# p2004dr/visual-slam

Hardware: AMD Instinct MI355X
Metric: frames/sec (extract+match+pose) at 640×480, 2000 ORB, 1/2/4/8 MI355X (higher is better)
Workload: dtype u8

## Files before the change

include/vslam_amd.h:

```cpp
#ifndef VSLAM_AMD_H
#define VSLAM_AMD_H

#include <stddef.h>
#include <stdint.h>

#ifdef __cplusplus
extern "C" {
#endif

#define MO_ABI_VERSION 7
int mo_abi_version(void);

#define MO_OK 0
#define MO_ERR_ARG (-1)
#define MO_ERR_HIP (-2)
#define MO_ERR_CAPACITY (-3)
#define MO_ERR_UNSUPPORTED (-4)
#define MO_ERR_INDEX (-5)

#define MO_ORDER_LIBSTDCXX 0
#define MO_ORDER_MSVC 1

typedef struct mo_ctx mo_ctx;

// ... 1 lines not shown
    float x, y, size, angle, response;
    int32_t octave, class_id;
} mo_keypoint;

typedef struct {
    int32_t nfeatures;
    float scale_factor;
    int32_t nlevels;
    int32_t edge_threshold;
    int32_t first_level;
    int32_t wta_k;
    int32_t score_type;
    int32_t patch_size;
    int32_t fast_threshold;
    int32_t select_order;
} mo_orb_params;

mo_ctx* mo_create(int device, int max_w, int max_h, int max_batch);
void mo_destroy(mo_ctx*);
const char* mo_last_error(mo_ctx*);
int mo_set_stream(mo_ctx*, void* hip_stream);
int mo_set_stream_null(mo_ctx*);
int mo_sync(mo_ctx*);
int mo_device_count(void);

int mo_orb_detect_compute(mo_ctx*, const mo_orb_params*, const uint8_t* img, int w, int h, int stride, int ch,
                          int batch, mo_keypoint* kps, uint8_t* desc, int cap, int* counts);

int mo_orb_compute(mo_ctx*, const mo_orb_params*, const uint8_t* img, int w, int h, int stride, int ch,
                   const mo_keypoint* kps_in, int n_in, int32_t* kept_idx, uint8_t* desc, int* n_out);

int mo_orb_grid_good_features(mo_ctx*, const uint8_t* img, int w, int h, int stride, int ch, int n_features, float* xy,
                              int* n_out);
int mo_orb_grid_detect_compute(mo_ctx*, const mo_orb_params*, const uint8_t* img, int w, int h, int stride, int ch, int n_features,
                               float* xy, int* n_xy, int32_t* kept_idx, uint8_t* desc, int* n_kept);

int mo_undistort(mo_ctx*, const uint8_t* img, int w, int h, int stride, int ch, const double K[9], const double dist[5], uint8_t* out);
int mo_dev_undistort(mo_ctx*, const uint8_t* d_src, int w, int h, int ch, int batch, const double K[9], const double dist[5],
                     uint8_t* d_dst);

int mo_match_knn2_ratio(mo_ctx*, const uint8_t* q, int nq, const uint8_t* t, int nt, const double* ratio,
                        int batch, int32_t* train_idx, int32_t* dist, uint8_t* pass);

int mo_init_two_view(mo_ctx*, const float* p1, const float* p2, int m, const double K[9], double thr_px,
                     double prob, int n_hyp, uint64_t seed, double R[9], double t[3], double E[9],
                     uint8_t* ransac_inlier , uint8_t* inlier, float* X,
                     int* n_good);

int mo_recover_pose(mo_ctx*, const double E[9], const float* p1, const float* p2, int m, const double K[9],
                    const uint8_t* mask_in, double R[9], double t[3], uint8_t* mask_out, float* X, int* n_good);

int mo_find_fundamental(mo_ctx*, const float* p1, const float* p2, int m, double thr_px, double prob, int n_hyp, uint64_t seed,
                        double F[9], uint8_t* mask, int* n_inliers);

int mo_track_pair(mo_ctx*, const mo_keypoint* kps1, int n1, const uint8_t* desc1, const mo_keypoint* kps2, int n2,
                  const uint8_t* desc2, int w, int h, double ratio, double disp_frac, const double K[9], double thr_px,
                  int n_hyp, uint64_t seed, double R[9], double t[3], double E[9], int32_t* sel_idx, int32_t* sel_dist,
                  int* n_sel, uint8_t* inlier, int* n_inliers);

typedef struct {
    uint64_t token;
    const mo_keypoint* kps;
    const uint8_t* desc;
    int32_t n;
} mo_frame_ref;

typedef struct {
    int32_t mode;
    int32_t w, h;
    double ratio;
    double disp_frac;
    double K[9];
    double thr_px;
    int32_t n_hyp;
    uint64_t seed;
    uint64_t pair_index;
} mo_pair_params;

typedef struct {
    int32_t* match_idx;
    int32_t* match_dist;
    uint8_t* match_pass;
    int32_t* sel_idx;
    int32_t* sel_dist;
    uint8_t* inlier;
    uint8_t* ransac;
    float* X;
    double R[9], t[3], E[9];
    int32_t n_sel;
    int32_t n_good;
    int32_t n1, n2;
    uint64_t token1, token2;
} mo_pair_out;

int mo_last_token(mo_ctx*, uint64_t* token);
int mo_pair_frontend(mo_ctx*, const mo_frame_ref* f1, const mo_frame_ref* f2, const mo_pair_params*, mo_pair_out*);

int mo_triangulate_points(mo_ctx*, const double P1[12], const double P2[12], const float* p1, const float* p2, int n,
                          float* X4);

typedef struct {
    const uint8_t* d_gray;
    int32_t w, h, batch;
    int32_t cap;
    double ratio;
    double K[9];
    double thr_px;
    int32_t n_hyp;
    uint64_t seed;
    mo_keypoint* d_kps;
    uint8_t* d_desc;
    int32_t* d_counts;
    int32_t* d_match_idx;
    int32_t* d_match_dist;
    uint8_t* d_match_pass;
    double* d_pose;
    float* d_points;
    int32_t* d_n_points;
    int32_t mode;
    double disp_frac;
    int32_t* d_sel_idx;
    int32_t* d_sel_dist;
    int32_t* d_sel_n;
    uint8_t* d_pose_mask;
    uint64_t pair_index_base;
    int32_t detector;
    float* d_grid_xy;
    int32_t* d_grid_n;
    int32_t* d_grid_kept;
    int32_t n_kf_pairs;
    const int32_t* d_kf_query;
    const int32_t* d_kf_train;
    const double* d_kf_P1;
    const double* d_kf_P2;
    double* d_kf_F;
} mo_batch_io;

#define MO_MODE_INIT 0
#define MO_MODE_TRACK 1
#define MO_MODE_KEYFRAME 2
#define MO_DETECT_ORB 0
#define MO_DETECT_GRID 1

int mo_dev_frontend_batch(mo_ctx*, const mo_orb_params*, const mo_batch_io*);
int mo_dev_orb_detect_compute(mo_ctx*, const mo_orb_params*, const uint8_t* d_gray, int w, int h, int batch,
                              mo_keypoint* d_kps, uint8_t* d_desc, int cap, int32_t* d_counts);
int mo_dev_match_pairs(mo_ctx*, const uint8_t* d_desc, const int32_t* d_counts, int cap, const int32_t* d_qf,
                       const int32_t* d_tf, int n_pairs, double ratio, int32_t* d_idx, int32_t* d_dist,
                       uint8_t* d_pass);

typedef struct {
    int32_t w, h, ch;
    int32_t chunk;
    int32_t cap;
    int32_t detector;
    int32_t mode;
    double ratio, disp_frac, K[9], thr_px;
    int32_t n_hyp;
    uint64_t seed;
    uint64_t pair_index_base;
    int32_t want_matches;
    int32_t want_points;
} mo_stream_params;

typedef struct {
    int32_t n_frames, n_pairs;
    uint64_t first_frame;
    uint64_t first_pair;
    int32_t cap, flags;
    int32_t prev_count;
    const int32_t* counts;
    const mo_keypoint* kps;
    const uint8_t* desc;
    const int32_t* sel_idx;
    const int32_t* sel_dist;
    const int32_t* sel_n;
    const double* pose;
    const uint8_t* pose_mask;
    const int32_t* n_points;
    const int32_t* match_idx;
    const int32_t* match_dist;
    const uint8_t* match_pass;
    const float* points;
} mo_stream_result;

typedef struct mo_stream mo_stream;
mo_stream* mo_stream_create(mo_ctx*, const mo_orb_params*, const mo_stream_params*);
void mo_stream_destroy(mo_stream*);
int mo_stream_submit(mo_stream*, const uint8_t* frames, int n, int stride, size_t frame_stride);
int mo_stream_collect(mo_stream*, mo_stream_result*);
int mo_stream_lanes(void);
const char* mo_stream_last_error(mo_stream*);

int mo_comm_unique_id(uint8_t id[128]);
int mo_comm_init(mo_ctx*, const uint8_t id[128], int rank, int world);
int mo_comm_destroy(mo_ctx*);
int mo_gather_map_points(mo_ctx*, const float* d_local, int rows_local, int rows_max, int cap, int root, float* d_all,
                         int32_t* d_rows_all);

typedef struct mo_map mo_map;
typedef struct {
    double ratio;
    double thr_px;
    int32_t n_hyp;
    uint64_t seed;
    uint64_t pair_index;
} mo_map_kf_params;
typedef struct {
    int32_t* match_idx;
    uint8_t* match_pass;
    uint8_t* inlier;
    float* points;
    int32_t* kf_len;
    int32_t* kf_redundant;
    double F[9];
    int32_t n_new;
    int32_t from_token;
    int64_t n_points, n_obs;
} mo_map_kf_out;
typedef struct {
    double ratio;
    double thr_px;
    int32_t min_inliers;
    int32_t max_candidates;
    int32_t n_hyp;
    uint64_t seed;
} mo_map_reloc_params;
typedef struct {
    int32_t* point;
    uint8_t* inlier;
    int32_t* cand_pos;
    int32_t* cand_score;
    int32_t* cand_inliers;
    double pose[12];
    int32_t ok;
    int32_t kf_pos;
    int32_t n_cand;
    int32_t n_corr;
    int32_t n_inliers;
    int32_t from_token;
} mo_map_reloc_out;
#define MO_MAP_XYZ 0
#define MO_MAP_COLOR 1
#define MO_MAP_ID 2
#define MO_MAP_OBS_OFF 3
#define MO_MAP_OBS_KF 4
#define MO_MAP_OBS_KP 5
#define MO_MAP_DREF_KF 6
#define MO_MAP_DREF_ROW 7
#define MO_MAP_LIST_OFF 8
#define MO_MAP_LIST_IDS 9
mo_map* mo_map_create(mo_ctx*, int kf_slots, int kf_rows, int64_t pts_cap, int64_t obs_cap);
void mo_map_destroy(mo_map*);
int mo_map_add_keyframe(mo_map*, const mo_frame_ref* f, const double P[12], const uint8_t* img, int w, int h, int ch,
                        const mo_map_kf_params*, mo_map_kf_out*);
int mo_map_add_points(mo_map*, int n, const float* xyz, const uint8_t* col, const int32_t* id, const int32_t* obs_off, const int32_t* obs_kf,
                      const int32_t* obs_kp, const int32_t* dref_kf, const int32_t* dref_row);
int mo_map_remove_keyframes(mo_map*, const int32_t* positions, int n);
int mo_map_sizes(mo_map*, int64_t out[6]);
int mo_map_download(mo_map*, int field, void* dst, size_t bytes);
int mo_map_write_ply(mo_map*, const char* path, int min_obs, int64_t* n_written);
int mo_map_relocalize(mo_map*, const mo_frame_ref* f, const double K[9], const mo_map_reloc_params*, mo_map_reloc_out*);

typedef struct {
    int32_t w, h;
    int32_t window;
    int32_t n_pass;
    double radius[4];
    double scale_factor;
    double ratio;
    double chi2;
    int32_t max_dist;
    int32_t min_matches;
    int32_t min_inliers;
} mo_map_track_params;
typedef struct {
    int32_t* point;
    int32_t* dist;
    uint8_t* inlier;
    double pose[12];
    double pass_pose[4][12];
    double pass_radius[4];
    int32_t pass_cand[4];
    int32_t pass_matches[4];
    int32_t pass_inliers[4];
    int32_t n_pass_run;
    int32_t n_local;
    int32_t ok;
    int32_t from_token;
} mo_map_track_out;
int mo_map_track(mo_map*, const mo_frame_ref* f, const double K[9], const double pose0[12], const mo_map_track_params*, mo_map_track_out*);
int mo_format_floats(const float* v, int64_t n, char* out, size_t cap, size_t* len);

int mo_dev_status(mo_ctx*, int32_t flags[4]);

int mo_stage_times(mo_ctx*, const char*** names, float* ms, int cap);
int mo_stage_times_back(mo_ctx*, int back, const char*** names, float* ms, int cap);

int mo_host_times(mo_ctx*, double us[4]);
int mo_set_host_timing(mo_ctx*, int on);

int mo_dbg_pyramid_level(mo_ctx*, const mo_orb_params*, const uint8_t* gray, int w, int h, int level, int blurred,
                         uint8_t* out , int* lw, int* lh);
int mo_dbg_fast_level(mo_ctx*, const mo_orb_params*, const uint8_t* gray, int w, int h, int level,
                      int32_t* xys , int cap, int* n);
int mo_dbg_min_eigen(mo_ctx*, const uint8_t* gray, int w, int h, float* eig );
int mo_dbg_set_poison(mo_ctx*, int byte );
int mo_dbg_retain_best(mo_ctx*, const float* resp, int n, int n_points, int select_order, int32_t* order, int* n_out);

#ifdef __cplusplus
}
#endif
#endif
```

visual-slam_amd/csrc/api.hip:

```cpp
#include <algorithm>
#include <cmath>
#include <cstring>
#include <vector>

#include "common.h"

int mo_decode_host_flags(mo_ctx* c, int f0, int f1, const char* cap_msg) {
    if (f0 & 1) { c->tie_overflow = true; c->tie_levels = f1; return mo_fail(c, MO_ERR_CAPACITY, "internal per-level keypoint capacity exceeded (response ties)"); }
    if (f0 & 2) return mo_fail(c, MO_ERR_CAPACITY, cap_msg);
    return MO_OK;
}

extern "C" int mo_set_host_timing(mo_ctx* c, int on) {
    if (!c) return MO_ERR_ARG;
    c->host_timing = on != 0;
    return MO_OK;
}

extern "C" int mo_host_times(mo_ctx* c, double us[4]) {
    if (!c || !us) return MO_ERR_ARG;
    for (int i = 0; i < 4; i++) us[i] = c->host_us[i];
    return MO_OK;
}

static bool grow_fin_slots(mo_ctx* c, int levels);

static int check_flags(mo_ctx* c) {
    int f[4] = {0, 0, 0, 0};
    HIPCHK(c, hipMemcpyAsync(f, mo_host_flags(c), sizeof(f), hipMemcpyDeviceToHost, c->stream));
    HIPCHK(c, hipStreamSynchronize(c->stream));
    return mo_decode_host_flags(c, f[0], f[1]);
}

extern "C" int mo_dev_status(mo_ctx* c, int32_t flags[4]) {
    if (!c) return MO_ERR_ARG;
    HIPCHK(c, hipSetDevice(c->device));
    int f[4] = {0, 0, 0, 0};
    HIPCHK(c, hipMemcpyAsync(f, c->d_flags, sizeof(f), hipMemcpyDeviceToHost, c->stream));
    HIPCHK(c, hipMemsetAsync(c->d_flags, 0, 4 * sizeof(int), c->stream));
    HIPCHK(c, hipStreamSynchronize(c->stream));
    if (flags) { flags[0] = f[0]; flags[1] = f[1]; flags[2] = flags[3] = 0; }
    if (f[0] & 1) grow_fin_slots(c, f[1]);
    if (f[0] & 15) return mo_fail(c, MO_ERR_CAPACITY, "a capacity flag was raised by a mo_dev_* call (see mo_dev_status in vslam_amd.h)");
    return MO_OK;
}

int mo_run_extract(mo_ctx* c, const mo_orb_params* p, const uint8_t* d_gray, int w, int h, int batch,
                   mo_keypoint* d_kps, uint8_t* d_desc, int cap, int32_t* d_counts, int host_call) {
    int rc = mo_build_plan(c, p, w, h, batch);
    if (rc) return rc;
    if (cap < 1) return mo_fail(c, MO_ERR_ARG, "cap must be >= 1");
    c->flags_cur = host_call ? mo_host_flags(c) : c->d_flags;
    if (host_call == 1) HIPCHK(c, hipMemsetAsync(mo_host_flags(c), 0, 4 * sizeof(int), c->stream));
    if (c->poison >= 0) {
        HIPCHK(c, hipMemsetAsync(c->d_pyr, c->poison, (size_t)c->batch_alloc * c->plan.pyr_stride, c->stream));
        HIPCHK(c, hipMemsetAsync(c->d_blur, c->poison, (size_t)c->batch_alloc * c->plan.blur_stride, c->stream));
    }
    if (host_call) mo_stage_mark(c, "h2d");
    else mo_stage_begin(c);
    const int blur_margin = (c->plan.edge_threshold - 19) & ~3, pyr_margin = std::max(blur_margin - 4, 0);
    if (batch <= MO_FS_MAX_BATCH && c->fs_ok) {
        if ((rc = orb_launch_front_single(c, d_gray, batch, d_desc != nullptr))) return rc;
        mo_stage_mark(c, "pyramid");
        if (d_desc) mo_stage_mark(c, "blur");
    } else {
        if ((rc = orb_launch_pyramid(c, d_gray, batch, c->plan.nlevels, pyr_margin))) return rc;
        mo_stage_mark(c, "pyramid");
        if (d_desc) {
            if ((rc = orb_launch_blur(c, d_gray, batch, c->plan.nlevels, blur_margin))) return rc;
            mo_stage_mark(c, "blur");
        }
    }
    if ((rc = orb_launch_fast(c, d_gray, batch))) return rc;
    mo_stage_mark(c, "fast_nms");
    if ((rc = orb_launch_select(c, d_gray, batch))) return rc;
    mo_stage_mark(c, "select_harris");
    if ((rc = orb_launch_describe(c, d_gray, batch, d_kps, d_desc, cap, d_counts))) return rc;
    mo_stage_mark(c, "angle_rbrief");
    return MO_OK;
}

static int run_grid_extract(mo_ctx* c, const mo_orb_params* p, const mo_batch_io* io) {
    const int w = io->w, h = io->h, batch = io->batch, cap = io->cap;
    int rc = mo_build_plan(c, p, w, h, batch);
    if (rc) return rc;
    if (p->nfeatures < 64) return mo_fail(c, MO_ERR_ARG, "n_features must be >= 64 (8x8 grid)");
    if (cap < 1) return mo_fail(c, MO_ERR_ARG, "cap must be >= 1");
    const int per_cell = p->nfeatures / 64, slots = 64 * per_cell;
    const size_t B = (size_t)batch;
    Layout L;
    const size_t o_eig = L.take(B * w * h * sizeof(float)), o_xy = L.take(B * slots * 2 * sizeof(float)), o_n = L.take(B * 66 * sizeof(int)),
                 o_kb = L.take(B * 65 * sizeof(int32_t));
    if ((rc = mo_reserve(c, c->d_tmp, c->tmp_bytes, L.total))) return rc;
    float* d_eig = L.at<float>(c->d_tmp, o_eig);
    float* d_xy = io->d_grid_xy ? io->d_grid_xy : L.at<float>(c->d_tmp, o_xy);
    int* d_n = io->d_grid_n ? io->d_grid_n : L.at<int>(c->d_tmp, o_n);
    c->flags_cur = c->d_flags;
    mo_stage_begin(c);
    if ((rc = gftt_launch(c, io->d_gray, w, h, p->nfeatures, d_eig, d_xy, d_n, batch))) return rc;
    int32_t* d_kb = L.at<int32_t>(c->d_tmp, o_kb);
    if ((rc = gftt_records_launch(c, d_xy, d_n, per_cell, w, h, p->edge_threshold, io->d_kps, io->d_grid_kept, cap, io->d_counts, batch, d_kb))) return rc;
    mo_stage_mark(c, "grid_good_features");
    const int blur_margin = (c->plan.edge_threshold - 19) & ~3;
    if ((rc = orb_launch_blur(c, io->d_gray, batch, 1, blur_margin))) return rc;
    mo_stage_mark(c, "blur");
    rc = orb_launch_describe_cells(c, io->d_kps, d_kb, io->d_desc, cap, batch);
    if (rc == MO_ERR_UNSUPPORTED) rc = orb_launch_describe_given(c, io->d_gray, io->d_kps, cap, io->d_desc, io->d_counts, batch, 1);
    if (rc) return rc;
    mo_stage_mark(c, "compute");
    return MO_OK;
}

static int stage_images(mo_ctx* c, const uint8_t* img, int w, int h, int stride, int ch, int batch, const uint8_t** d_gray) {
    if (!img) return mo_fail(c, MO_ERR_ARG, "img is NULL");
    if (ch != 1 && ch != 3) return mo_fail(c, MO_ERR_ARG, "ch must be 1 (gray) or 3 (BGR)");
    if (stride < w * ch) return mo_fail(c, MO_ERR_ARG, "stride smaller than a row");
    size_t row = (size_t)w * ch, frame = row * h;
    int rc = mo_reserve(c, c->d_in, c->d_in_bytes, frame * batch);
    if (rc) return rc;
    HIPCHK(c, hipMemcpy2DAsync(c->d_in, row, img, (size_t)stride, row, (size_t)h * batch, hipMemcpyHostToDevice, c->stream));
    if (ch == 3) {
        rc = mo_reserve(c, c->d_gray, c->d_gray_bytes, (size_t)w * h * batch);
        if (rc) return rc;
        if ((rc = orb_launch_gray(c, c->d_in, w, h, batch, c->d_gray))) return rc;
        *d_gray = c->d_gray;
    } else {
        *d_gray = c->d_in;
    }
    return MO_OK;
}

static int reserve_out(mo_ctx* c, int batch, int cap) {
    const size_t n = (size_t)batch * cap;
    int rc = mo_reserve(c, c->d_kps, c->kps_bytes, n * sizeof(mo_keypoint));
    if (!rc) rc = mo_reserve(c, c->d_desc, c->desc_bytes, n * 32);
    if (!rc) rc = mo_reserve(c, c->d_counts, c->counts_bytes, (size_t)batch * sizeof(int));
    return rc;
}

int mo_host_stage(mo_ctx* c, size_t bytes) {
    if (c->h_stage_bytes >= bytes) return MO_OK;
    if (c->h_stage) { HIPCHK(c, hipStreamSynchronize(c->stream)); hipHostFree(c->h_stage); c->h_stage = nullptr; c->h_stage_bytes = 0; }
    bytes = (bytes + ((size_t)1 << 20) - 1) & ~(((size_t)1 << 20) - 1);
    HIPCHK(c, hipHostMalloc((void**)&c->h_stage, bytes, hipHostMallocMapped | hipHostMallocCoherent));
    c->h_stage_bytes = bytes;
    return MO_OK;
}

static bool grow_fin_slots(mo_ctx* c, int levels) {
    if (!c->plan_valid) return false;
    if (!levels) levels = (1 << c->plan.nlevels) - 1;
    bool grown = false;
    for (int L = 0; L < c->plan.nlevels; L++)
        if (((levels >> L) & 1) && c->plan.lv[L].fin_cap < c->plan.lv[L].cand_cap && c->fin_slack[L] < (1 << 24)) { c->fin_slack[L] *= 8; grown = true; }
    c->fin_slack_dirty = c->fin_slack_dirty || grown;
    return grown;
}

static int detect_compute_once(mo_ctx* c, const mo_orb_params* p, const uint8_t* img, int w, int h, int stride, int ch,
                               int batch, mo_keypoint* kps, uint8_t* desc, int cap, int* counts) {
    HIPCHK(c, hipSetDevice(c->device));
    if (batch == 1 && (size_t)w * h * ch + (size_t)cap * 60 <= (size_t)64 << 20) return mo_detect_single(c, p, img, w, h, stride, ch, kps, desc, cap, counts);
    HostClock clk(c);
    const uint8_t* d_gray = nullptr;
    int rc = mo_build_plan(c, p, w, h, batch);
    if (rc) return rc;
    mo_stage_begin(c);
    if ((rc = stage_images(c, img, w, h, stride, ch, batch, &d_gray))) return rc;
    if ((rc = reserve_out(c, batch, cap))) return rc;
    if ((rc = mo_run_extract(c, p, d_gray, w, h, batch, c->d_kps, desc ? c->d_desc : nullptr, cap, c->d_counts, true))) return rc;
    const size_t n_rows = (size_t)batch * cap, o_cnt = 4 * sizeof(int), o_kps = (o_cnt + (size_t)batch * sizeof(int) + 15) & ~(size_t)15;
    const size_t o_desc = o_kps + n_rows * sizeof(mo_keypoint), total = o_desc + (desc ? n_rows * 32 : 0);
    if (total <= (size_t)2 << 20) {
        if ((rc = mo_host_stage(c, total))) return rc;
        uint8_t* hs = c->h_stage;
        HIPCHK(c, hipMemcpyAsync(hs, mo_host_flags(c), 4 * sizeof(int), hipMemcpyDeviceToHost, c->stream));
        HIPCHK(c, hipMemcpyAsync(hs + o_cnt, c->d_counts, (size_t)batch * sizeof(int), hipMemcpyDeviceToHost, c->stream));
        HIPCHK(c, hipMemcpyAsync(hs + o_kps, c->d_kps, n_rows * sizeof(mo_keypoint), hipMemcpyDeviceToHost, c->stream));
        if (desc) HIPCHK(c, hipMemcpyAsync(hs + o_desc, c->d_desc, n_rows * 32, hipMemcpyDeviceToHost, c->stream));
        mo_stage_mark(c, "d2h");
        clk.enqueued();
        HIPCHK(c, hipStreamSynchronize(c->stream));
        clk.waited();
        std::memcpy(counts, hs + o_cnt, (size_t)batch * sizeof(int));
        if ((rc = mo_decode_host_flags(c, ((const int*)hs)[0], ((const int*)hs)[1]))) return rc;
        for (int f = 0; f < batch; f++) {
            const int n = std::min(counts[f], cap);
            if (n <= 0) continue;
            std::memcpy(kps + (size_t)f * cap, hs + o_kps + (size_t)f * cap * sizeof(mo_keypoint), (size_t)n * sizeof(mo_keypoint));
            if (desc) std::memcpy(desc + (size_t)f * cap * 32, hs + o_desc + (size_t)f * cap * 32, (size_t)n * 32);
        }
        return MO_OK;
    }
    HIPCHK(c, hipMemcpyAsync(counts, c->d_counts, (size_t)batch * sizeof(int), hipMemcpyDeviceToHost, c->stream));
    rc = check_flags(c);
    if (rc) return rc;
    for (int f = 0; f < batch; f++) {
        int n = std::min(counts[f], cap);
        if (n <= 0) continue;
        HIPCHK(c, hipMemcpyAsync(kps + (size_t)f * cap, c->d_kps + (size_t)f * cap, (size_t)n * sizeof(mo_keypoint),
                                 hipMemcpyDeviceToHost, c->stream));
        if (desc)
            HIPCHK(c, hipMemcpyAsync(desc + (size_t)f * cap * 32, c->d_desc + (size_t)f * cap * 32, (size_t)n * 32,
                                     hipMemcpyDeviceToHost, c->stream));
    }
    HIPCHK(c, hipStreamSynchronize(c->stream));
    return MO_OK;
}

extern "C" int mo_orb_detect_compute(mo_ctx* c, const mo_orb_params* p, const uint8_t* img, int w, int h, int stride, int ch,
                                     int batch, mo_keypoint* kps, uint8_t* desc, int cap, int* counts) {
    if (!c) return MO_ERR_ARG;
    if (!kps || !counts) return mo_fail(c, MO_ERR_ARG, "kps/counts is NULL");
    for (;;) {
        c->tie_overflow = false; c->tie_levels = 0;
        const int rc = detect_compute_once(c, p, img, w, h, stride, ch, batch, kps, desc, cap, counts);
        if (rc != MO_ERR_CAPACITY || !c->tie_overflow || !grow_fin_slots(c, c->tie_levels)) return rc;
    }
}

extern "C" int mo_orb_compute(mo_ctx* c, const mo_orb_params* p, const uint8_t* img, int w, int h, int stride, int ch,
                              const mo_keypoint* kps_in, int n_in, int32_t* kept_idx, uint8_t* desc, int* n_out) {
    if (!c) return MO_ERR_ARG;
    if (!p || !n_out || (n_in > 0 && (!kps_in || !kept_idx || !desc))) return mo_fail(c, MO_ERR_ARG, "NULL argument");
    HIPCHK(c, hipSetDevice(c->device));
    *n_out = 0;
    int nlevels = 0;
    bool sorted = true;
    for (int i = 0; i < n_in; i++) {
        int L = kps_in[i].octave;
        if (L < 0) return mo_fail(c, MO_ERR_ARG, "keypoint octave < 0");
        if (i > 0 && L < kps_in[i - 1].octave) sorted = false;
        nlevels = std::max(nlevels, L);
    }
    nlevels++;
    if (nlevels > MO_MAX_LEVELS) return mo_fail(c, MO_ERR_UNSUPPORTED, "keypoint octave >= 12");
    std::vector<int> keep;
    int et = p->edge_threshold;
    if (!(et > 0 && (h <= et * 2 || w <= et * 2))) {
        for (int i = 0; i < n_in; i++) {
            int x = (int)lrintf(kps_in[i].x), y = (int)lrintf(kps_in[i].y);
            if (et > 0 && !(x >= et && x < w - et && y >= et && y < h - et)) continue;
            keep.push_back(i);
        }
    }
    if (!sorted) {
        std::vector<int> re;
        for (int L = 0; L < nlevels; L++)
            for (int i : keep)
                if (kps_in[i].octave == L) re.push_back(i);
        keep.swap(re);
    }
    int n = (int)keep.size();
    for (int i = 0; i < n; i++) kept_idx[i] = keep[i];
    *n_out = n;
    if (n == 0) return MO_OK;
    mo_orb_params pp = *p;
    if (nlevels > pp.nlevels) pp.nlevels = nlevels;
    int rc = mo_build_plan(c, &pp, w, h, 1);
    if (rc) return rc;
    const uint8_t* d_gray = nullptr;
    if ((rc = stage_images(c, img, w, h, stride, ch, 1, &d_gray))) return rc;
    std::vector<mo_keypoint> kk(n);
    for (int i = 0; i < n; i++) kk[i] = kps_in[keep[i]];
    const size_t kb = (size_t)n * sizeof(mo_keypoint);
    Layout L;
    const size_t o_k = L.take(kb), o_d = L.take((size_t)n * 32);
    if ((rc = mo_reserve(c, c->d_tmp, c->tmp_bytes, L.total))) return rc;
    mo_keypoint* d_k = L.at<mo_keypoint>(c->d_tmp, o_k);
    uint8_t* d_d = L.at<uint8_t>(c->d_tmp, o_d);
    HIPCHK(c, hipMemcpyAsync(d_k, kk.data(), kb, hipMemcpyHostToDevice, c->stream));
    mo_stage_begin(c);
    if ((rc = orb_launch_pyramid(c, d_gray, 1, nlevels, 0))) return rc;
    if ((rc = orb_launch_blur(c, d_gray, 1, nlevels, 0))) return rc;
    if ((rc = orb_launch_describe_given(c, d_gray, d_k, n, d_d))) return rc;
    mo_stage_mark(c, "compute");
    HIPCHK(c, hipMemcpyAsync(desc, d_d, (size_t)n * 32, hipMemcpyDeviceToHost, c->stream));
    HIPCHK(c, hipStreamSynchronize(c->stream));
    return MO_OK;
}

extern "C" int mo_dev_undistort(mo_ctx* c, const uint8_t* d_src, int w, int h, int ch, int batch, const double K[9],
                                const double dist[5], uint8_t* d_dst) {
    if (!c) return MO_ERR_ARG;
    if (!d_src || !d_dst || !K || !dist || d_src == d_dst) return mo_fail(c, MO_ERR_ARG, "NULL argument (or in-place)");
    if (w < 1 || h < 1 || batch < 1 || (ch != 1 && ch != 3)) return mo_fail(c, MO_ERR_ARG, "bad size / channel count");
    if (!(K[0] != 0.0) || !(K[4] != 0.0)) return mo_fail(c, MO_ERR_ARG, "focal length is zero");
    HIPCHK(c, hipSetDevice(c->device));
    return undistort_launch(c, d_src, d_dst, w, h, ch, batch, K, dist);
}

extern "C" int mo_undistort(mo_ctx* c, const uint8_t* img, int w, int h, int stride, int ch, const double K[9], const double dist[5],
                            uint8_t* out) {
    if (!c) return MO_ERR_ARG;
    if (!img || !out || !K || !dist) return mo_fail(c, MO_ERR_ARG, "NULL argument");
    if (w < 1 || h < 1 || (ch != 1 && ch != 3) || stride < w * ch) return mo_fail(c, MO_ERR_ARG, "bad size / stride / channel count");
    if (!(K[0] != 0.0) || !(K[4] != 0.0)) return mo_fail(c, MO_ERR_ARG, "focal length is zero");
    HIPCHK(c, hipSetDevice(c->device));
    const size_t row = (size_t)w * ch, frame = row * h;
    Layout L;
    const size_t o_src = L.take(frame), o_dst = L.take(frame);
    int rc = mo_reserve(c, c->d_tmp, c->tmp_bytes, L.total);
    if (rc) return rc;
    uint8_t* d_src = L.at<uint8_t>(c->d_tmp, o_src);
    uint8_t* d_dst = L.at<uint8_t>(c->d_tmp, o_dst);
    HIPCHK(c, hipMemcpy2DAsync(d_src, row, img, (size_t)stride, row, (size_t)h, hipMemcpyHostToDevice, c->stream));
    mo_stage_begin(c);
    if ((rc = undistort_launch(c, d_src, d_dst, w, h, ch, 1, K, dist))) return rc;
    mo_stage_mark(c, "undistort");
    HIPCHK(c, hipMemcpyAsync(out, d_dst, frame, hipMemcpyDeviceToHost, c->stream));
    HIPCHK(c, hipStreamSynchronize(c->stream));
    return MO_OK;
}

static int gftt_run(mo_ctx* c, const uint8_t* img, int w, int h, int stride, int ch, int n_features, float* xy, int* n_out,
                    float* eig_out) {
    if (w < 64 || h < 64 || w > c->max_w || h > c->max_h) return mo_fail(c, MO_ERR_ARG, "image size outside the context limits");
    if (n_features < 64) return mo_fail(c, MO_ERR_ARG, "n_features must be >= 64 (8x8 grid)");
    const uint8_t* d_gray = nullptr;
    int rc = stage_images(c, img, w, h, stride, ch, 1, &d_gray);
    if (rc) return rc;
    const int per_cell = n_features / 64;
    const size_t eig_b = (size_t)w * h * sizeof(float), xy_b = (size_t)64 * per_cell * 2 * sizeof(float);
    Layout L;
    const size_t o_eig = L.take(eig_b), o_xy = L.take(xy_b), o_n = L.take(64 * sizeof(int));
    if ((rc = mo_reserve(c, c->d_tmp, c->tmp_bytes, L.total))) return rc;
    float* d_eig = L.at<float>(c->d_tmp, o_eig);
    float* d_xy = L.at<float>(c->d_tmp, o_xy);
    int* d_n = L.at<int>(c->d_tmp, o_n);
    c->flags_cur = mo_host_flags(c);
    HIPCHK(c, hipMemsetAsync(mo_host_flags(c), 0, 4 * sizeof(int), c->stream));
    mo_stage_begin(c);
    if ((rc = gftt_launch(c, d_gray, w, h, n_features, d_eig, d_xy, d_n))) return rc;
    mo_stage_mark(c, "grid_good_features");
    if (eig_out) HIPCHK(c, hipMemcpyAsync(eig_out, d_eig, eig_b, hipMemcpyDeviceToHost, c->stream));
    std::vector<float> hxy((size_t)64 * per_cell * 2);
    int hn[64];
    HIPCHK(c, hipMemcpyAsync(hxy.data(), d_xy, xy_b, hipMemcpyDeviceToHost, c->stream));
    HIPCHK(c, hipMemcpyAsync(hn, d_n, sizeof(hn), hipMemcpyDeviceToHost, c->stream));
    HIPCHK(c, hipStreamSynchronize(c->stream));
    int n = 0;
    if (xy)
        for (int cell = 0; cell < 64; cell++)
            for (int i = 0; i < hn[cell]; i++, n++) {
                xy[2 * n] = hxy[((size_t)cell * per_cell + i) * 2];
                xy[2 * n + 1] = hxy[((size_t)cell * per_cell + i) * 2 + 1];
            }
    if (n_out) *n_out = n;
    return MO_OK;
}

extern "C" int mo_orb_grid_good_features(mo_ctx* c, const uint8_t* img, int w, int h, int stride, int ch, int n_features,
                                         float* xy, int* n_out) {
    if (!c) return MO_ERR_ARG;
    if (!img || !xy || !n_out) return mo_fail(c, MO_ERR_ARG, "NULL argument");
    HIPCHK(c, hipSetDevice(c->device));
    return gftt_run(c, img, w, h, stride, ch, n_features, xy, n_out, nullptr);
}

extern "C" int mo_orb_grid_detect_compute(mo_ctx* c, const mo_orb_params* p, const uint8_t* img, int w, int h, int stride, int ch,
                                          int n_features, float* xy, int* n_xy, int32_t* kept_idx, uint8_t* desc, int* n_kept) {
    if (!c) return MO_ERR_ARG;
    if (!p || !img || !xy || !n_xy || !kept_idx || !desc || !n_kept) return mo_fail(c, MO_ERR_ARG, "NULL argument");
    HIPCHK(c, hipSetDevice(c->device));
    HostClock clk(c);
    *n_xy = 0; *n_kept = 0;
    c->last_token = 0;
    if (w < 64 || h < 64 || w > c->max_w || h > c->max_h) return mo_fail(c, MO_ERR_ARG, "image size outside the context limits");
    if (n_features < 64) return mo_fail(c, MO_ERR_ARG, "n_features must be >= 64 (8x8 grid)");
    if (ch != 1 && ch != 3) return mo_fail(c, MO_ERR_ARG, "ch must be 1 (gray) or 3 (BGR)");
    if (stride < w * ch) return mo_fail(c, MO_ERR_ARG, "stride smaller than a row");
    int rc = mo_build_plan(c, p, w, h, 1);
// ... 135 lines not shown
    if (!p1 || !p2 || !K || !R || !t || !inlier || !X || !n_good) return mo_fail(c, MO_ERR_ARG, "NULL argument");
    if (m < 0) return mo_fail(c, MO_ERR_ARG, "m must be >= 0");
    HIPCHK(c, hipSetDevice(c->device));
    *n_good = 0;
    if (m < 8) {
        for (int i = 0; i < 9; i++) R[i] = NAN;
        for (int i = 0; i < 3; i++) t[i] = NAN;
        std::memset(inlier, 0, (size_t)m);
        if (ransac_inlier) std::memset(ransac_inlier, 0, (size_t)m);
        if (E) for (int i = 0; i < 9; i++) E[i] = NAN;
        for (int i = 0; i < 3 * m; i++) X[i] = NAN;
        return MO_OK;
    }
    const size_t pb = (size_t)m * 2 * sizeof(float);
    Layout L;
    const size_t o_pose = L.take(12 * sizeof(double)), o_E = L.take(9 * sizeof(double)), o_n = L.take(sizeof(int32_t)), o_p1 = L.take(pb),
                 o_p2 = L.take(pb), o_X = L.take((size_t)m * 3 * sizeof(float)), o_inl = L.take(m), o_ran = L.take(m);
    int rc = mo_reserve(c, c->d_tmp, c->tmp_bytes, L.total);
    if (rc) return rc;
    uint8_t* b = (uint8_t*)c->d_tmp;
    double* d_pose = L.at<double>(b, o_pose);
    double* d_E = L.at<double>(b, o_E);
    int32_t* d_n = L.at<int32_t>(b, o_n);
    float* d_p1 = L.at<float>(b, o_p1);
    float* d_p2 = L.at<float>(b, o_p2);
    float* d_X = L.at<float>(b, o_X);
    uint8_t* d_inl = b + o_inl;
    uint8_t* d_ran = b + o_ran;
    HIPCHK(c, hipMemcpyAsync(d_p1, p1, pb, hipMemcpyHostToDevice, c->stream));
    HIPCHK(c, hipMemcpyAsync(d_p2, p2, pb, hipMemcpyHostToDevice, c->stream));
    TwoViewArgs a;
    a.n_pairs = 1; a.cap = m; a.n_hyp = n_hyp;
    for (int i = 0; i < 9; i++) a.K[i] = K[i];
    a.thr_px = thr_px; a.seed = seed;
    a.d_p1 = d_p1; a.d_p2 = d_p2; a.m_fixed = m;
    a.d_pose = d_pose; a.d_E = d_E; a.d_points = d_X; a.d_inlier = d_inl; a.d_ransac = d_ran; a.d_n_points = d_n;
    mo_stage_begin(c);
    if ((rc = twoview_launch(c, a))) return rc;
    mo_stage_mark(c, "two_view");
    double pose[12];
    int32_t ng = 0;
    HIPCHK(c, hipMemcpyAsync(pose, d_pose, sizeof(pose), hipMemcpyDeviceToHost, c->stream));
    if (E) HIPCHK(c, hipMemcpyAsync(E, d_E, 9 * sizeof(double), hipMemcpyDeviceToHost, c->stream));
    HIPCHK(c, hipMemcpyAsync(&ng, d_n, sizeof(ng), hipMemcpyDeviceToHost, c->stream));
    HIPCHK(c, hipMemcpyAsync(X, d_X, (size_t)m * 3 * sizeof(float), hipMemcpyDeviceToHost, c->stream));
    HIPCHK(c, hipMemcpyAsync(inlier, d_inl, (size_t)m, hipMemcpyDeviceToHost, c->stream));
    if (ransac_inlier) HIPCHK(c, hipMemcpyAsync(ransac_inlier, d_ran, (size_t)m, hipMemcpyDeviceToHost, c->stream));
    HIPCHK(c, hipStreamSynchronize(c->stream));
    for (int i = 0; i < 9; i++) R[i] = pose[i];
    for (int i = 0; i < 3; i++) t[i] = pose[9 + i];
    *n_good = ng;
    return MO_OK;
}

extern "C" int mo_recover_pose(mo_ctx* c, const double E[9], const float* p1, const float* p2, int m, const double K[9],
                               const uint8_t* mask_in, double R[9], double t[3], uint8_t* mask_out, float* X, int* n_good) {
    if (!c) return MO_ERR_ARG;
    if (!E || !K || !R || !t || !n_good || m < 0 || (m > 0 && (!p1 || !p2 || !mask_out))) return mo_fail(c, MO_ERR_ARG, "NULL / negative argument");
    HIPCHK(c, hipSetDevice(c->device));
    *n_good = 0;
    for (int i = 0; i < 9; i++) R[i] = NAN;
    for (int i = 0; i < 3; i++) t[i] = NAN;
    if (m == 0) return MO_OK;
    const size_t pb = (size_t)m * 2 * sizeof(float);
    Layout L;
    const size_t o_p1 = L.take(pb), o_p2 = L.take(pb), o_E = L.take(9 * sizeof(double)), o_min = L.take(m), o_pose = L.take(12 * sizeof(double)),
                 o_X = L.take((size_t)m * 3 * sizeof(float)), o_inl = L.take(m), o_n = L.take(sizeof(int32_t));
    int rc = mo_reserve(c, c->d_tmp, c->tmp_bytes, L.total);
    if (rc) return rc;
    uint8_t* b = (uint8_t*)c->d_tmp;
    HIPCHK(c, hipMemcpyAsync(b + o_p1, p1, pb, hipMemcpyHostToDevice, c->stream));
    HIPCHK(c, hipMemcpyAsync(b + o_p2, p2, pb, hipMemcpyHostToDevice, c->stream));
    HIPCHK(c, hipMemcpyAsync(b + o_E, E, 9 * sizeof(double), hipMemcpyHostToDevice, c->stream));
    if (mask_in) HIPCHK(c, hipMemcpyAsync(b + o_min, mask_in, (size_t)m, hipMemcpyHostToDevice, c->stream));
    TwoViewArgs a;
    a.n_pairs = 1; a.cap = m;
    for (int i = 0; i < 9; i++) a.K[i] = K[i];
    a.thr_px = 1.0;
    a.d_p1 = L.at<float>(b, o_p1); a.d_p2 = L.at<float>(b, o_p2); a.m_fixed = m;
    a.d_E_in = L.at<double>(b, o_E); a.d_mask_in = mask_in ? b + o_min : nullptr;
    a.d_pose = L.at<double>(b, o_pose); a.d_points = L.at<float>(b, o_X); a.d_inlier = b + o_inl; a.d_n_points = L.at<int32_t>(b, o_n);
    mo_stage_begin(c);
    if ((rc = twoview_launch(c, a))) return rc;
    mo_stage_mark(c, "recover_pose");
    double pose[12];
    int32_t ng = 0;
    HIPCHK(c, hipMemcpyAsync(pose, b + o_pose, sizeof(pose), hipMemcpyDeviceToHost, c->stream));
    HIPCHK(c, hipMemcpyAsync(mask_out, b + o_inl, (size_t)m, hipMemcpyDeviceToHost, c->stream));
    if (X) HIPCHK(c, hipMemcpyAsync(X, b + o_X, (size_t)m * 3 * sizeof(float), hipMemcpyDeviceToHost, c->stream));
    HIPCHK(c, hipMemcpyAsync(&ng, b + o_n, sizeof(ng), hipMemcpyDeviceToHost, c->stream));
    HIPCHK(c, hipStreamSynchronize(c->stream));
    for (int i = 0; i < 9; i++) R[i] = pose[i];
    for (int i = 0; i < 3; i++) t[i] = pose[9 + i];
    *n_good = ng;
    return MO_OK;
}

extern "C" int mo_find_fundamental(mo_ctx* c, const float* p1, const float* p2, int m, double thr_px, double prob, int n_hyp,
                                   uint64_t seed, double F[9], uint8_t* mask, int* n_inliers) {
    (void)prob;
    if (!c) return MO_ERR_ARG;
    if (!F || !n_inliers || m < 0 || (m > 0 && (!p1 || !p2 || !mask))) return mo_fail(c, MO_ERR_ARG, "NULL / negative argument");
    HIPCHK(c, hipSetDevice(c->device));
    *n_inliers = 0;
    for (int i = 0; i < 9; i++) F[i] = NAN;
    if (m < 8) { if (m > 0) std::memset(mask, 0, (size_t)m); return MO_OK; }
    const size_t pb = (size_t)m * 2 * sizeof(float);
    Layout L;
    const size_t o_p1 = L.take(pb), o_p2 = L.take(pb), o_F = L.take(9 * sizeof(double)), o_X = L.take((size_t)m * 3 * sizeof(float)),
                 o_ran = L.take(m), o_n = L.take(sizeof(int32_t));
    int rc = mo_reserve(c, c->d_tmp, c->tmp_bytes, L.total);
    if (rc) return rc;
    uint8_t* b = (uint8_t*)c->d_tmp;
    HIPCHK(c, hipMemcpyAsync(b + o_p1, p1, pb, hipMemcpyHostToDevice, c->stream));
    HIPCHK(c, hipMemcpyAsync(b + o_p2, p2, pb, hipMemcpyHostToDevice, c->stream));
    TwoViewArgs a = tv_fundamental(1, m, n_hyp, thr_px, seed, 0);
    a.d_p1 = L.at<float>(b, o_p1); a.d_p2 = L.at<float>(b, o_p2); a.m_fixed = m;
    a.d_E = L.at<double>(b, o_F); a.d_points = L.at<float>(b, o_X); a.d_ransac = b + o_ran; a.d_n_points = L.at<int32_t>(b, o_n);
    mo_stage_begin(c);
    if ((rc = twoview_launch(c, a))) return rc;
    mo_stage_mark(c, "find_fundamental");
    int32_t ng = 0;
    HIPCHK(c, hipMemcpyAsync(F, b + o_F, 9 * sizeof(double), hipMemcpyDeviceToHost, c->stream));
    HIPCHK(c, hipMemcpyAsync(mask, b + o_ran, (size_t)m, hipMemcpyDeviceToHost, c->stream));
    HIPCHK(c, hipMemcpyAsync(&ng, b + o_n, sizeof(ng), hipMemcpyDeviceToHost, c->stream));
    HIPCHK(c, hipStreamSynchronize(c->stream));
    *n_inliers = ng;
    return MO_OK;
}

extern "C" int mo_track_pair(mo_ctx* c, const mo_keypoint* kps1, int n1, const uint8_t* desc1, const mo_keypoint* kps2, int n2,
                             const uint8_t* desc2, int w, int h, double ratio, double disp_frac, const double K[9], double thr_px,
                             int n_hyp, uint64_t seed, double R[9], double t[3], double E[9], int32_t* sel_idx, int32_t* sel_dist,
                             int* n_sel, uint8_t* inlier, int* n_inliers) {
    if (!c) return MO_ERR_ARG;
    if (!K || !R || !t || !n_sel || !n_inliers || n1 < 0 || n2 < 0) return mo_fail(c, MO_ERR_ARG, "NULL / negative argument");
    *n_sel = 0; *n_inliers = 0;
    for (int i = 0; i < 9; i++) { R[i] = NAN; if (E) E[i] = NAN; }
    for (int i = 0; i < 3; i++) t[i] = NAN;
    if (n1 == 0 || n2 == 0) return MO_OK;
    if (!kps1 || !kps2 || !desc1 || !desc2 || !sel_idx || !inlier) return mo_fail(c, MO_ERR_ARG, "NULL argument");
    mo_frame_ref f1 = {0, kps1, desc1, n1}, f2 = {0, kps2, desc2, n2};
    mo_pair_params pp;
    std::memset(&pp, 0, sizeof(pp));
    pp.mode = MO_MODE_TRACK; pp.w = w; pp.h = h; pp.ratio = ratio; pp.disp_frac = disp_frac; pp.thr_px = thr_px; pp.n_hyp = n_hyp; pp.seed = seed;
    for (int i = 0; i < 9; i++) pp.K[i] = K[i];
    mo_pair_out o;
    std::memset(&o, 0, sizeof(o));
    o.sel_idx = sel_idx; o.sel_dist = sel_dist; o.inlier = inlier;
    const int rc = mo_pair_frontend(c, &f1, &f2, &pp, &o);
    if (rc) return rc;
    *n_sel = o.n_sel; *n_inliers = o.n_good;
    for (int i = 0; i < 9; i++) { R[i] = o.R[i]; if (E) E[i] = o.E[i]; }
    for (int i = 0; i < 3; i++) t[i] = o.t[i];
    return MO_OK;
}

extern "C" int mo_triangulate_points(mo_ctx* c, const double P1[12], const double P2[12], const float* p1, const float* p2,
                                     int n, float* X4) {
    if (!c) return MO_ERR_ARG;
    if (n < 0 || !P1 || !P2 || (n > 0 && (!p1 || !p2 || !X4))) return mo_fail(c, MO_ERR_ARG, "NULL argument");
    if (n == 0) return MO_OK;
    HIPCHK(c, hipSetDevice(c->device));
    const size_t pb = (size_t)n * 2 * sizeof(float);
    Layout L;
    const size_t o_p1 = L.take(pb), o_p2 = L.take(pb), o_X = L.take((size_t)n * 4 * sizeof(float));
    int rc = mo_reserve(c, c->d_tmp, c->tmp_bytes, L.total);
    if (rc) return rc;
    float* d_p1 = L.at<float>(c->d_tmp, o_p1);
    float* d_p2 = L.at<float>(c->d_tmp, o_p2);
    float* d_X = L.at<float>(c->d_tmp, o_X);
    HIPCHK(c, hipMemcpyAsync(d_p1, p1, pb, hipMemcpyHostToDevice, c->stream));
    HIPCHK(c, hipMemcpyAsync(d_p2, p2, pb, hipMemcpyHostToDevice, c->stream));
    if ((rc = triangulate_launch(c, P1, P2, d_p1, d_p2, n, d_X))) return rc;
    HIPCHK(c, hipMemcpyAsync(X4, d_X, (size_t)n * 4 * sizeof(float), hipMemcpyDeviceToHost, c->stream));
    HIPCHK(c, hipStreamSynchronize(c->stream));
    return MO_OK;
}

extern "C" int mo_dev_orb_detect_compute(mo_ctx* c, const mo_orb_params* p, const uint8_t* d_gray, int w, int h, int batch,
                                         mo_keypoint* d_kps, uint8_t* d_desc, int cap, int32_t* d_counts) {
    if (!c) return MO_ERR_ARG;
    if (!d_gray || !d_kps || !d_counts) return mo_fail(c, MO_ERR_ARG, "NULL device pointer");
    HIPCHK(c, hipSetDevice(c->device));
    return mo_run_extract(c, p, d_gray, w, h, batch, d_kps, d_desc, cap, d_counts, false);
}

extern "C" int mo_dev_match_pairs(mo_ctx* c, const uint8_t* d_desc, const int32_t* d_counts, int cap, const int32_t* d_qf,
                                  const int32_t* d_tf, int n_pairs, double ratio, int32_t* d_idx, int32_t* d_dist,
                                  uint8_t* d_pass) {
    if (!c) return MO_ERR_ARG;
    if (!d_desc || !d_counts || !d_idx || !d_dist || !d_pass) return mo_fail(c, MO_ERR_ARG, "NULL device pointer");
    HIPCHK(c, hipSetDevice(c->device));
    mo_stage_begin(c);
    int rc = match_launch_pairs(c, d_desc, d_desc, (size_t)cap * 32, (size_t)cap * 32, d_counts, d_qf, d_tf, 0, 0, n_pairs, cap,
                                ratio, d_idx, d_dist, d_pass);
    mo_stage_mark(c, "match_knn2_ratio");
    return rc;
}

__global__ void k_pair_frames(int32_t* qf, int32_t* tf, int n) {
    int i = blockIdx.x * blockDim.x + threadIdx.x;
    if (i < n) { qf[i] = i; tf[i] = i + 1; }
}

extern "C" int mo_dev_frontend_batch(mo_ctx* c, const mo_orb_params* p, const mo_batch_io* io) {
    if (!c) return MO_ERR_ARG;
    if (!io || !io->d_gray || !io->d_kps || !io->d_desc || !io->d_counts) return mo_fail(c, MO_ERR_ARG, "NULL in mo_batch_io");
    HIPCHK(c, hipSetDevice(c->device));
    if (io->detector != MO_DETECT_ORB && io->detector != MO_DETECT_GRID) return mo_fail(c, MO_ERR_ARG, "mo_batch_io.detector must be MO_DETECT_ORB or MO_DETECT_GRID");
    int rc = io->detector == MO_DETECT_GRID ? run_grid_extract(c, p, io)
                                            : mo_run_extract(c, p, io->d_gray, io->w, io->h, io->batch, io->d_kps, io->d_desc, io->cap, io->d_counts, false);
    if (rc) return rc;
    if (io->mode == MO_MODE_KEYFRAME) {
        const int np = io->n_kf_pairs;
        if (np < 1) return MO_OK;
        if (!io->d_kf_query || !io->d_kf_train || !io->d_kf_P1 || !io->d_kf_P2 || !io->d_match_idx || !io->d_match_dist || !io->d_match_pass ||
            !io->d_points || !io->d_n_points)
            return mo_fail(c, MO_ERR_ARG, "MO_MODE_KEYFRAME needs d_kf_query / d_kf_train / d_kf_P1 / d_kf_P2, the match outputs, d_points and d_n_points");
        if (io->n_hyp < 1) return mo_fail(c, MO_ERR_ARG, "MO_MODE_KEYFRAME needs n_hyp >= 1");
        rc = match_launch_pairs(c, io->d_desc, io->d_desc, (size_t)io->cap * 32, (size_t)io->cap * 32, io->d_counts, io->d_kf_query, io->d_kf_train,
                                0, 0, np, io->cap, io->ratio, io->d_match_idx, io->d_match_dist, io->d_match_pass);
        if (rc) return rc;
        mo_stage_mark(c, "match_knn2_ratio");
        TwoViewArgs a = tv_fundamental(np, io->cap, io->n_hyp, io->thr_px, io->seed, io->pair_index_base);
        a.d_kps = io->d_kps; a.d_counts = io->d_counts; a.d_match_idx = io->d_match_idx; a.d_match_pass = io->d_match_pass;
        a.d_qf = io->d_kf_query; a.d_tf = io->d_kf_train; a.need_two = 1; a.d_P1 = io->d_kf_P1; a.d_P2 = io->d_kf_P2;
        a.d_E = io->d_kf_F; a.d_points = io->d_points; a.d_n_points = io->d_n_points; a.d_inlier = io->d_pose_mask;
        if ((rc = twoview_launch(c, a))) return rc;
        mo_stage_mark(c, "keyframe_f_ransac_triangulate");
        return MO_OK;
    }
    int n_pairs = io->batch - 1;
    if (n_pairs < 1 || !io->d_match_idx) return MO_OK;
    if (!io->d_match_dist || !io->d_match_pass) return mo_fail(c, MO_ERR_ARG, "match outputs missing");
    if (c->pair_frames_n < n_pairs) {
        if (c->d_pair_frames) { HIPCHK(c, hipStreamSynchronize(c->stream)); HIPCHK(c, hipFree(c->d_pair_frames)); c->d_pair_frames = nullptr; }
        c->pair_frames_n = 0;
        HIPCHK(c, hipMalloc((void**)&c->d_pair_frames, (size_t)n_pairs * 2 * sizeof(int32_t)));
        hipLaunchKernelGGL(k_pair_frames, dim3((n_pairs + 255) / 256), dim3(256), 0, c->stream, c->d_pair_frames, c->d_pair_frames + n_pairs,
                           n_pairs);
        HIPCHK(c, hipGetLastError());
        c->pair_frames_n = n_pairs;
        c->pair_frames_split = n_pairs;
    }
    int32_t* qf = c->d_pair_frames;
    int32_t* tf = qf + c->pair_frames_split;
    rc = match_launch_pairs(c, io->d_desc, io->d_desc, (size_t)io->cap * 32, (size_t)io->cap * 32, io->d_counts, qf, tf, 0, 0,
                            n_pairs, io->cap, io->ratio, io->d_match_idx, io->d_match_dist, io->d_match_pass);
    if (rc) return rc;
    mo_stage_mark(c, "match_knn2_ratio");
    if (io->n_hyp > 0) {
        if (!io->d_points || !io->d_n_points) return mo_fail(c, MO_ERR_ARG, "two-view outputs missing");
        TwoViewArgs a;
        a.n_pairs = n_pairs; a.cap = io->cap; a.n_hyp = io->n_hyp;
        for (int i = 0; i < 9; i++) a.K[i] = io->K[i];
        a.thr_px = io->thr_px; a.seed = io->seed; a.pair_base = io->pair_index_base;
        a.d_kps = io->d_kps; a.d_counts = io->d_counts; a.d_match_idx = io->d_match_idx; a.d_match_pass = io->d_match_pass;
        a.d_pose = io->d_pose; a.d_points = io->d_points; a.d_n_points = io->d_n_points; a.d_inlier = io->d_pose_mask;
        if (io->mode == MO_MODE_TRACK) {
            if (!io->d_sel_idx || !io->d_sel_n) return mo_fail(c, MO_ERR_ARG, "MO_MODE_TRACK needs d_sel_idx and d_sel_n");
            if ((rc = track_select_launch(c, io->d_kps, io->d_counts, qf, tf, io->d_match_idx, io->d_match_dist, io->d_match_pass,
                                          io->cap, n_pairs, io->w, io->h, io->disp_frac, io->d_sel_idx, io->d_sel_dist, io->d_sel_n)))
                return rc;
            mo_stage_mark(c, "track_filters");
            a.d_sel = io->d_sel_idx; a.d_sel_n = io->d_sel_n;
        } else if (io->mode != MO_MODE_INIT) return mo_fail(c, MO_ERR_ARG, "mo_batch_io.mode must be MO_MODE_INIT or MO_MODE_TRACK");
        if ((rc = twoview_launch(c, a))) return rc;
        mo_stage_mark(c, "two_view");
    }
    return MO_OK;
}

extern "C" int mo_dbg_pyramid_level(mo_ctx* c, const mo_orb_params* p, const uint8_t* gray, int w, int h, int level,
                                    int blurred, uint8_t* out, int* lw, int* lh) {
    if (!c) return MO_ERR_ARG;
    HIPCHK(c, hipSetDevice(c->device));
    int rc = mo_build_plan(c, p, w, h, 1);
    if (rc) return rc;
    if (level < 0 || level >= c->plan.nlevels) return mo_fail(c, MO_ERR_ARG, "level out of range");
    const uint8_t* d_gray = nullptr;
    if ((rc = stage_images(c, gray, w, h, w, 1, 1, &d_gray))) return rc;
    const bool fused = (blurred & 2) != 0;
    blurred &= 1;
    if (fused) {
        if (!c->fs_ok) return mo_fail(c, MO_ERR_UNSUPPORTED, std::string("the single-frame pyramid kernel does not cover this geometry: ") + c->fs_why);
        HIPCHK(c, hipMemsetAsync(c->d_pyr, 0xA5, (size_t)c->plan.pyr_stride, c->stream));
        HIPCHK(c, hipMemsetAsync(c->d_blur, 0xA5, (size_t)c->plan.blur_stride, c->stream));
        if ((rc = orb_launch_front_single(c, d_gray, 1, 1))) return rc;
    } else if ((rc = orb_launch_pyramid(c, d_gray, 1, c->plan.nlevels, 0))) return rc;
    const LevelInfo& v = c->plan.lv[level];
    *lw = v.w; *lh = v.h;
    if (blurred) {
        if (!fused && (rc = orb_launch_blur(c, d_gray, 1, c->plan.nlevels, 0))) return rc;
        HIPCHK(c, hipMemcpy2DAsync(out, v.w, c->d_blur + v.boff, v.bpitch, v.w, v.h, hipMemcpyDeviceToHost, c->stream));
    } else {
        const uint8_t* src = level == 0 ? d_gray : c->d_pyr + v.off;
        HIPCHK(c, hipMemcpy2DAsync(out, v.w, src, v.pitch, v.w, v.h, hipMemcpyDeviceToHost, c->stream));
    }
    HIPCHK(c, hipStreamSynchronize(c->stream));
    return MO_OK;
}

extern "C" int mo_dbg_fast_level(mo_ctx* c, const mo_orb_params* p, const uint8_t* gray, int w, int h, int level,
                                 int32_t* xys, int cap, int* n) {
    if (!c) return MO_ERR_ARG;
    HIPCHK(c, hipSetDevice(c->device));
    int rc = mo_build_plan(c, p, w, h, 1);
    if (rc) return rc;
    if (level < 0 || level >= c->plan.nlevels) return mo_fail(c, MO_ERR_ARG, "level out of range");
    const uint8_t* d_gray = nullptr;
    if ((rc = stage_images(c, gray, w, h, w, 1, 1, &d_gray))) return rc;
    if ((rc = orb_launch_pyramid(c, d_gray, 1, c->plan.nlevels, 0))) return rc;
    if ((rc = orb_launch_fast(c, d_gray, 1))) return rc;
    const LevelInfo& v = c->plan.lv[level];
    std::vector<int> cnt(std::max(v.nstrips, 1));
    std::vector<uint32_t> ent((size_t)std::max(v.cand_cap, 1));
    if (v.nstrips > 0) {
        HIPCHK(c, hipMemcpyAsync(cnt.data(), c->d_strip_cnt + v.strip_base, v.nstrips * sizeof(int), hipMemcpyDeviceToHost, c->stream));
        HIPCHK(c, hipMemcpyAsync(ent.data(), c->d_cand + v.cand_off, (size_t)v.cand_cap * sizeof(uint32_t), hipMemcpyDeviceToHost, c->stream));
    }
    HIPCHK(c, hipStreamSynchronize(c->stream));
    int k = 0;
    for (int s = 0; s < v.nstrips; s++)
        for (int i = 0; i < cnt[s]; i++) {
            uint32_t e = ent[(size_t)s * v.strip_cap + i];
            if (k < cap) { xys[3 * k] = e & 0xFFF; xys[3 * k + 1] = (e >> 12) & 0xFFF; xys[3 * k + 2] = e >> 24; }
            k++;
        }
    *n = k;
    return MO_OK;
}

extern "C" int mo_dbg_retain_best(mo_ctx* c, const float* resp, int n, int n_points, int select_order, int32_t* order,
                                  int* n_out) {
    if (!c) return MO_ERR_ARG;
    HIPCHK(c, hipSetDevice(c->device));
    if (n <= 0) { *n_out = 0; return MO_OK; }
    float* d_r = nullptr; int32_t* d_o = nullptr; int* d_n = nullptr;
    HIPCHK(c, hipMalloc((void**)&d_r, (size_t)n * sizeof(float)));
    HIPCHK(c, hipMalloc((void**)&d_o, (size_t)n * sizeof(int32_t)));
    HIPCHK(c, hipMalloc((void**)&d_n, sizeof(int)));
    HIPCHK(c, hipMemcpyAsync(d_r, resp, (size_t)n * sizeof(float), hipMemcpyHostToDevice, c->stream));
    int rc = orb_launch_retain_probe(c, d_r, n, n_points, select_order, d_o, d_n);
    if (!rc) {
        HIPCHK(c, hipMemcpyAsync(n_out, d_n, sizeof(int), hipMemcpyDeviceToHost, c->stream));
        HIPCHK(c, hipStreamSynchronize(c->stream));
        HIPCHK(c, hipMemcpy(order, d_o, (size_t)(*n_out) * sizeof(int32_t), hipMemcpyDeviceToHost));
    }
    hipFree(d_r); hipFree(d_o); hipFree(d_n);
    return rc;
}
```

visual-slam_amd/csrc/common.h:

```cpp
#pragma once
#include <hip/hip_runtime.h>
#include <chrono>
#include <cstring>
#include <stdint.h>
#include <string>
#include <type_traits>
#include <vector>

#include "../../include/vslam_amd.h"

#define MO_MAX_LEVELS 12
#define MO_HALF_PATCH 15
#define MO_STRIP_ROWS 8
#ifndef MO_STRIP_ROWS_LATENCY
#define MO_STRIP_ROWS_LATENCY 2
#endif
#define SEL_MAXSTRIPS 2047

struct LevelInfo {
    int w, h, pitch;
    int off;
    int bpitch, boff;
    float scale;
    int quota;
    int bx0, by0, bw, bh;
    uint32_t inv_bw;
    int strip_rows;
    int nstrips;
    int strip_cap;
    int strip_base;
    int cand_off;
    int cand_cap;
    int fin_off, fin_cap;
    int scr_off;
};

struct Plan {
    int w, h, nlevels;
    int edge_threshold, fast_threshold, select_order, nfeatures;
    int pyr_stride;
    int blur_stride;
    int strips_per_frame;
    int cand_stride;
    int fin_stride;
    int umax[MO_HALF_PATCH + 1];
    int gk[7];
    LevelInfo lv[MO_MAX_LEVELS];
};

struct FinalKp {
    uint16_t x, y;
    float response;
};

struct ResizeTab {
    uint32_t* xpk = nullptr; uint32_t* ypk = nullptr;
    int* xofs = nullptr; int* xc1 = nullptr; int* yofs = nullptr; int* yc1 = nullptr;
    bool two_pass_ok = true;
};

#define MO_RESULT_SLOTS 4
#define MO_NSTAGES 16
#define MO_TIMING_SLOTS 64

struct TimingSet {
    hipEvent_t ev[MO_NSTAGES + 1] = {};
    const char* names[MO_NSTAGES + 1] = {};
    int n_stages = 0;
};

struct mo_ctx {
    int device = 0;
    int max_w = 0, max_h = 0, max_batch = 0;
    hipStream_t own_stream = nullptr, stream = nullptr;
    int match_mode = 0;
    int poison = -1;
    std::string err;

    bool plan_valid = false;
    int fin_slack[MO_MAX_LEVELS] = {1, 1, 1, 1, 1, 1, 1, 1, 1, 1, 1, 1};
    bool fin_slack_dirty = false;
    bool tie_overflow = false;
    int tie_levels = 0;
    mo_orb_params plan_params{};
    Plan plan{};
    ResizeTab rtab[MO_MAX_LEVELS];
    int batch_alloc = 0;

    uint8_t* d_in = nullptr;       size_t d_in_bytes = 0;
    uint8_t* d_gray = nullptr;     size_t d_gray_bytes = 0;
    uint8_t* d_pyr = nullptr;
    uint8_t* d_blur = nullptr;
    uint32_t* d_cand = nullptr;
    int* d_strip_cnt = nullptr;
    uint64_t* d_scratch = nullptr;
    size_t scratch_stride = 0;
    FinalKp* d_fin = nullptr;
    int* d_fin_cnt = nullptr;
    uint32_t* d_tile_tab[2] = {nullptr, nullptr};
    int tile_cum[2][MO_MAX_LEVELS + 1] = {};
    int tile_margin = 0;
    uint32_t* d_fs_tab = nullptr; int fs_tiles = 0, fs_stride = 0, fs_lds = 0; bool fs_ok = false; int fs_geom[10] = {}; const char* fs_why = "";
    uint32_t* d_strip_tab = nullptr; int n_strip_tab = 0;
    uint32_t* d_dtile_tab = nullptr; int n_dtiles = 0, dtile_icw_off = 0;
    int* d_dtodo = nullptr; size_t dtodo_bytes = 0;
    int* d_flags = nullptr;
    int* flags_cur = nullptr;
    unsigned lds_attr_done = 0;
    mo_keypoint* d_kps = nullptr; uint8_t* d_desc = nullptr; int* d_counts = nullptr; size_t kps_bytes = 0, desc_bytes = 0, counts_bytes = 0;
    mo_keypoint* d_slot_kps = nullptr; uint8_t* d_slot_desc = nullptr; int32_t* d_slot_cnt = nullptr; int32_t* d_slot_ids = nullptr;
    int slot_cap = 0, slot_cur = -1;
    uint64_t slot_token[MO_RESULT_SLOTS] = {}; int slot_n[MO_RESULT_SLOTS] = {}; uint64_t token_next = 1, last_token = 0;
    bool host_timing = false;
    uint8_t* d_mq = nullptr; uint8_t* d_mt = nullptr; int32_t* d_midx = nullptr; int32_t* d_mdist = nullptr;
    uint8_t* d_mpass = nullptr; size_t m_q_bytes = 0, m_t_bytes = 0, m_idx_bytes = 0, m_dist_bytes = 0, m_pass_bytes = 0;
    uint2* d_match_part = nullptr; size_t match_part_bytes = 0;
    void* d_tv = nullptr; size_t tv_bytes = 0;
    float* d_stream_pts = nullptr; size_t stream_pts_bytes = 0;
    uint32_t* d_track_keys = nullptr; size_t track_keys_bytes = 0;
    void* d_tmp = nullptr; size_t tmp_bytes = 0;

    void* comm = nullptr; int comm_rank = 0, comm_world = 1;
    int32_t* d_comm_cnt = nullptr;

    double host_us[4] = {0, 0, 0, 0};
    uint8_t* h_stage = nullptr; size_t h_stage_bytes = 0;
    int32_t* d_pair_frames = nullptr; int pair_frames_n = 0, pair_frames_split = 0;
    TimingSet tsets[MO_TIMING_SLOTS];
    int tcur = 0;
    bool timing = true;
};

int mo_fail(mo_ctx* c, int code, const std::string& msg);

#define HIPCHK(c, expr)                                                                              \
    do {                                                                                             \
        hipError_t e__ = (expr);                                                                     \
        if (e__ != hipSuccess)                                                                       \
            return mo_fail((c), MO_ERR_HIP, std::string(#expr) + ": " + hipGetErrorString(e__));     \
    } while (0)

template <class T> int mo_reserve(mo_ctx* c, T*& p, size_t& have_bytes, size_t need_bytes) {
    if (need_bytes <= have_bytes && p) return MO_OK;
    T* old = p;
    p = nullptr; have_bytes = 0;
    if (old) HIPCHK(c, hipFree(old));
    HIPCHK(c, hipMalloc((void**)&p, need_bytes ? need_bytes : 16));
    have_bytes = need_bytes;
    return MO_OK;
}

static inline size_t mo_align(size_t v, size_t a) { return (v + a - 1) & ~(a - 1); }

struct Layout {
    size_t total = 0;
    size_t take(size_t bytes) { const size_t o = total; total += mo_align(bytes, 256); return o; }
    template <class T> static T* at(void* base, size_t off) { return (T*)((uint8_t*)base + off); }
};

static inline void mo_copy_rows(uint8_t* dst, const uint8_t* src, size_t row, int h, size_t stride) {
    if (stride == row) std::memcpy(dst, src, row * h);
    else for (int y = 0; y < h; y++) std::memcpy(dst + (size_t)y * row, src + (size_t)y * stride, row);
}

int mo_host_stage(mo_ctx* c, size_t bytes);
static inline int* mo_host_flags(mo_ctx* c) { return c->d_flags + 4; }
int mo_decode_host_flags(mo_ctx* c, int f0, int f1, const char* cap_msg = "more keypoints than cap; counts holds the required sizes");

static inline double now_us() { return std::chrono::duration<double, std::micro>(std::chrono::steady_clock::now().time_since_epoch()).count(); }
struct HostClock {
    mo_ctx* c; double t0, t1 = 0, t2 = 0;
    explicit HostClock(mo_ctx* c_) : c(c_), t0(now_us()) { c->timing = c->host_timing; }
    void enqueued() { t1 = now_us(); }
    void waited() { t2 = now_us(); }
    ~HostClock() {
        const double t3 = now_us();
        if (t1 == 0) t1 = t2 = t3; else if (t2 == 0) t2 = t3;
        c->host_us[0] = t1 - t0; c->host_us[1] = t2 - t1; c->host_us[2] = t3 - t2; c->host_us[3] = t3 - t0;
        c->timing = true;
    }
};

int mo_run_extract(mo_ctx* c, const mo_orb_params* p, const uint8_t* d_gray, int w, int h, int batch, mo_keypoint* d_kps, uint8_t* d_desc,
                   int cap, int32_t* d_counts, int host_call);
int mo_detect_single(mo_ctx* c, const mo_orb_params* p, const uint8_t* img, int w, int h, int stride, int ch, mo_keypoint* kps,
                     uint8_t* desc, int cap, int* counts);

int mo_slot_acquire(mo_ctx* c, int rows, int* slot);
uint64_t mo_slot_commit(mo_ctx* c, int slot, int n);
uint8_t* mo_stage_dev(mo_ctx* c);
int mo_slot_of(const mo_ctx* c, uint64_t token);
int mo_frame_lookup(mo_ctx* c, const mo_frame_ref* f, const char* what, int* slot, int* n);
int mo_frame_copy_rows(mo_ctx* c, const mo_frame_ref* f, int slot, int n, mo_keypoint* d_kps, uint8_t* d_desc);
void mo_copy_out_launch(mo_ctx* c, const void* d_src, void* h_dst_dev, size_t bytes);

void mo_stage_begin(mo_ctx* c);
void mo_stage_mark(mo_ctx* c, const char* name);

int mo_build_plan(mo_ctx* c, const mo_orb_params* p, int w, int h, int batch);

int orb_launch_gray(mo_ctx* c, const uint8_t* d_bgr, int w, int h, int batch, uint8_t* d_gray);
int orb_launch_ingest(mo_ctx* c, const uint8_t* src_mapped, int w, int h, int ch, uint8_t* d_gray, int* flags_clear);
int orb_launch_pyramid(mo_ctx* c, const uint8_t* d_gray, int batch, int nlevels, int margin);
#define MO_FS_MAX_BATCH 2
int fs_build(mo_ctx* c);
int orb_launch_front_single(mo_ctx* c, const uint8_t* d_gray, int batch, int want_blur);
void mo_linear_coeffs(int srcsize, int dstsize, std::vector<int>& ofs, std::vector<int>& c1);
int orb_launch_blur(mo_ctx* c, const uint8_t* d_gray, int batch, int nlevels, int margin);
int orb_launch_fast(mo_ctx* c, const uint8_t* d_gray, int batch, int level_lo = 0, int level_hi = MO_MAX_LEVELS);
int orb_launch_select(mo_ctx* c, const uint8_t* d_gray, int batch, int level_lo = 0, int level_hi = MO_MAX_LEVELS);
int orb_launch_describe(mo_ctx* c, const uint8_t* d_gray, int batch, mo_keypoint* d_kps, uint8_t* d_desc, int cap,
                        int* d_counts);
int orb_launch_describe_given(mo_ctx* c, const uint8_t* d_gray, const mo_keypoint* d_kps, int n, uint8_t* d_desc, const int* d_n = nullptr,
                              int batch = 1, int n_stride = 0);
int gftt_records_launch(mo_ctx* c, const float* d_xy, int* d_cell_n, int per_cell, int w, int h, int edge, mo_keypoint* d_rec,
                        int32_t* d_kept, int rec_stride, int32_t* d_counts_out, int batch, int32_t* d_kbase = nullptr);
int orb_launch_describe_cells(mo_ctx* c, const mo_keypoint* d_kps, const int32_t* d_kbase, uint8_t* d_desc, int cap, int batch);
int orb_launch_retain_probe(mo_ctx* c, const float* d_resp, int n, int n_points, int order, int32_t* d_order,
                            int* d_nout);
int match_launch_pairs(mo_ctx* c, const uint8_t* d_q, const uint8_t* d_t, size_t q_stride, size_t t_stride,
                       const int32_t* d_counts, const int32_t* d_qf, const int32_t* d_tf, int nq_fixed, int nt_fixed,
                       int n_pairs, int out_stride, double ratio, int32_t* d_idx, int32_t* d_dist, uint8_t* d_pass);
int gftt_launch(mo_ctx* c, const uint8_t* d_gray, int w, int h, int n_features, float* d_eig, float* d_xy, int* d_n, int batch = 1);
struct TwoViewArgs {
    int n_pairs = 0, cap = 0, n_hyp = 0;
    int model = 0;
    double K[9] = {}, thr_px = 0;
    uint64_t seed = 0;
    uint64_t pair_base = 0;
    const mo_keypoint* d_kps = nullptr; const int32_t* d_counts = nullptr; const int32_t* d_match_idx = nullptr; const uint8_t* d_match_pass = nullptr;
    const int32_t* d_sel = nullptr; const int32_t* d_sel_n = nullptr;
    const float* d_p1 = nullptr; const float* d_p2 = nullptr; int m_fixed = 0;
    const int32_t* d_qf = nullptr; const int32_t* d_tf = nullptr;
    int need_two = 0;
    const double* d_P1 = nullptr; const double* d_P2 = nullptr;
    const double* d_E_in = nullptr; const uint8_t* d_mask_in = nullptr;
    double* d_pose = nullptr;
    double* d_E = nullptr;
    float* d_points = nullptr;
    uint8_t* d_inlier = nullptr;
    uint8_t* d_ransac = nullptr;
    int32_t* d_n_points = nullptr;
    int* flags = nullptr;
};
static_assert(std::is_trivially_copyable<TwoViewArgs>::value, "TwoViewArgs is a kernel argument");
static inline TwoViewArgs tv_fundamental(int n_pairs, int cap, int n_hyp, double thr_px, uint64_t seed, uint64_t pair_base) {
    TwoViewArgs a;
    a.n_pairs = n_pairs; a.cap = cap; a.n_hyp = n_hyp; a.model = 1;
    a.K[0] = a.K[4] = a.K[8] = 1.0;
    a.thr_px = thr_px; a.seed = seed; a.pair_base = pair_base;
    return a;
}
int twoview_launch(mo_ctx* c, const TwoViewArgs& a);
int undistort_launch(mo_ctx* c, const uint8_t* d_src, uint8_t* d_dst, int w, int h, int ch, int batch, const double K[9],
                     const double dist[5]);
int track_select_launch(mo_ctx* c, const mo_keypoint* d_kps, const int32_t* d_counts, const int32_t* d_qf, const int32_t* d_tf,
                        const int32_t* d_midx, const int32_t* d_mdist, const uint8_t* d_mpass, int cap, int n_pairs, int w, int h,
                        double disp_frac, int32_t* d_sel, int32_t* d_sel_dist, int32_t* d_sel_n);
size_t twoview_workspace_bytes(int n_pairs, int cap, int n_hyp);
int triangulate_launch(mo_ctx* c, const double* P1, const double* P2, const float* d_p1, const float* d_p2, int n, float* d_X4);
```

visual-slam_amd/csrc/ctx.hip:

```cpp
#include <algorithm>
#include <cmath>
#include <cstring>
#include <vector>

#include <cstdlib>

#include "common.h"

int mo_fail(mo_ctx* c, int code, const std::string& msg) {
    if (c) c->err = msg;
    return code;
}

static std::string g_create_err;

static inline int cv_round_f(float v) { return (int)lrintf(v); }
static inline int cv_round_d(double v) { return (int)lrint(v); }
static inline int align_up(int v, int a) { return (v + a - 1) / a * a; }

extern "C" int mo_abi_version(void) { return MO_ABI_VERSION; }

extern "C" int mo_device_count(void) {
    int n = 0;
    if (hipGetDeviceCount(&n) != hipSuccess) return 0;
    return n;
}

extern "C" mo_ctx* mo_create(int device, int max_w, int max_h, int max_batch) {
    int n = 0;
    hipError_t e = hipGetDeviceCount(&n);
    if (e != hipSuccess || n <= 0) {
        g_create_err = "mo_create: no HIP device available (this library has no CPU fallback)";
        return nullptr;
    }
    if (device < 0 || device >= n || max_w < 64 || max_h < 64 || max_w > 4095 || max_h > 4095 || max_batch < 1) {
        g_create_err = "mo_create: bad arguments (need 64 <= w,h <= 4095, batch >= 1, valid device)";
        return nullptr;
    }
    if (hipSetDevice(device) != hipSuccess) {
        g_create_err = "mo_create: hipSetDevice failed";
        return nullptr;
    }
    mo_ctx* c = new mo_ctx();
    c->device = device;
    c->max_w = max_w; c->max_h = max_h; c->max_batch = max_batch;
    if (hipStreamCreateWithFlags(&c->own_stream, hipStreamNonBlocking) != hipSuccess) {
        g_create_err = "mo_create: hipStreamCreate failed";
        delete c;
        return nullptr;
    }
    c->stream = c->own_stream;
    if (const char* e = getenv("VSLAM_AMD_MATCHER")) c->match_mode = std::strcmp(e, "mfma") == 0 ? 1 : 0;
    const unsigned evf = (unsigned)hipEventDisableSystemFence;
    for (TimingSet& t : c->tsets)
        for (int i = 0; i <= MO_NSTAGES; i++) hipEventCreateWithFlags(&t.ev[i], evf);
    if (hipMalloc((void**)&c->d_flags, 8 * sizeof(int)) != hipSuccess) {
        g_create_err = "mo_create: hipMalloc failed";
        delete c;
        return nullptr;
    }
    hipMemset(c->d_flags, 0, 8 * sizeof(int));
    c->flags_cur = c->d_flags;
    return c;
}

static void free_plan_buffers(mo_ctx* c) {
    for (int L = 0; L < MO_MAX_LEVELS; L++) {
        ResizeTab& t = c->rtab[L];
        if (t.xpk) hipFree(t.xpk);
        t = ResizeTab();
    }
    void* bufs[] = {c->d_pyr, c->d_blur, c->d_cand, c->d_strip_cnt, c->d_scratch, c->d_fin, c->d_fin_cnt, c->d_tile_tab[0], c->d_tile_tab[1], c->d_strip_tab, c->d_dtile_tab};
    c->d_dtile_tab = nullptr; c->n_dtiles = 0;
    if (c->d_fs_tab) hipFree(c->d_fs_tab);
    c->d_fs_tab = nullptr; c->fs_ok = false;
    for (void* b : bufs) if (b) hipFree(b);
    c->d_tile_tab[0] = c->d_tile_tab[1] = nullptr; c->d_strip_tab = nullptr; c->n_strip_tab = 0;
    c->d_pyr = c->d_blur = nullptr; c->d_cand = nullptr; c->d_strip_cnt = nullptr; c->d_scratch = nullptr;
    c->d_fin = nullptr; c->d_fin_cnt = nullptr;
    c->batch_alloc = 0;
    c->plan_valid = false;
}

extern "C" void mo_destroy(mo_ctx* c) {
    if (!c) return;
    hipSetDevice(c->device);
    hipDeviceSynchronize();
    mo_comm_destroy(c);
    free_plan_buffers(c);
    void* bufs[] = {c->d_in, c->d_gray, c->d_flags, c->d_kps, c->d_desc, c->d_counts, c->d_mq, c->d_mt,
                    c->d_midx, c->d_mdist, c->d_mpass, c->d_match_part, c->d_tv, c->d_tmp, c->d_pair_frames, c->d_dtodo, c->d_comm_cnt,
                    c->d_slot_kps, c->d_slot_desc, c->d_slot_cnt, c->d_slot_ids, c->d_track_keys, c->d_stream_pts};
    for (void* b : bufs) if (b) hipFree(b);
    if (c->h_stage) hipHostFree(c->h_stage);
    for (TimingSet& t : c->tsets) {
        for (int i = 0; i <= MO_NSTAGES; i++) if (t.ev[i]) hipEventDestroy(t.ev[i]);
    }
    if (c->own_stream) hipStreamDestroy(c->own_stream);
    delete c;
}

extern "C" const char* mo_last_error(mo_ctx* c) { return c ? c->err.c_str() : g_create_err.c_str(); }

extern "C" int mo_set_stream(mo_ctx* c, void* s) {
    if (!c) return MO_ERR_ARG;
    c->stream = s ? (hipStream_t)s : c->own_stream;
    return MO_OK;
}

extern "C" int mo_set_stream_null(mo_ctx* c) {
    if (!c) return MO_ERR_ARG;
    c->stream = nullptr;
    return MO_OK;
}

extern "C" int mo_sync(mo_ctx* c) {
    if (!c) return MO_ERR_ARG;
    HIPCHK(c, hipStreamSynchronize(c->stream));
    return MO_OK;
}

void mo_stage_begin(mo_ctx* c) {
    c->tcur = (c->tcur + 1) % MO_TIMING_SLOTS;
    TimingSet& t = c->tsets[c->tcur];
    t.n_stages = 0;
    if (c->timing) hipEventRecord(t.ev[0], c->stream);
}

void mo_stage_mark(mo_ctx* c, const char* name) {
    TimingSet& t = c->tsets[c->tcur];
    if (!c->timing || t.n_stages >= MO_NSTAGES) return;
    t.names[t.n_stages] = name;
    t.n_stages++;
    hipEventRecord(t.ev[t.n_stages], c->stream);
}

extern "C" int mo_stage_times_back(mo_ctx* c, int back, const char*** names, float* ms, int cap) {
    if (!c) return MO_ERR_ARG;
    if (back < 0 || back >= MO_TIMING_SLOTS) return mo_fail(c, MO_ERR_ARG, "mo_stage_times_back: back outside the ring of event sets");
    TimingSet& t = c->tsets[((c->tcur - back) % MO_TIMING_SLOTS + MO_TIMING_SLOTS) % MO_TIMING_SLOTS];
    if (t.n_stages == 0) return 0;
    HIPCHK(c, hipEventSynchronize(t.ev[t.n_stages]));
    int n = std::min(cap, t.n_stages);
    for (int i = 0; i < n; i++) {
        float v = 0;
        hipEventElapsedTime(&v, t.ev[i], t.ev[i + 1]);
        ms[i] = v;
    }
    t.names[t.n_stages] = nullptr;
    if (names) *names = t.names;
    return n;
}

extern "C" int mo_stage_times(mo_ctx* c, const char*** names, float* ms, int cap) { return mo_stage_times_back(c, 0, names, ms, cap); }

void mo_linear_coeffs(int srcsize, int dstsize, std::vector<int>& ofs, std::vector<int>& c1) {
    ofs.assign(dstsize, 0);
    c1.assign(dstsize, 0);
    double inv_scale = (double)dstsize / (double)srcsize;
    double scale = 1.0 / inv_scale;
    int minofst = 0, maxofst = dstsize;
    for (int val = 0; val < dstsize; val++) {
        double fval = scale * ((double)val + 0.5) - 0.5;
        int ival = (int)std::floor(fval);
        if (ival >= 0 && srcsize > 1) {
            if (ival < srcsize - 1) {
                ofs[val] = ival;
                c1[val] = cv_round_d((fval - (double)ival) * 256.0);
            } else {
                ofs[val] = srcsize - 1;
                maxofst = std::min(maxofst, val);
            }
        } else {
            minofst = std::max(minofst, val + 1);
        }
    }
    for (int val = 0; val < dstsize; val++) {
        if (val < minofst) { ofs[val] = 0; c1[val] = 0; }
        if (val >= maxofst) { ofs[val] = srcsize - 1; c1[val] = 0; }
    }
}

static bool params_equal(const mo_orb_params& a, const mo_orb_params& b) {
    return std::memcmp(&a, &b, sizeof(a)) == 0;
}

int mo_build_plan(mo_ctx* c, const mo_orb_params* p, int w, int h, int batch) {
    if (!p) return mo_fail(c, MO_ERR_ARG, "params is NULL");
    if (w < 64 || h < 64 || w > c->max_w || h > c->max_h)
        return mo_fail(c, MO_ERR_ARG, "image size outside the context's max_w/max_h (or < 64)");
    if (batch < 1 || batch > c->max_batch) return mo_fail(c, MO_ERR_ARG, "batch outside 1..max_batch");
    if (p->nlevels < 1 || p->nlevels > MO_MAX_LEVELS) return mo_fail(c, MO_ERR_ARG, "nlevels must be 1..12");
    if (p->first_level != 0 || p->wta_k != 2 || p->score_type != 0 || p->patch_size != 31)
        return mo_fail(c, MO_ERR_UNSUPPORTED,
                       "only firstLevel=0, WTA_K=2, HARRIS_SCORE, patchSize=31 (the reference's values) are built");
    if (p->edge_threshold < 19 || p->edge_threshold > 1024)
        return mo_fail(c, MO_ERR_UNSUPPORTED, "edge_threshold must be >= 19 (descriptor radius)");
    if (p->nfeatures < 1 || !(p->scale_factor > 1.0f) || p->scale_factor > 2.0f)
        return mo_fail(c, MO_ERR_ARG, "nfeatures >= 1, 1 < scale_factor <= 2");
    if (p->select_order != MO_ORDER_LIBSTDCXX && p->select_order != MO_ORDER_MSVC)
        return mo_fail(c, MO_ERR_ARG, "select_order must be MO_ORDER_LIBSTDCXX or MO_ORDER_MSVC");

    const bool same_key = c->plan_valid && params_equal(c->plan_params, *p) && c->plan.w == w && c->plan.h == h;
    const bool same = same_key && !c->fin_slack_dirty;
    if (!same_key)
        for (int L = 0; L < MO_MAX_LEVELS; L++) c->fin_slack[L] = 1;
    if (same && batch <= c->batch_alloc) return MO_OK;
    HIPCHK(c, hipStreamSynchronize(c->stream));
    free_plan_buffers(c);

    Plan& P = c->plan;
    std::memset(&P, 0, sizeof(P));
    P.w = w; P.h = h; P.nlevels = p->nlevels;
    P.edge_threshold = p->edge_threshold;
    P.fast_threshold = std::min(std::max(p->fast_threshold, 0), 255);
    P.select_order = p->select_order;
    P.nfeatures = p->nfeatures;

    int nl = p->nlevels;
    {
        float factor = (float)(1.0 / (double)p->scale_factor);
        float nd = p->nfeatures * (1 - factor) / (1 - (float)std::pow((double)factor, (double)nl));
        int sum = 0;
        for (int L = 0; L < nl - 1; L++) {
            P.lv[L].quota = cv_round_f(nd);
            sum += P.lv[L].quota;
            nd *= factor;
        }
        P.lv[nl - 1].quota = std::max(p->nfeatures - sum, 0);
    }
    {
        int umax[MO_HALF_PATCH + 2];
        int vmax = (int)std::floor(MO_HALF_PATCH * std::sqrt(2.f) / 2 + 1);
        int vmin = (int)std::ceil(MO_HALF_PATCH * std::sqrt(2.f) / 2);
        for (int v = 0; v <= vmax; ++v) umax[v] = cv_round_d(std::sqrt((double)MO_HALF_PATCH * MO_HALF_PATCH - v * v));
        for (int v = MO_HALF_PATCH, v0 = 0; v >= vmin; --v) {
            while (umax[v0] == umax[v0 + 1]) ++v0;
            umax[v] = v0;
            ++v0;
        }
        for (int v = 0; v <= MO_HALF_PATCH; v++) P.umax[v] = umax[v];
    }
    {
        double k[7], sum = 0;
        for (int i = 0; i < 7; i++) {
            double x = 2.0 * i - 6.0;
            k[i] = std::exp(x * x * (-0.125 / 4.0));
            sum += k[i];
        }
        double mul1 = 1.0 / sum;
        for (int i = 0; i < 7; i++) P.gk[i] = cv_round_f((float)(k[i] * mul1) * 256.f);
    }

    int et = p->edge_threshold;
    int pyr_off = 0, blur_off = 0, strip_base = 0, cand_off = 0, fin_off = 0, scr_off = 0;
    for (int L = 0; L < nl; L++) {
        LevelInfo& v = P.lv[L];
        v.scale = (float)std::pow((double)p->scale_factor, (double)L);
        float inv_scale = 1.0f / v.scale;
        v.w = cv_round_f((float)w * inv_scale);
        v.h = cv_round_f((float)h * inv_scale);
        if (v.w < 1 || v.h < 1) return mo_fail(c, MO_ERR_ARG, "pyramid level collapses to zero size; reduce nlevels");
        if (L == 0) { v.pitch = w; v.off = 0; }
        else {
            v.pitch = align_up(v.w, 16);
            v.off = pyr_off;
            pyr_off += align_up(v.pitch * v.h, 256);
        }
        v.bpitch = align_up(v.w, 16);
        v.boff = blur_off;
        blur_off += align_up(v.bpitch * v.h, 256);
        if (v.w <= 2 * et || v.h <= 2 * et) { v.bx0 = v.by0 = et; v.bw = v.bh = 0; }
        else { v.bx0 = et; v.by0 = et; v.bw = v.w - 2 * et; v.bh = v.h - 2 * et; }
        v.inv_bw = v.bw > 1 ? 0xFFFFFFFFu / (uint32_t)v.bw + 1u : 0u;
        v.strip_rows = c->max_batch <= 2 ? MO_STRIP_ROWS_LATENCY : MO_STRIP_ROWS;
        while (v.strip_rows > 1 && v.strip_rows * v.bw > 16384) v.strip_rows /= 2;
        while (v.strip_rows < MO_STRIP_ROWS && v.bh > 0 && (v.bh + v.strip_rows - 1) / v.strip_rows > SEL_MAXSTRIPS && 2 * v.strip_rows * v.bw <= 16384)
            v.strip_rows *= 2;
        if (v.bw > 16384) return mo_fail(c, MO_ERR_UNSUPPORTED, "level too wide");
        v.nstrips = v.bh > 0 ? (v.bh + v.strip_rows - 1) / v.strip_rows : 0;
        v.strip_cap = ((v.strip_rows + 1) / 2) * ((v.bw + 1) / 2);
        v.strip_base = strip_base;
        strip_base += v.nstrips;
        v.cand_off = cand_off;
        v.cand_cap = v.nstrips * v.strip_cap;
        cand_off += v.cand_cap;
        v.fin_off = fin_off;
        v.fin_cap = (int)std::max<long long>(1, std::min<long long>(v.cand_cap, (4ll * v.quota + 256) * c->fin_slack[L]));
        fin_off += v.fin_cap;
        v.scr_off = scr_off;
        scr_off += v.cand_cap + (v.cand_cap + 1) / 2 + (v.cand_cap / 2 + 8) / 4 + 2 + v.cand_cap / 64 + 12;
    }
    P.pyr_stride = std::max(pyr_off, 256);
    P.blur_stride = blur_off;
    P.strips_per_frame = std::max(strip_base, 1);
    P.cand_stride = std::max(cand_off, 1);
    P.fin_stride = fin_off;
    c->scratch_stride = (size_t)scr_off;

    for (int L = 1; L < nl; L++) {
        std::vector<int> xo, xc, yo, yc;
        mo_linear_coeffs(P.lv[L - 1].w, P.lv[L].w, xo, xc);
        mo_linear_coeffs(P.lv[L - 1].h, P.lv[L].h, yo, yc);
        const int dw = P.lv[L].w, dh = P.lv[L].h, wp = ((dw + 63) & ~63) + 64, hp = ((dh + 63) & ~63) + 64;
        auto pack = [](const std::vector<int>& o, const std::vector<int>& c1, int srcsize, int padded) {
            std::vector<uint32_t> t((size_t)padded);
            for (int i = 0; i < padded; i++) {
                const int j = std::min(i, (int)o.size() - 1), o1 = std::min(o[j] + 1, srcsize - 1);
                t[i] = (uint32_t)o[j] | ((uint32_t)(o1 - o[j]) << 15) | ((uint32_t)c1[j] << 16);
            }
            return t;
        };
        const std::vector<uint32_t> xp = pack(xo, xc, P.lv[L - 1].w, wp), yp = pack(yo, yc, P.lv[L - 1].h, hp);
        bool window_ok = true;
        for (int x = 0; x < dw && window_ok; x++) {
            const int xl = std::min(x + 3, dw - 1);
            window_ok = std::min(xo[xl] + 1, P.lv[L - 1].w - 1) - xo[x] <= 7;
        }
        c->rtab[L].two_pass_ok = window_ok;
        size_t n = (size_t)wp + hp + 2 * dw + 2 * dh;
        int* d = nullptr;
        HIPCHK(c, hipMalloc((void**)&d, n * sizeof(int)));
        ResizeTab& t = c->rtab[L];
        t.xpk = (uint32_t*)d; t.ypk = t.xpk + wp;
        t.xofs = d + wp + hp; t.xc1 = t.xofs + dw; t.yofs = t.xc1 + dw; t.yc1 = t.yofs + dh;
        HIPCHK(c, hipMemcpy(t.xpk, xp.data(), xp.size() * sizeof(uint32_t), hipMemcpyHostToDevice));
        HIPCHK(c, hipMemcpy(t.ypk, yp.data(), yp.size() * sizeof(uint32_t), hipMemcpyHostToDevice));
        HIPCHK(c, hipMemcpy(t.xofs, xo.data(), xo.size() * sizeof(int), hipMemcpyHostToDevice));
        HIPCHK(c, hipMemcpy(t.xc1, xc.data(), xc.size() * sizeof(int), hipMemcpyHostToDevice));
        HIPCHK(c, hipMemcpy(t.yofs, yo.data(), yo.size() * sizeof(int), hipMemcpyHostToDevice));
        HIPCHK(c, hipMemcpy(t.yc1, yc.data(), yc.size() * sizeof(int), hipMemcpyHostToDevice));
    }

    size_t B = (size_t)batch;
    HIPCHK(c, hipMalloc((void**)&c->d_pyr, B * P.pyr_stride));
    HIPCHK(c, hipMalloc((void**)&c->d_blur, B * P.blur_stride));
    HIPCHK(c, hipMalloc((void**)&c->d_cand, B * P.cand_stride * sizeof(uint32_t)));
    HIPCHK(c, hipMalloc((void**)&c->d_strip_cnt, B * P.strips_per_frame * sizeof(int)));
    HIPCHK(c, hipMalloc((void**)&c->d_scratch, B * c->scratch_stride * sizeof(uint64_t)));
    if (hipMalloc((void**)&c->d_fin, B * P.fin_stride * sizeof(FinalKp)) != hipSuccess)
        return mo_fail(c, MO_ERR_HIP, "hipMalloc of the final-keypoint slots failed: " + std::to_string(B * P.fin_stride * sizeof(FinalKp)) +
                                          " bytes (" + std::to_string(batch) + " frames x " + std::to_string(P.fin_stride) + " slots; slots grow with response ties)");
    HIPCHK(c, hipMalloc((void**)&c->d_fin_cnt, B * MO_MAX_LEVELS * sizeof(int)));
    {
        const int rc_fs = fs_build(c);
        if (rc_fs) return rc_fs;
    }
    c->batch_alloc = batch;
    c->plan_params = *p;
    c->plan_valid = true;
    c->fin_slack_dirty = false;
    return MO_OK;
}
```

visual-slam_amd/csrc/orb_kernels.hip:

```cpp
#include <cstring>

#include "common.h"
#include "select_replay.h"
#include "fast_score.h"

__constant__ __attribute__((aligned(16))) int8_t c_pattern[256 * 4] = {
#include "orb_pattern.inc"
};

#define WAVE 64

__device__ __forceinline__ int reflect101(int p, int len) {
    if (len == 1) return 0;
    while (p < 0 || p >= len) p = p < 0 ? -p : 2 * len - 2 - p;
    return p;
}

__device__ __forceinline__ void xcd_map(uint32_t lin, uint32_t per, uint32_t inv_per, uint32_t batch, int& frame, int& item) {
    const uint32_t b8 = batch & ~7u, cut = per * b8;
    const bool head = lin < cut;
    const uint32_t n = head ? lin >> 3 : lin - cut;
    const uint32_t q = inv_per ? __umulhi(n, inv_per) : n;
    item = (int)(n - q * per);
    frame = (int)(head ? (lin & 7u) + 8u * q : b8 + q);
}

__device__ __forceinline__ const uint8_t* level_ptr(const Plan& P, int L, const uint8_t* gray, const uint8_t* pyr,
                                                    int frame) {
    return L == 0 ? gray + (size_t)frame * P.w * P.h : pyr + (size_t)frame * P.pyr_stride + P.lv[L].off;
}

__global__ void k_gray(const uint8_t* __restrict__ bgr, uint8_t* __restrict__ gray, size_t npx) {
    size_t i = (size_t)blockIdx.x * blockDim.x + threadIdx.x;
    if (i >= npx) return;
    int b = bgr[3 * i], g = bgr[3 * i + 1], r = bgr[3 * i + 2];
    gray[i] = (uint8_t)((b * 3735 + g * 19235 + r * 9798 + (1 << 14)) >> 15);
}

int orb_launch_gray(mo_ctx* c, const uint8_t* d_bgr, int w, int h, int batch, uint8_t* d_gray) {
    size_t npx = (size_t)w * h * batch;
    hipLaunchKernelGGL(k_gray, dim3((unsigned)((npx + 255) / 256)), dim3(256), 0, c->stream, d_bgr, d_gray, npx);
    HIPCHK(c, hipGetLastError());
    return MO_OK;
}

__global__ __launch_bounds__(256) void k_ingest(const uint8_t* __restrict__ src, uint8_t* __restrict__ gray, int npx, int ch, int* flags_clear) {
    const int i = (blockIdx.x * 256 + threadIdx.x) * 16;
    if (blockIdx.x == 0 && threadIdx.x == 0 && flags_clear) { flags_clear[0] = 0; flags_clear[1] = 0; flags_clear[2] = 0; flags_clear[3] = 0; }
    if (i >= npx) return;
    if (i + 16 <= npx) {
        if (ch == 1) {
            *(uint4*)(gray + i) = *(const uint4*)(src + i);
        } else {
            const uint4* s4 = (const uint4*)(src + (size_t)3 * i);
            const uint4 a = s4[0], b = s4[1], c = s4[2];
            const uint32_t wsrc[12] = {a.x, a.y, a.z, a.w, b.x, b.y, b.z, b.w, c.x, c.y, c.z, c.w};
            uint32_t o[4];
#pragma unroll
            for (int q = 0; q < 4; q++) {
                uint32_t v = 0;
#pragma unroll
                for (int k = 0; k < 4; k++) {
                    const int byte = 3 * (4 * q + k);
                    const uint32_t bb = (wsrc[byte >> 2] >> (8 * (byte & 3))) & 255u, gg = (wsrc[(byte + 1) >> 2] >> (8 * ((byte + 1) & 3))) & 255u,
                                   rr = (wsrc[(byte + 2) >> 2] >> (8 * ((byte + 2) & 3))) & 255u;
                    v |= ((bb * 3735u + gg * 19235u + rr * 9798u + (1u << 14)) >> 15) << (8 * k);
                }
                o[q] = v;
            }
            *(uint4*)(gray + i) = make_uint4(o[0], o[1], o[2], o[3]);
        }
        return;
    }
    for (int j = i; j < npx; j++) {
        if (ch == 1) gray[j] = src[j];
        else gray[j] = (uint8_t)(((int)src[3 * (size_t)j] * 3735 + (int)src[3 * (size_t)j + 1] * 19235 + (int)src[3 * (size_t)j + 2] * 9798 + (1 << 14)) >> 15);
    }
}

int orb_launch_ingest(mo_ctx* c, const uint8_t* src_mapped, int w, int h, int ch, uint8_t* d_gray, int* flags_clear) {
    const int npx = w * h;
    hipLaunchKernelGGL(k_ingest, dim3((unsigned)((npx + 4095) / 4096)), dim3(256), 0, c->stream, src_mapped, d_gray, npx, ch, flags_clear);
    HIPCHK(c, hipGetLastError());
    return MO_OK;
}

typedef unsigned short u16x2 __attribute__((ext_vector_type(2)));
__device__ __forceinline__ uint32_t udot2(uint32_t a, uint32_t b, uint32_t c) {
    return __builtin_amdgcn_udot2(__builtin_bit_cast(u16x2, a), __builtin_bit_cast(u16x2, b), c, false);
}

#define RS_TW 64
#define RS_TH 64
#define RS_SRC_ROWS 136
#define RS_SRC_PITCH 144

__global__ __launch_bounds__(256) void k_resize(const uint8_t* __restrict__ src, size_t src_fstride, int spitch, int sw, int sh,
                                                uint8_t* __restrict__ dst, size_t dst_fstride, int dpitch, int dw, int dh,
                                                const int* __restrict__ xofs, const int* __restrict__ xc1,
                                                const int* __restrict__ yofs, const int* __restrict__ yc1,
                                                uint32_t inv_per, uint32_t inv_gx, int org) {
    __shared__ __attribute__((aligned(16))) uint8_t s_src[RS_SRC_ROWS * RS_SRC_PITCH];
    __shared__ int s_xo[RS_TW], s_xc[RS_TW], s_yo[RS_TH], s_yc[RS_TH];
    const int tid = threadIdx.x;
    int bx = blockIdx.x, by = blockIdx.y, bz = blockIdx.z;
    {
        int rem;
        xcd_map(bx + gridDim.x * (by + gridDim.y * bz), gridDim.x * gridDim.y, inv_per, gridDim.z, bz, rem);
        by = (int)(inv_gx ? __umulhi((uint32_t)rem, inv_gx) : (uint32_t)rem);
        bx = rem - by * (int)gridDim.x;
    }
    const int tx0 = org + bx * RS_TW, ty0 = org + by * RS_TH;
    const uint8_t* s = src + (size_t)bz * src_fstride;
    const int sx0 = xofs[tx0], sx1 = min(xofs[min(tx0 + RS_TW - 1, dw - 1)] + 1, sw - 1);
    const int sy0 = yofs[ty0], sy1 = min(yofs[min(ty0 + RS_TH - 1, dh - 1)] + 1, sh - 1);
    const int sxa = sx0 & ~3;
    const int ncols = sx1 - sxa + 1, nrows = sy1 - sy0 + 1;
    if (ncols > RS_SRC_PITCH || nrows > RS_SRC_ROWS) return;
    if (tid < RS_TW) {
        int x = min(tx0 + tid, dw - 1);
        s_xo[tid] = xofs[x];
        s_xc[tid] = xc1[x];
    } else if (tid < RS_TW + RS_TH) {
        int y = min(ty0 + tid - RS_TW, dh - 1);
        s_yo[tid - RS_TW] = yofs[y];
        s_yc[tid - RS_TW] = yc1[y];
    }
    if ((spitch & 3) == 0 && (((size_t)s) & 3) == 0) {
        const int ndw = (ncols + 3) >> 2;
        const uint32_t inv = 0x100000u / (uint32_t)ndw + 1u;
        const uint8_t* s0 = s + (size_t)sy0 * spitch + sxa;
        for (int i = tid; i < nrows * ndw; i += 256) {
            const uint32_t r = ((uint32_t)i * inv) >> 20, c4 = (uint32_t)i - r * (uint32_t)ndw;
            ((uint32_t*)(s_src + r * RS_SRC_PITCH))[c4] = *(const uint32_t*)(s0 + r * (uint32_t)spitch + 4u * c4);
        }
    } else {
        for (int i = tid; i < nrows * ncols; i += 256) {
            int r = i / ncols, cc = i - r * ncols;
            s_src[r * RS_SRC_PITCH + cc] = s[(size_t)(sy0 + r) * spitch + sxa + cc];
        }
    }
    __syncthreads();
    const int c0 = (tid & 15) * 4, x = tx0 + c0;
    if (x >= dw) return;
    int ox[4], ox1[4];
    uint32_t mx1[4];
#pragma unroll
    for (int k = 0; k < 4; k++) {
        ox[k] = s_xo[c0 + k] - sxa;
        ox1[k] = min(s_xo[c0 + k] + 1, sw - 1) - sxa;
        mx1[k] = s_xc[c0 + k];
    }
#pragma unroll
    for (int half = 0; half < RS_TH / 16; half++) {
        const int ry = (tid >> 4) + 16 * half, y = ty0 + ry;
        if (y >= dh) break;
        const int oy = s_yo[ry] - sy0, oy1 = min(s_yo[ry] + 1, sh - 1) - sy0;
        const uint32_t my1 = s_yc[ry], my0 = 256 - my1;
        const uint8_t* r0 = s_src + oy * RS_SRC_PITCH;
        const uint8_t* r1 = s_src + oy1 * RS_SRC_PITCH;
        uint32_t packed = 0;
#pragma unroll
        for (int k = 0; k < 4; k++) {
            const uint32_t mx0 = 256 - mx1[k];
            uint32_t h0 = mx0 * r0[ox[k]] + mx1[k] * r0[ox1[k]];
            uint32_t h1 = mx0 * r1[ox[k]] + mx1[k] * r1[ox1[k]];
            uint32_t v = my0 * h0 + my1 * h1;
            packed |= ((v + 32768u) >> 16) << (8 * k);
        }
        *(uint32_t*)(dst + (size_t)bz * dst_fstride + (size_t)y * dpitch + x) = packed;
    }
}


#define RS2_ROWS 136
#define RS2_UNR 5
__global__ __launch_bounds__(256) void k_resize2(const uint8_t* __restrict__ src, size_t src_fstride, int spitch, int sw, int sh,
                                                 uint8_t* __restrict__ dst, size_t dst_fstride, int dpitch, int dw, int dh,
                                                 const uint32_t* __restrict__ xpk, const uint32_t* __restrict__ ypk,
                                                 uint32_t inv_per, uint32_t inv_gx, int org) {
    __shared__ __attribute__((aligned(16))) uint2 s_h[RS2_ROWS][16];
    const int tid = threadIdx.x;
    int bx = blockIdx.x, by = blockIdx.y, bz = blockIdx.z;
    {
        int rem;
        xcd_map(bx + gridDim.x * (by + gridDim.y * bz), gridDim.x * gridDim.y, inv_per, gridDim.z, bz, rem);
        by = (int)(inv_gx ? __umulhi((uint32_t)rem, inv_gx) : (uint32_t)rem);
        bx = rem - by * (int)gridDim.x;
    }
    const int tx0 = org + bx * RS_TW, ty0 = org + by * RS_TH;
    const uint32_t ey0 = ypk[ty0], ey1 = ypk[min(ty0 + RS_TH - 1, dh - 1)];
    const int sy0 = (int)(ey0 & 0x7FFFu), sy1 = (int)(ey1 & 0x7FFFu) + (int)((ey1 >> 15) & 1u);
    const int nrows = sy1 - sy0 + 1;
    if (nrows > RS2_ROWS) return;
    const int cg = tid & 15, rr = tid >> 4;
    const uint4 xe = *(const uint4*)(xpk + tx0 + 4 * cg);
    uint32_t ye[RS_TH / 16];
#pragma unroll
    for (int half = 0; half < RS_TH / 16; half++) ye[half] = ypk[ty0 + rr + 16 * half];
    const uint32_t xk[4] = {xe.x, xe.y, xe.z, xe.w};
    const int ox0 = (int)(xk[0] & 0x7FFFu), ab = ox0 & ~3;
    const uint32_t sh8 = (uint32_t)(ox0 & 3);
    uint32_t sel[4], coef[4];
#pragma unroll
    for (int k = 0; k < 4; k++) {
        const uint32_t a = (xk[k] & 0x7FFFu) - (uint32_t)ox0, b = a + ((xk[k] >> 15) & 1u), c1 = xk[k] >> 16;
        sel[k] = a | (b << 16) | 0x0C000C00u;
        coef[k] = (256u - c1) | (c1 << 16);
    }
    const int o1 = min(ab + 4, spitch - 4), o2 = min(ab + 8, spitch - 4);
    const uint8_t* s0 = src + (size_t)bz * src_fstride + (size_t)sy0 * spitch;
    for (int r0 = rr; r0 < nrows; r0 += 16 * RS2_UNR) {
        uint32_t w[RS2_UNR][3];
#pragma unroll
        for (int i = 0; i < RS2_UNR; i++) {
            const uint8_t* row = s0 + (uint32_t)(min(r0 + 16 * i, nrows - 1) * spitch);
            w[i][0] = *(const uint32_t*)(row + ab); w[i][1] = *(const uint32_t*)(row + o1); w[i][2] = *(const uint32_t*)(row + o2);
        }
#pragma unroll
        for (int i = 0; i < RS2_UNR; i++) {
            const int r = r0 + 16 * i;
            if (r >= nrows) break;
            const uint32_t u0 = __builtin_amdgcn_alignbyte(w[i][1], w[i][0], sh8), u1 = __builtin_amdgcn_alignbyte(w[i][2], w[i][1], sh8);
            uint32_t hv[4];
#pragma unroll
            for (int k = 0; k < 4; k++) hv[k] = udot2(__builtin_amdgcn_perm(u1, u0, sel[k]), coef[k], 0u);
            s_h[r][cg] = make_uint2(hv[0] | (hv[1] << 16), hv[2] | (hv[3] << 16));
        }
    }
    __syncthreads();
    const int x = tx0 + 4 * cg;
    if (x >= dw) return;
#pragma unroll
    for (int half = 0; half < RS_TH / 16; half++) {
        const int y = ty0 + rr + 16 * half;
        if (y >= dh) break;
        const uint32_t e = ye[half], c1 = e >> 16, cy = (256u - c1) | (c1 << 16);
        const int oy = (int)(e & 0x7FFFu) - sy0, oy1 = oy + (int)((e >> 15) & 1u);
        const uint2 a = s_h[oy][cg], b = s_h[oy1][cg];
        const uint32_t v0 = udot2(__builtin_amdgcn_perm(b.x, a.x, 0x05040100u), cy, 32768u);
        const uint32_t v1 = udot2(__builtin_amdgcn_perm(b.x, a.x, 0x07060302u), cy, 32768u);
        const uint32_t v2 = udot2(__builtin_amdgcn_perm(b.y, a.y, 0x05040100u), cy, 32768u);
        const uint32_t v3 = udot2(__builtin_amdgcn_perm(b.y, a.y, 0x07060302u), cy, 32768u);
        const uint32_t packed = __builtin_amdgcn_perm(v1, v0, 0x0C0C0602u) | (__builtin_amdgcn_perm(v3, v2, 0x0C0C0602u) << 16);
        *(uint32_t*)(dst + (size_t)bz * dst_fstride + (size_t)y * dpitch + x) = packed;
    }
}

int orb_launch_pyramid(mo_ctx* c, const uint8_t* d_gray, int batch, int nlevels, int margin) {
    const Plan& P = c->plan;
    for (int L = 1; L < nlevels; L++) {
        const LevelInfo& s = P.lv[L - 1];
        const LevelInfo& d = P.lv[L];
        const uint8_t* src = L == 1 ? d_gray : c->d_pyr + s.off;
        size_t sfs = L == 1 ? (size_t)P.w * P.h : (size_t)P.pyr_stride;
        const ResizeTab& t = c->rtab[L];
        const int org = (d.w > 2 * margin + 8 && d.h > 2 * margin + 8) ? margin : 0;
        dim3 grid((d.w - 2 * org + RS_TW - 1) / RS_TW, (d.h - 2 * org + RS_TH - 1) / RS_TH, batch);
        const uint32_t per = grid.x * grid.y, inv_per = per > 1 ? 0xFFFFFFFFu / per + 1u : 0u, inv_gx = grid.x > 1 ? 0xFFFFFFFFu / grid.x + 1u : 0u;
        const bool al4 = ((((size_t)src) | sfs | (size_t)s.pitch) & 3) == 0 && s.pitch >= 12;
        if (al4 && t.two_pass_ok)
            hipLaunchKernelGGL(k_resize2, grid, dim3(256), 0, c->stream, src, sfs, s.pitch, s.w, s.h, c->d_pyr + d.off,
                               (size_t)P.pyr_stride, d.pitch, d.w, d.h, t.xpk, t.ypk, inv_per, inv_gx, org);
        else
            hipLaunchKernelGGL(k_resize, grid, dim3(256), 0, c->stream, src, sfs, s.pitch, s.w, s.h, c->d_pyr + d.off,
                               (size_t)P.pyr_stride, d.pitch, d.w, d.h, t.xofs, t.xc1, t.yofs, t.yc1, inv_per, inv_gx, org);
    }
    HIPCHK(c, hipGetLastError());
    return MO_OK;
}

#define BT_W 64
#define BT_QW (BT_W / 4)
#define BT_PP (256 / BT_QW)
#define BT_H 58
#define BT_PW (BT_W + 16)
#define BT_ROWS (BT_H + 6)


__device__ __forceinline__ uint32_t hi16_pair_sat_u8(uint32_t a, uint32_t b) {
    uint32_t d;
    asm("v_sat_pk_u8_i16 %0, %1" : "=v"(d) : "v"(__builtin_amdgcn_perm(b, a, 0x07060302u)));
    return d;
}

__global__ __launch_bounds__(256) void k_blur(Plan P, const uint32_t* __restrict__ tile_tab, uint32_t inv_per, int org,
                                              const uint8_t* __restrict__ gray, const uint8_t* __restrict__ pyr,
                                              uint8_t* __restrict__ blur) {
    __shared__ __attribute__((aligned(16))) uint8_t s_px[BT_ROWS * BT_PW];
    __shared__ __attribute__((aligned(16))) uint32_t s_row[(BT_ROWS / 2) * BT_W];
    int tile = blockIdx.x, frame = blockIdx.y;
    xcd_map(blockIdx.x + gridDim.x * blockIdx.y, gridDim.x, inv_per, gridDim.y, frame, tile);
    const uint32_t te = tile_tab[tile];
    const int L = te & 0xFF;
    const LevelInfo lv = P.lv[L];
    const int tx0 = org + (int)((te >> 8) & 0xFFF) * BT_W, ty0 = org + (int)(te >> 20) * BT_H;
    const uint8_t* img = level_ptr(P, L, gray, pyr, frame);
    const int tid = threadIdx.x;
    if ((lv.pitch & 3) == 0 && (((size_t)img) & 3) == 0) {
        auto stage = [&](int r, int c4) {
            const int y = reflect101(ty0 + r - 3, lv.h), x0 = tx0 - 4 + 4 * c4;
            const uint8_t* row = img + (uint32_t)(y * lv.pitch);
            uint32_t v;
            if (x0 >= 0 && x0 + 3 < lv.w) v = *(const uint32_t*)(row + x0);
            else {
                v = 0;
#pragma unroll
                for (int b = 0; b < 4; b++) v |= (uint32_t)row[reflect101(x0 + b, lv.w)] << (8 * b);
            }
            ((uint32_t*)(s_px + r * BT_PW))[c4] = v;
        };
        if (ty0 >= 3 && ty0 + BT_ROWS - 3 <= lv.h && tx0 >= 4 && tx0 + BT_W + 4 <= lv.w) {
            const uint8_t* base = img + (uint32_t)((ty0 - 3) * lv.pitch + tx0 - 4);
#pragma unroll
            for (int r = tid / BT_QW; r < BT_ROWS; r += BT_PP)
                ((uint32_t*)(s_px + r * BT_PW))[1 + tid % BT_QW] = *(const uint32_t*)(base + (uint32_t)(r * lv.pitch) + 4 + 4 * (tid % BT_QW));
            if (tid < 2 * BT_ROWS)
                ((uint32_t*)(s_px + (tid >> 1) * BT_PW))[(tid & 1) * (BT_QW + 1)] =
                    *(const uint32_t*)(base + (uint32_t)((tid >> 1) * lv.pitch) + (tid & 1) * (BT_W + 4));
        } else {
            for (int r = tid / BT_QW; r < BT_ROWS; r += BT_PP) stage(r, 1 + tid % BT_QW);
            for (int i = tid; i < 2 * BT_ROWS; i += 256) stage(i >> 1, (i & 1) * (BT_QW + 1));
        }
    } else {
        for (int i = tid; i < BT_ROWS * (BT_W + 6); i += 256) {
            int r = i / (BT_W + 6), cidx = i - r * (BT_W + 6);
            int y = reflect101(ty0 + r - 3, lv.h), x = reflect101(tx0 + cidx - 3, lv.w);
            s_px[r * BT_PW + cidx + 1] = img[(size_t)y * lv.pitch + x];
        }
    }
    __syncthreads();
    const uint32_t g0 = P.gk[0], g1 = P.gk[1], g2 = P.gk[2], g3 = P.gk[3];
#pragma unroll
    for (int h2 = 0; h2 < BT_ROWS / 2 / BT_PP; h2++) {
        const uint32_t ta = g0 | (g1 << 8) | (g2 << 16) | (g3 << 24), tb = g2 | (g1 << 8) | (g0 << 16);
        const int p = tid / BT_QW + BT_PP * h2, q = tid % BT_QW;
        uint32_t o[2][4];
#pragma unroll
        for (int h = 0; h < 2; h++) {
            const uint32_t* pw = (const uint32_t*)(s_px + (2 * p + h) * BT_PW + 4 * q);
            const uint32_t w0 = pw[0], w1 = pw[1], w2 = pw[2];
            o[h][0] = __builtin_amdgcn_udot4(__builtin_amdgcn_alignbyte(w1, w0, 1), ta, __builtin_amdgcn_udot4(__builtin_amdgcn_alignbyte(w2, w1, 1), tb, 0, false), false);
            o[h][1] = __builtin_amdgcn_udot4(__builtin_amdgcn_alignbyte(w1, w0, 2), ta, __builtin_amdgcn_udot4(__builtin_amdgcn_alignbyte(w2, w1, 2), tb, 0, false), false);
            o[h][2] = __builtin_amdgcn_udot4(__builtin_amdgcn_alignbyte(w1, w0, 3), ta, __builtin_amdgcn_udot4(__builtin_amdgcn_alignbyte(w2, w1, 3), tb, 0, false), false);
            o[h][3] = __builtin_amdgcn_udot4(w1, ta, __builtin_amdgcn_udot4(w2, tb, 0, false), false);
        }
        uint4 packed;
        packed.x = o[0][0] | (o[1][0] << 16);
        packed.y = o[0][1] | (o[1][1] << 16);
        packed.z = o[0][2] | (o[1][2] << 16);
        packed.w = o[0][3] | (o[1][3] << 16);
        *(uint4*)(&s_row[p * BT_W + 4 * q]) = packed;
    }
    __syncthreads();
#pragma unroll
    for (int h2 = 0; h2 < BT_ROWS / 2 / BT_PP; h2++) {
        const int p = tid / BT_QW + BT_PP * h2, c0 = (tid % BT_QW) * 4;
        const int x = tx0 + c0, y = ty0 + 2 * p;
        if (p < BT_H / 2 && y < lv.h && x < lv.w) {
            const uint32_t e0 = g0 | (g1 << 16), e1 = g2 | (g3 << 16), e2 = g2 | (g1 << 16), e3 = g0;
            const uint32_t d0 = g0 << 16, d1 = g1 | (g2 << 16), d2 = g3 | (g2 << 16), d3 = g1 | (g0 << 16);
            uint4 v[4];
#pragma unroll
            for (int j = 0; j < 4; j++) v[j] = *(const uint4*)(&s_row[(p + j) * BT_W + c0]);
            uint32_t se[4], so[4];
#pragma unroll
            for (int k = 0; k < 4; k++) {
                const uint32_t a0 = k == 0 ? v[0].x : k == 1 ? v[0].y : k == 2 ? v[0].z : v[0].w;
                const uint32_t a1 = k == 0 ? v[1].x : k == 1 ? v[1].y : k == 2 ? v[1].z : v[1].w;
                const uint32_t a2 = k == 0 ? v[2].x : k == 1 ? v[2].y : k == 2 ? v[2].z : v[2].w;
                const uint32_t a3 = k == 0 ? v[3].x : k == 1 ? v[3].y : k == 2 ? v[3].z : v[3].w;
                se[k] = udot2(a0, e0, udot2(a1, e1, udot2(a2, e2, udot2(a3, e3, 1u << 15))));
                so[k] = udot2(a0, d0, udot2(a1, d1, udot2(a2, d2, udot2(a3, d3, 1u << 15))));
            }
            const uint32_t pe = hi16_pair_sat_u8(se[0], se[1]) | (hi16_pair_sat_u8(se[2], se[3]) << 16);
            const uint32_t po = hi16_pair_sat_u8(so[0], so[1]) | (hi16_pair_sat_u8(so[2], so[3]) << 16);
            uint8_t* out = blur + (size_t)frame * P.blur_stride + lv.boff + (size_t)y * lv.bpitch + x;
            *(uint32_t*)out = pe;
            if (y + 1 < lv.h) *(uint32_t*)(out + lv.bpitch) = po;
        }
    }
}

int orb_launch_blur(mo_ctx* c, const uint8_t* d_gray, int batch, int nlevels, int margin) {
    const Plan& P = c->plan;
    if (nlevels < 1 || nlevels > P.nlevels) return mo_fail(c, MO_ERR_ARG, "blur: level count outside the plan");
    const int slot = margin > 0 ? 1 : 0;
    if (slot && c->tile_margin != margin && c->d_tile_tab[1]) { hipFree(c->d_tile_tab[1]); c->d_tile_tab[1] = nullptr; }
    if (!c->d_tile_tab[slot]) {
        std::vector<uint32_t> tab;
        for (int L = 0; L < P.nlevels; L++) {
            const int cw = std::max(P.lv[L].w - 2 * margin, 1), chh = std::max(P.lv[L].h - 2 * margin, 1);
            const int tx = (cw + BT_W - 1) / BT_W, ty = (chh + BT_H - 1) / BT_H;
            c->tile_cum[slot][L] = (int)tab.size();
            for (int y = 0; y < ty; y++)
                for (int x = 0; x < tx; x++) tab.push_back((uint32_t)L | ((uint32_t)x << 8) | ((uint32_t)y << 20));
        }
        c->tile_cum[slot][P.nlevels] = (int)tab.size();
        HIPCHK(c, hipMalloc((void**)&c->d_tile_tab[slot], tab.size() * sizeof(uint32_t)));
        HIPCHK(c, hipMemcpy(c->d_tile_tab[slot], tab.data(), tab.size() * sizeof(uint32_t), hipMemcpyHostToDevice));
        if (slot) c->tile_margin = margin;
    }
    const uint32_t per = (uint32_t)c->tile_cum[slot][nlevels], inv_per = per > 1 ? 0xFFFFFFFFu / per + 1u : 0u;
    hipLaunchKernelGGL(k_blur, dim3(per, batch), dim3(256), 0, c->stream, P, c->d_tile_tab[slot], inv_per, margin, d_gray, c->d_pyr,
                       c->d_blur);
    HIPCHK(c, hipGetLastError());
    return MO_OK;
}

__device__ __forceinline__ bool arc9(uint32_t m) {
    uint32_t m32 = m | (m << 16);
    uint32_t x = m32 & (m32 >> 1);
    x &= x >> 2;
    x &= x >> 4;
    x &= m32 >> 8;
    return (x & 0xFFFFu) != 0;
}

__device__ __forceinline__ int arc_score(const int d[16]) {
    int m2[16], m4[16], best = -1000;
#pragma unroll
    for (int i = 0; i < 16; i++) m2[i] = min(d[i], d[(i + 1) & 15]);
#pragma unroll
    for (int i = 0; i < 16; i++) m4[i] = min(m2[i], m2[(i + 2) & 15]);
#pragma unroll
    for (int i = 0; i < 16; i++) {
        int m8 = min(m4[i], m4[(i + 4) & 15]);
        int m9 = min(m8, d[(i + 8) & 15]);
        best = max(best, m9);
    }
    return best - 1;
}

#define FAST_LOAD_D(d, v, p, TW)                                                                              \
    d[0] = v - p[3 * TW];   d[1] = v - p[3 * TW + 1];   d[2] = v - p[2 * TW + 2];   d[3] = v - p[TW + 3];        \
    d[4] = v - p[3];        d[5] = v - p[-TW + 3];      d[6] = v - p[-2 * TW + 2];  d[7] = v - p[-3 * TW + 1];   \
    d[8] = v - p[-3 * TW];  d[9] = v - p[-3 * TW - 1];  d[10] = v - p[-2 * TW - 2]; d[11] = v - p[-TW - 3];      \
    d[12] = v - p[-3];      d[13] = v - p[TW - 3];      d[14] = v - p[2 * TW - 2];  d[15] = v - p[3 * TW - 1];

typedef short s16x2 __attribute__((ext_vector_type(2)));
__device__ __forceinline__ s16x2 pk_min(s16x2 a, s16x2 b) { return __builtin_elementwise_min(a, b); }
__device__ __forceinline__ s16x2 pk_max(s16x2 a, s16x2 b) { return __builtin_elementwise_max(a, b); }

__device__ __forceinline__ int sub16(int a, int b) { int r; asm("v_sub_u16 %0, %1, %2" : "=v"(r) : "v"(a), "v"(b)); return r; }
__device__ __forceinline__ int min16(int a, int b) { int r; asm("v_min_i16 %0, %1, %2" : "=v"(r) : "v"(a), "v"(b)); return r; }
__device__ __forceinline__ int max16(int a, int b) { int r; asm("v_max_i16 %0, %1, %2" : "=v"(r) : "v"(a), "v"(b)); return r; }
__device__ __forceinline__ int add16(int a, int b) { int r; asm("v_add_u16 %0, %1, %2" : "=v"(r) : "v"(a), "v"(b)); return r; }
__device__ __forceinline__ int min16u(int a, int b) { int r; asm("v_min_u16 %0, %1, %2" : "=v"(r) : "v"(a), "v"(b)); return r; }
__device__ __forceinline__ int max16u(int a, int b) { int r; asm("v_max_u16 %0, %1, %2" : "=v"(r) : "v"(a), "v"(b)); return r; }
__device__ __forceinline__ unsigned long long ballot_gt16(int a, int b) {
    unsigned long long m;
    asm("v_cmp_gt_i16 %0, %1, %2" : "=s"(m) : "v"(a), "v"(b));
    return m;
}

__device__ __forceinline__ void lds_store_u16_masked(unsigned long long mask, uint32_t addr, uint32_t val) {
    unsigned long long keep;
    asm volatile("s_mov_b64 %0, exec\n\ts_and_b64 exec, exec, %1\n\tds_write_b16 %2, %3\n\ts_mov_b64 exec, %0"
                 : "=&s"(keep) : "s"(mask), "v"(addr), "v"(val) : "memory", "scc");
}

#define FAST_KEEP_WORDS 512
#define FAST_STACK 384
#define FAST_NMS_Q 128

template <int TW, int NT>
__global__ __launch_bounds__(NT) void k_fast(Plan P, const uint32_t* __restrict__ strip_tab, uint32_t inv_per, int strip0,
                                              const uint8_t* __restrict__ gray, const uint8_t* __restrict__ pyr,
                                              uint32_t* __restrict__ cand, int* __restrict__ strip_cnt, int score_bytes) {
    extern __shared__ __attribute__((aligned(16))) uint8_t smem[];
    int strip = blockIdx.x, frame = blockIdx.y;
    xcd_map(blockIdx.x + gridDim.x * blockIdx.y, gridDim.x, inv_per, gridDim.y, frame, strip);
    const uint32_t se = strip_tab[strip0 + strip];
    const int L = se & 0xFF;
    const LevelInfo lv = P.lv[L];
    strip = (int)(se >> 8);
    if (strip >= lv.nstrips) return;
    const int R = lv.strip_rows;
    const int y0 = lv.by0 + strip * R;
    const int rows = min(R, lv.by0 + lv.bh - y0);
    const int SW = lv.bw + 2;
    const int xs0 = lv.bx0 - 1;
    uint8_t* s_score = smem;
    uint8_t* s_tile = smem + score_bytes;
    constexpr int NW = NT / 64;
    __shared__ int s_wsum[NW];
    __shared__ __attribute__((aligned(16))) uint16_t s_wq[NW][FAST_STACK];
    uint32_t* const s_keep = (uint32_t*)&s_wq[0][0];
    static_assert(sizeof(uint16_t) * NW * FAST_STACK >= 4 * FAST_KEEP_WORDS + sizeof(uint16_t) * NW * FAST_NMS_Q, "bitmap and queues overlay the stacks");
    const uint8_t* img = level_ptr(P, L, gray, pyr, frame);
    const int t = P.fast_threshold;
    const int tid = threadIdx.x, lane = tid & 63;
    const int wv = __builtin_amdgcn_readfirstlane(tid >> 6);

    const bool al16 = (lv.pitch & 15) == 0 && (((size_t)img) & 15) == 0;
    const bool al4 = (lv.pitch & 3) == 0 && (((size_t)img) & 3) == 0;
    const int gx0 = al16 ? (xs0 - 3) & ~15 : (xs0 - 3) & ~3, lead = xs0 - 3 - gx0;
    const int th = rows + 8, gy0 = y0 - 4;
    if (al16) {
        const int tw16 = (SW + 6 + lead + 15) >> 4;
        const uint32_t inv = 0xFFFFFFFFu / (uint32_t)tw16 + 1u;
        for (int i = tid; i < th * tw16; i += NT) {
            const int r = tw16 > 1 ? (int)__umulhi((uint32_t)i, inv) : i, c16 = i - r * tw16;
            *(uint4*)(s_tile + r * TW + 16 * c16) = *(const uint4*)(img + (size_t)(gy0 + r) * lv.pitch + gx0 + 16 * c16);
        }
    } else if (al4) {
        const int tw4 = (SW + 6 + lead + 3) >> 2;
        for (int r = wv; r < th; r += NW) {
            const uint32_t* src = (const uint32_t*)(img + (size_t)(gy0 + r) * lv.pitch + gx0);
            uint32_t* dst = (uint32_t*)(s_tile + r * TW);
            for (int c4 = lane; c4 < tw4; c4 += 64) dst[c4] = src[c4];
        }
    } else {
        const int tw_used = (SW + 6 + lead + 3) & ~3;
        for (int r = wv; r < th; r += NW) {
            const uint8_t* src = img + (size_t)(gy0 + r) * lv.pitch + gx0;
            for (int cc = lane; cc < tw_used; cc += 64) s_tile[r * TW + cc] = (gx0 + cc < lv.w) ? src[cc] : 0;
        }
    }
    for (int i = tid; i < ((rows + 2) * SW + 3) >> 2; i += NT) ((uint32_t*)s_score)[i] = 0;
    __syncthreads();

    typedef const volatile __attribute__((address_space(3))) uint8_t lds_cvu8;
    const int xbits = R > 8 ? 11 : 12;
    const uint32_t xmask = (1u << xbits) - 1u;
    auto score_one = [&](uint32_t e, int flip, bool own) {
        const int r = e >> xbits, x = e & xmask;
        const int pos = r * SW + x;
        lds_cvu8* p = (lds_cvu8*)&s_tile[(r + 3) * TW + x + 3 + lead];
        const int v = (int)p[0];
        int q[16];
#define FAST_P(k, o) q[k] = (int)p[o];
        FAST_P(0, 3 * TW)        FAST_P(1, 3 * TW + 1)    FAST_P(2, 2 * TW + 2)    FAST_P(3, TW + 3)
        FAST_P(4, 3)             FAST_P(5, -TW + 3)       FAST_P(6, -2 * TW + 2)   FAST_P(7, -3 * TW + 1)
        FAST_P(8, -3 * TW)       FAST_P(9, -3 * TW - 1)   FAST_P(10, -2 * TW - 2)  FAST_P(11, -TW - 3)
        FAST_P(12, -3)           FAST_P(13, TW - 3)       FAST_P(14, 2 * TW - 2)   FAST_P(15, 3 * TW - 1)
#undef FAST_P
        auto mn = [](int a, int b2) { return min16u(a, b2); };
        auto mx = [](int a, int b2) { return max16u(a, b2); };
        const int L = flip ? sub16(fast_arc_extreme(q, mn, mx), v) : sub16(v, fast_arc_extreme(q, mx, mn));
        const int b = (int)(short)L;
        if (own && b > t) s_score[pos] = (uint8_t)(b - 1);
    };
    {
        uint16_t* wq = s_wq[wv];
        const int nxc = (SW + 63) >> 6;
        int qd = 0, qb = 0;
        int ra = 0, ja = wv, rb = 0, jb = wv + NW;
        while (ja >= nxc) { ja -= nxc; ra++; }
        while (jb >= nxc) { jb -= nxc; rb++; }
        const int tv = t;
        auto chunk = [&](int r, int j) {
            const int x = (j << 6) + lane;
            const int rem = SW - (j << 6);
            const unsigned long long valid = rem >= 64 ? ~0ull : (1ull << rem) - 1ull;
            const uint8_t* w = &s_tile[r * TW + lead + min(x, SW - 1)];
            const int v = w[3 * TW + 3];
            const int p0 = w[6 * TW + 3], p4 = w[3 * TW + 6], p8 = w[3], p12 = w[3 * TW];
            const int pair_hi = min16u(min16u(max16u(p0, p4), max16u(p4, p8)), min16u(max16u(p8, p12), max16u(p12, p0)));
            const int pair_lo = max16u(max16u(min16u(p0, p4), min16u(p4, p8)), max16u(min16u(p8, p12), min16u(p12, p0)));
            const unsigned long long md = ballot_gt16(sub16(v, tv), pair_hi) & valid;
            const unsigned long long mb = ballot_gt16(pair_lo, add16(v, tv)) & valid;
            const uint32_t e = (uint32_t)((r << xbits) | x);
            const uint32_t wq_lds = (uint32_t)(uintptr_t)wq;
            lds_store_u16_masked(md, wq_lds + 2u * (uint32_t)(qd + __builtin_amdgcn_mbcnt_hi((unsigned)(md >> 32), __builtin_amdgcn_mbcnt_lo((unsigned)md, 0u))), e);
            qd += __popcll(md);
            lds_store_u16_masked(mb, wq_lds + 2u * (uint32_t)(FAST_STACK - 1 - qb - (int)__builtin_amdgcn_mbcnt_hi((unsigned)(mb >> 32), __builtin_amdgcn_mbcnt_lo((unsigned)mb, 0u))), e);
            qb += __popcll(mb);
        };
        while (ra < rows + 2) {
            chunk(ra, ja);
            if (rb < rows + 2) chunk(rb, jb);
            if (qd >= 64 || qb >= 64) {
                replay::wave_sync();
                while (qd >= 64) { qd -= 64; score_one(wq[qd + lane], 0, true); }
                while (qb >= 64) { qb -= 64; score_one(wq[FAST_STACK - 1 - qb - lane], 0xFF, true); }
                replay::wave_sync();
            }
            ja += 2 * NW;
            while (ja >= nxc) { ja -= nxc; ra++; }
            jb += 2 * NW;
            while (jb >= nxc) { jb -= nxc; rb++; }
        }
        replay::wave_sync();
        if (qd > 0) score_one(wq[min(lane, qd - 1)], 0, lane < qd);
        if (qb > 0) score_one(wq[FAST_STACK - 1 - min(lane, qb - 1)], 0xFF, lane < qb);
    }
    __syncthreads();
    for (int i = tid; i < FAST_KEEP_WORDS; i += NT) s_keep[i] = 0;
    __syncthreads();

    const int nitems = rows * lv.bw;
    {
        const uint32_t inv_sw = 0xFFFFFFFFu / (uint32_t)SW + 1u;
        auto nms_at = [&](int p) {
            const int r = (int)__umulhi((uint32_t)p, inv_sw), x = p - r * SW;
            if (r < 1 || r > rows || x < 1 || x > lv.bw) return;
            const uint8_t* c = &s_score[p];
            const int mid = c[0];
            const int nb = max16u(max16u(max16u((int)c[-SW - 1], (int)c[-SW]), max16u((int)c[-SW + 1], (int)c[-1])),
                                  max16u(max16u((int)c[1], (int)c[SW - 1]), max16u((int)c[SW], (int)c[SW + 1])));
            if ((uint16_t)mid > (uint16_t)nb) {
                const int i = (r - 1) * lv.bw + (x - 1);
                atomicOr(&s_keep[i >> 5], 1u << (i & 31));
            }
        };
        uint16_t* const nq = (uint16_t*)(s_keep + FAST_KEEP_WORDS) + wv * FAST_NMS_Q;
        const uint32_t nq_lds = (uint32_t)(uintptr_t)nq;
        const int k_end = ((rows + 1) * SW + 3) >> 2;
        int qn = 0;
        for (int k0 = (SW >> 2) + (wv << 6); k0 < k_end; k0 += NT) {
            const int k = k0 + lane;
            const uint32_t w = k < k_end ? ((const uint32_t*)s_score)[k] : 0u;
#pragma unroll
            for (int bq = 0; bq < 4; bq++) {
                const unsigned long long m = __ballot((w & (0xFFu << (8 * bq))) != 0u);
                lds_store_u16_masked(m, nq_lds + 2u * (uint32_t)(qn + __builtin_amdgcn_mbcnt_hi((unsigned)(m >> 32), __builtin_amdgcn_mbcnt_lo((unsigned)m, 0u))),
                                     (uint32_t)(4 * k + bq));
                qn += __popcll(m);
                if (qn >= 64) {
                    replay::wave_sync();
                    qn -= 64;
                    nms_at(nq[qn + lane]);
                    replay::wave_sync();
                }
            }
        }
        replay::wave_sync();
        if (lane < qn) nms_at(nq[lane]);
    }
    __syncthreads();
    const int nwords = (nitems + 31) >> 5, wpt = (nwords + NT - 1) / NT;
    uint32_t kw[2] = {0u, 0u};
#pragma unroll
    for (int q = 0; q < 2; q++)
        if (q < wpt && tid * wpt + q < nwords) kw[q] = s_keep[tid * wpt + q];
    const int cnt = __popc(kw[0]) + __popc(kw[1]);
    int incl = cnt;
#pragma unroll
    for (int o = 1; o < 64; o <<= 1) {
        int n = __shfl_up(incl, o, 64);
        if (lane >= o) incl += n;
    }
    if (lane == 63) s_wsum[wv] = incl;
    __syncthreads();
    int base = 0;
    for (int k = 0; k < wv; k++) base += s_wsum[k];
    int total = 0;
    for (int k = 0; k < NW; k++) total += s_wsum[k];
    int pos = base + incl - cnt;
    uint32_t* out = cand + (size_t)frame * P.cand_stride + lv.cand_off + (size_t)strip * lv.strip_cap;
#pragma unroll
    for (int q = 0; q < 2; q++) {
        uint32_t bits = kw[q];
        while (bits) {
            const int j = __ffs((int)bits) - 1;
            bits &= bits - 1;
            const int i = (tid * wpt + q) * 32 + j;
            const int rr = lv.bw > 1 ? (int)__umulhi((uint32_t)i, lv.inv_bw) : i, xx = i - rr * lv.bw;
            const int sc = s_score[(rr + 1) * SW + xx + 1];
            if (pos < lv.strip_cap) out[pos] = ((uint32_t)sc << 24) | ((uint32_t)(y0 + rr) << 12) | (uint32_t)(lv.bx0 + xx);
            pos++;
        }
    }
    if (tid == 0) strip_cnt[(size_t)frame * P.strips_per_frame + lv.strip_base + strip] = min(total, lv.strip_cap);
}

template <int TW, int NT> static int launch_fast_tw(mo_ctx* c, const uint8_t* d_gray, int batch, size_t score_bytes, int max_rows,
                                                    int strip0, int nstrips) {
    const Plan& P = c->plan;
    size_t lds = score_bytes + (size_t)(max_rows + 8) * TW + 16;
    if (lds > 128 * 1024) return mo_fail(c, MO_ERR_UNSUPPORTED, "level too wide for the FAST strip kernel");
    const unsigned bit = (TW == 704 ? 1u : TW == 1344 ? 2u : TW == 2112 ? 4u : TW == 608 ? 32u : 8u) << (NT == 512 ? 8 : 0);
    if (!(c->lds_attr_done & bit)) {
        HIPCHK(c, hipFuncSetAttribute((const void*)k_fast<TW, NT>, hipFuncAttributeMaxDynamicSharedMemorySize, 128 * 1024));
        c->lds_attr_done |= bit;
    }
    if (!c->d_strip_tab) {
        std::vector<uint32_t> tab((size_t)P.strips_per_frame, 0xFFFFFF00u);
        for (int L = 0; L < P.nlevels; L++)
            for (int st = 0; st < P.lv[L].nstrips; st++) tab[(size_t)P.lv[L].strip_base + st] = (uint32_t)L | ((uint32_t)st << 8);
        HIPCHK(c, hipMalloc((void**)&c->d_strip_tab, tab.size() * sizeof(uint32_t)));
        HIPCHK(c, hipMemcpy(c->d_strip_tab, tab.data(), tab.size() * sizeof(uint32_t), hipMemcpyHostToDevice));
        c->n_strip_tab = (int)tab.size();
    }
    const uint32_t per = (uint32_t)nstrips, inv_per = per > 1 ? 0xFFFFFFFFu / per + 1u : 0u;
    hipLaunchKernelGGL((k_fast<TW, NT>), dim3(nstrips, batch), dim3(NT), lds, c->stream, P, c->d_strip_tab, inv_per, strip0, d_gray,
                       c->d_pyr, c->d_cand, c->d_strip_cnt, (int)score_bytes);
    HIPCHK(c, hipGetLastError());
    return MO_OK;
}

int orb_launch_fast(mo_ctx* c, const uint8_t* d_gray, int batch, int level_lo, int level_hi) {
    const Plan& P = c->plan;
    level_lo = std::max(level_lo, 0); level_hi = std::min(level_hi, P.nlevels);
    if (level_lo >= level_hi) return MO_OK;
    const int strip0 = P.lv[level_lo].strip_base;
    const int nstrips = (level_hi < P.nlevels ? P.lv[level_hi].strip_base : P.strips_per_frame) - strip0;
    if (nstrips < 1) return MO_OK;
    size_t score_bytes = 0;
    int tw_need = 0, max_rows = 1;
    for (int L = 0; L < P.nlevels; L++) {
        const LevelInfo& v = P.lv[L];
        score_bytes = std::max(score_bytes, (((size_t)(v.strip_rows + 2) * (v.bw + 2) + 15) & ~(size_t)15));
        tw_need = std::max(tw_need, (v.bw + 2 + 6 + 15 + 15) & ~15);
        max_rows = std::max(max_rows, v.strip_rows);
    }
    if (P.strips_per_frame < 1) return MO_OK;
// ... 790 lines not shown
```

visual-slam_amd/vslam_amd/__init__.py:

```python
import ctypes as C
import os
import weakref

import numpy as np

_PKG_ROOT = os.path.dirname(os.path.dirname(os.path.abspath(__file__)))
LIB_PATH = os.environ.get("VSLAM_AMD_LIB") or os.path.join(_PKG_ROOT, "libvslam_amd.so")

MO_OK, MO_ERR_ARG, MO_ERR_HIP, MO_ERR_CAPACITY, MO_ERR_UNSUPPORTED, MO_ERR_INDEX = 0, -1, -2, -3, -4, -5
ABI_VERSION = 7
ORDER_LIBSTDCXX, ORDER_MSVC = 0, 1

KP_DTYPE = np.dtype([("x", "<f4"), ("y", "<f4"), ("size", "<f4"), ("angle", "<f4"), ("response", "<f4"),
                     ("octave", "<i4"), ("class_id", "<i4")])
assert KP_DTYPE.itemsize == 28


class NativeUnavailable(RuntimeError):
    pass


class NativeError(RuntimeError):
    def __init__(self, code, msg):
        super().__init__("libvslam_amd error %d: %s" % (code, msg))
        self.code = code


class OrbParams(C.Structure):
    _fields_ = [("nfeatures", C.c_int32), ("scale_factor", C.c_float), ("nlevels", C.c_int32),
                ("edge_threshold", C.c_int32), ("first_level", C.c_int32), ("wta_k", C.c_int32),
                ("score_type", C.c_int32), ("patch_size", C.c_int32), ("fast_threshold", C.c_int32),
                ("select_order", C.c_int32)]


class BatchIO(C.Structure):
    _fields_ = [("d_gray", C.c_void_p), ("w", C.c_int32), ("h", C.c_int32), ("batch", C.c_int32), ("cap", C.c_int32),
                ("ratio", C.c_double), ("K", C.c_double * 9), ("thr_px", C.c_double), ("n_hyp", C.c_int32),
                ("seed", C.c_uint64),
                ("d_kps", C.c_void_p), ("d_desc", C.c_void_p), ("d_counts", C.c_void_p), ("d_match_idx", C.c_void_p),
                ("d_match_dist", C.c_void_p), ("d_match_pass", C.c_void_p), ("d_pose", C.c_void_p),
                ("d_points", C.c_void_p), ("d_n_points", C.c_void_p),
                ("mode", C.c_int32), ("disp_frac", C.c_double), ("d_sel_idx", C.c_void_p), ("d_sel_dist", C.c_void_p),
                ("d_sel_n", C.c_void_p), ("d_pose_mask", C.c_void_p), ("pair_index_base", C.c_uint64),
                ("detector", C.c_int32), ("d_grid_xy", C.c_void_p), ("d_grid_n", C.c_void_p), ("d_grid_kept", C.c_void_p),
                ("n_kf_pairs", C.c_int32), ("d_kf_query", C.c_void_p), ("d_kf_train", C.c_void_p), ("d_kf_P1", C.c_void_p),
                ("d_kf_P2", C.c_void_p), ("d_kf_F", C.c_void_p)]


class FrameRef(C.Structure):
    _fields_ = [("token", C.c_uint64), ("kps", C.c_void_p), ("desc", C.c_void_p), ("n", C.c_int32)]


class PairParams(C.Structure):
    _fields_ = [("mode", C.c_int32), ("w", C.c_int32), ("h", C.c_int32), ("ratio", C.c_double), ("disp_frac", C.c_double),
                ("K", C.c_double * 9), ("thr_px", C.c_double), ("n_hyp", C.c_int32), ("seed", C.c_uint64), ("pair_index", C.c_uint64)]


class PairOut(C.Structure):
    _fields_ = [("match_idx", C.c_void_p), ("match_dist", C.c_void_p), ("match_pass", C.c_void_p), ("sel_idx", C.c_void_p),
                ("sel_dist", C.c_void_p), ("inlier", C.c_void_p), ("ransac", C.c_void_p), ("X", C.c_void_p),
                ("R", C.c_double * 9), ("t", C.c_double * 3), ("E", C.c_double * 9), ("n_sel", C.c_int32), ("n_good", C.c_int32),
                ("n1", C.c_int32), ("n2", C.c_int32), ("token1", C.c_uint64), ("token2", C.c_uint64)]


class MapKfParams(C.Structure):
    _fields_ = [("ratio", C.c_double), ("thr_px", C.c_double), ("n_hyp", C.c_int32), ("seed", C.c_uint64), ("pair_index", C.c_uint64)]


class MapKfOut(C.Structure):
    _fields_ = [("match_idx", C.c_void_p), ("match_pass", C.c_void_p), ("inlier", C.c_void_p), ("points", C.c_void_p), ("kf_len", C.c_void_p),
                ("kf_redundant", C.c_void_p), ("F", C.c_double * 9), ("n_new", C.c_int32), ("from_token", C.c_int32),
                ("n_points", C.c_int64), ("n_obs", C.c_int64)]


class MapRelocParams(C.Structure):
    _fields_ = [("ratio", C.c_double), ("thr_px", C.c_double), ("min_inliers", C.c_int32), ("max_candidates", C.c_int32), ("n_hyp", C.c_int32),
                ("seed", C.c_uint64)]


class MapRelocOut(C.Structure):
    _fields_ = [("point", C.c_void_p), ("inlier", C.c_void_p), ("cand_pos", C.c_void_p), ("cand_score", C.c_void_p), ("cand_inliers", C.c_void_p),
                ("pose", C.c_double * 12), ("ok", C.c_int32), ("kf_pos", C.c_int32), ("n_cand", C.c_int32), ("n_corr", C.c_int32),
                ("n_inliers", C.c_int32), ("from_token", C.c_int32)]


class MapTrackParams(C.Structure):
    _fields_ = [("w", C.c_int32), ("h", C.c_int32), ("window", C.c_int32), ("n_pass", C.c_int32), ("radius", C.c_double * 4),
                ("scale_factor", C.c_double), ("ratio", C.c_double), ("chi2", C.c_double), ("max_dist", C.c_int32), ("min_matches", C.c_int32),
                ("min_inliers", C.c_int32)]


class MapTrackOut(C.Structure):
    _fields_ = [("point", C.c_void_p), ("dist", C.c_void_p), ("inlier", C.c_void_p), ("pose", C.c_double * 12), ("pass_pose", (C.c_double * 12) * 4),
                ("pass_radius", C.c_double * 4), ("pass_cand", C.c_int32 * 4), ("pass_matches", C.c_int32 * 4), ("pass_inliers", C.c_int32 * 4),
                ("n_pass_run", C.c_int32), ("n_local", C.c_int32), ("ok", C.c_int32), ("from_token", C.c_int32)]


class StreamParams(C.Structure):
    _fields_ = [("w", C.c_int32), ("h", C.c_int32), ("ch", C.c_int32), ("chunk", C.c_int32), ("cap", C.c_int32), ("detector", C.c_int32),
                ("mode", C.c_int32), ("ratio", C.c_double), ("disp_frac", C.c_double), ("K", C.c_double * 9), ("thr_px", C.c_double),
                ("n_hyp", C.c_int32), ("seed", C.c_uint64), ("pair_index_base", C.c_uint64), ("want_matches", C.c_int32),
                ("want_points", C.c_int32)]


class StreamResult(C.Structure):
    _fields_ = [("n_frames", C.c_int32), ("n_pairs", C.c_int32), ("first_frame", C.c_uint64), ("first_pair", C.c_uint64), ("cap", C.c_int32),
                ("flags", C.c_int32), ("prev_count", C.c_int32), ("counts", C.c_void_p), ("kps", C.c_void_p), ("desc", C.c_void_p),
                ("sel_idx", C.c_void_p), ("sel_dist", C.c_void_p), ("sel_n", C.c_void_p), ("pose", C.c_void_p), ("pose_mask", C.c_void_p),
                ("n_points", C.c_void_p), ("match_idx", C.c_void_p), ("match_dist", C.c_void_p), ("match_pass", C.c_void_p),
                ("points", C.c_void_p)]


MODE_INIT, MODE_TRACK, MODE_KEYFRAME = 0, 1, 2
DETECT_ORB, DETECT_GRID = 0, 1
TIMING_SLOTS = 64


_vp, _i, _d = C.c_void_p, C.c_int, C.c_double
SIGNATURES = {
    "mo_create": (_vp, [_i, _i, _i, _i]),
    "mo_destroy": (None, [_vp]),
    "mo_last_error": (C.c_char_p, [_vp]),
    "mo_set_stream": (_i, [_vp, _vp]),
    "mo_set_stream_null": (_i, [_vp]),
    "mo_sync": (_i, [_vp]),
    "mo_device_count": (_i, []),
    "mo_abi_version": (_i, []),
    "mo_orb_detect_compute": (_i, [_vp, _vp, _vp, _i, _i, _i, _i, _i, _vp, _vp, _i, _vp]),
    "mo_orb_compute": (_i, [_vp, _vp, _vp, _i, _i, _i, _i, _vp, _i, _vp, _vp, _vp]),
    "mo_orb_grid_good_features": (_i, [_vp, _vp, _i, _i, _i, _i, _i, _vp, _vp]),
    "mo_orb_grid_detect_compute": (_i, [_vp, _vp, _vp, _i, _i, _i, _i, _i, _vp, _vp, _vp, _vp, _vp]),
    "mo_dbg_min_eigen": (_i, [_vp, _vp, _i, _i, _vp]),
    "mo_dbg_set_poison": (_i, [_vp, _i]),
    "mo_undistort": (_i, [_vp, _vp, _i, _i, _i, _i, _vp, _vp, _vp]),
    "mo_dev_undistort": (_i, [_vp, _vp, _i, _i, _i, _i, _vp, _vp, _vp]),
    "mo_match_knn2_ratio": (_i, [_vp, _vp, _i, _vp, _i, _vp, _i, _vp, _vp, _vp]),
    "mo_init_two_view": (_i, [_vp, _vp, _vp, _i, _vp, _d, _d, _i, C.c_uint64, _vp, _vp, _vp, _vp, _vp, _vp, _vp]),
    "mo_recover_pose": (_i, [_vp, _vp, _vp, _vp, _i, _vp, _vp, _vp, _vp, _vp, _vp, _vp]),
    "mo_find_fundamental": (_i, [_vp, _vp, _vp, _i, _d, _d, _i, C.c_uint64, _vp, _vp, _vp]),
    "mo_track_pair": (_i, [_vp, _vp, _i, _vp, _vp, _i, _vp, _i, _i, _d, _d, _vp, _d, _i, C.c_uint64, _vp, _vp, _vp, _vp, _vp, _vp, _vp,
                           _vp]),
    "mo_triangulate_points": (_i, [_vp, _vp, _vp, _vp, _vp, _i, _vp]),
    "mo_dev_frontend_batch": (_i, [_vp, _vp, _vp]),
    "mo_dev_orb_detect_compute": (_i, [_vp, _vp, _vp, _i, _i, _i, _vp, _vp, _i, _vp]),
    "mo_dev_match_pairs": (_i, [_vp, _vp, _vp, _i, _vp, _vp, _i, _d, _vp, _vp, _vp]),
    "mo_dev_status": (_i, [_vp, _vp]),
    "mo_stream_create": (_vp, [_vp, _vp, _vp]),
    "mo_stream_destroy": (None, [_vp]),
    "mo_stream_submit": (_i, [_vp, _vp, _i, _i, C.c_size_t]),
    "mo_stream_collect": (_i, [_vp, _vp]),
    "mo_stream_last_error": (C.c_char_p, [_vp]),
    "mo_stream_lanes": (_i, []),
    "mo_comm_unique_id": (_i, [_vp]),
    "mo_comm_init": (_i, [_vp, _vp, _i, _i]),
    "mo_comm_destroy": (_i, [_vp]),
    "mo_gather_map_points": (_i, [_vp, _vp, _i, _i, _i, _i, _vp, _vp]),
    "mo_host_times": (_i, [_vp, _vp]),
    "mo_set_host_timing": (_i, [_vp, _i]),
    "mo_last_token": (_i, [_vp, _vp]),
    "mo_pair_frontend": (_i, [_vp, _vp, _vp, _vp, _vp]),
    "mo_stage_times": (_i, [_vp, _vp, _vp, _i]),
    "mo_stage_times_back": (_i, [_vp, _i, _vp, _vp, _i]),
    "mo_dbg_pyramid_level": (_i, [_vp, _vp, _vp, _i, _i, _i, _i, _vp, _vp, _vp]),
    "mo_dbg_fast_level": (_i, [_vp, _vp, _vp, _i, _i, _i, _vp, _i, _vp]),
    "mo_dbg_retain_best": (_i, [_vp, _vp, _i, _i, _i, _vp, _vp]),
    "mo_map_create": (_vp, [_vp, _i, _i, C.c_int64, C.c_int64]),
    "mo_map_destroy": (None, [_vp]),
    "mo_map_add_keyframe": (_i, [_vp, _vp, _vp, _vp, _i, _i, _i, _vp, _vp]),
    "mo_map_add_points": (_i, [_vp, _i, _vp, _vp, _vp, _vp, _vp, _vp, _vp, _vp]),
    "mo_map_remove_keyframes": (_i, [_vp, _vp, _i]),
    "mo_map_sizes": (_i, [_vp, _vp]),
    "mo_map_download": (_i, [_vp, _i, _vp, C.c_size_t]),
    "mo_map_write_ply": (_i, [_vp, C.c_char_p, _i, _vp]),
    "mo_map_relocalize": (_i, [_vp, _vp, _vp, _vp, _vp]),
    "mo_map_track": (_i, [_vp, _vp, _vp, _vp, _vp, _vp]),
    "mo_format_floats": (_i, [_vp, C.c_int64, _vp, C.c_size_t, _vp]),
}

_lib = None


def _preload_shared_hip_runtime():
    import importlib.util
    import sys
    if "torch" in sys.modules:
        return
    try:
        spec = importlib.util.find_spec("torch")
    except Exception:
        spec = None
    if spec is None or not spec.submodule_search_locations:
        return
    cand = os.path.join(list(spec.submodule_search_locations)[0], "lib", "libamdhip64.so")
    if os.path.exists(cand):
        try:
            C.CDLL(cand, mode=C.RTLD_GLOBAL)
        except OSError:
            pass


def load_library():
    global _lib
    if _lib is not None:
        return _lib
    if not os.path.exists(LIB_PATH):
        raise NativeUnavailable(
            "%s is missing: build it with `make -C visual-slam_amd/csrc` (or __graft_entry__.build()). "
            "There is no CPU fallback." % LIB_PATH)
    _preload_shared_hip_runtime()
    lib = C.CDLL(LIB_PATH)
    for name, (res, args) in SIGNATURES.items():
        try:
            fn = getattr(lib, name)
        except AttributeError:
            if os.environ.get("VSLAM_AMD_LIB"):
                continue
            raise
        fn.restype = res
        fn.argtypes = args
    if not os.environ.get("VSLAM_AMD_LIB") and lib.mo_abi_version() != ABI_VERSION:
        raise NativeUnavailable("libvslam_amd.so has ABI version %d, this binding was written for %d: rebuild (make -C visual-slam_amd/csrc)"
                                % (lib.mo_abi_version(), ABI_VERSION))
    _lib = lib
    return lib


def device_count():
    return int(load_library().mo_device_count())


def _ptr(a):
    return None if a is None else a.ctypes.data_as(C.c_void_p)


_resident = {}


def _bind_resident(ctx, token, kps_arr, desc):
    if not token or desc is None:
        return
    desc.flags.writeable = False
    kps_arr.flags.writeable = False
    key = id(desc)
    _resident[key] = (token, weakref.ref(ctx), weakref.ref(desc, lambda _, key=key: _resident.pop(key, None)), weakref.ref(kps_arr))


def resident_token(ctx, desc, kps_arr=None):
    e = _resident.get(id(desc))
    if e is None or e[1]() is not ctx or e[2]() is not desc:
        return 0
    if kps_arr is not None and e[3]() is not kps_arr:
        return 0
    return e[0]


def _resident_kps(desc):
    e = _resident.get(id(desc))
    return e[3]() if e is not None and e[2]() is desc else None


def orb_params(nfeatures=2000, scale_factor=1.2, nlevels=8, edge_threshold=31, fast_threshold=7,
               select_order=ORDER_LIBSTDCXX):
    return OrbParams(int(nfeatures), float(scale_factor), int(nlevels), int(edge_threshold), 0, 2, 0, 31,
                     int(fast_threshold), int(select_order))


class Context:

    def __init__(self, device=0, max_w=2048, max_h=2048, max_batch=1):
        self.lib = load_library()
        if self.lib.mo_device_count() <= 0:
            raise NativeUnavailable("no HIP device visible: the MI355X front-end has no CPU fallback")
        self.h = self.lib.mo_create(int(device), int(max_w), int(max_h), int(max_batch))
        if not self.h:
            raise NativeUnavailable(self.lib.mo_last_error(None).decode())
        self.device = device
        self.max_batch = max_batch

    def close(self):
        if getattr(self, "h", None):
            for m in list(getattr(self, "_maps", ())):
                m.close()
            self.lib.mo_destroy(self.h)
            self.h = None

    def __del__(self):
        try:
            self.close()
        except Exception:
            pass

    def _check(self, rc):
        if rc != MO_OK:
            raise NativeError(rc, self.lib.mo_last_error(self.h).decode())

    def set_stream(self, stream_handle):
        if stream_handle is None:
            self._check(self.lib.mo_set_stream(self.h, None))
        elif int(stream_handle) == 0:
            self._check(self.lib.mo_set_stream_null(self.h))
        else:
            self._check(self.lib.mo_set_stream(self.h, C.c_void_p(int(stream_handle))))

    def sync(self):
        self._check(self.lib.mo_sync(self.h))

    def dev_status(self):
        f = (C.c_int32 * 4)()
        rc = self.lib.mo_dev_status(self.h, f)
        if rc not in (MO_OK, MO_ERR_CAPACITY):
            self._check(rc)
        return int(f[0])

    @staticmethod
    def comm_unique_id():
        lib = load_library()
        buf = (C.c_uint8 * 128)()
        rc = lib.mo_comm_unique_id(buf)
        if rc != MO_OK:
            raise NativeUnavailable("RCCL could not be loaded (mo_comm_unique_id returned %d)" % rc)
        return bytes(buf)

    def comm_init(self, unique_id, rank, world):
        buf = (C.c_uint8 * 128).from_buffer_copy(unique_id)
        self._check(self.lib.mo_comm_init(self.h, buf, int(rank), int(world)))

    def gather_map_points(self, d_local_ptr, rows_local, rows_max, cap, root, d_all_ptr, d_rows_all_ptr):
        self._check(self.lib.mo_gather_map_points(self.h, C.c_void_p(d_local_ptr), int(rows_local), int(rows_max), int(cap), int(root),
                                                  C.c_void_p(d_all_ptr) if d_all_ptr else None, C.c_void_p(d_rows_all_ptr)))

    def stage_times(self, back=0):
        names = C.POINTER(C.c_char_p)()
        ms = (C.c_float * 32)()
        n = self.lib.mo_stage_times_back(self.h, back, C.byref(names), ms, 32)
        if n < 0:
            self._check(n)
        return [(names[i].decode(), float(ms[i])) for i in range(n)]

    def set_host_timing(self, on):
        self._check(self.lib.mo_set_host_timing(self.h, int(bool(on))))

    def host_times(self):
        us = (C.c_double * 4)()
        self._check(self.lib.mo_host_times(self.h, us))
        return dict(enqueue_us=us[0], wait_us=us[1], unpack_us=us[2], total_us=us[3])

    def orb_detect_compute(self, images, prm, want_desc=True, cap=None):
        a = np.ascontiguousarray(images, dtype=np.uint8)
        if a.ndim == 2:
            a = a[None]
        elif a.ndim == 3 and a.shape[-1] == 3 and images.ndim == 3:
            a = a[None]
        ch = 3 if a.ndim == 4 else 1
        b, h, w = a.shape[0], a.shape[1], a.shape[2]
        cap = int(cap or (prm.nfeatures + 1024))
        while True:
            kps = np.empty((b, cap), KP_DTYPE)
            desc = np.empty((b, cap, 32), np.uint8) if want_desc else None
            counts = np.zeros(b, np.int32)
            rc = self.lib.mo_orb_detect_compute(self.h, C.byref(prm), _ptr(a), w, h, w * ch, ch, b, _ptr(kps),
                                                _ptr(desc), cap, _ptr(counts))
            if rc == MO_ERR_CAPACITY and counts.max() > cap:
                cap = int(counts.max())
                continue
            self._check(rc)
            break
        self.last_token = 0
        if b == 1 and want_desc:
            tok = C.c_uint64(0)
            self.lib.mo_last_token(self.h, C.byref(tok))
            self.last_token = int(tok.value)
        out = []
        for f in range(b):
            n = int(counts[f])
            out.append((kps[f, :n], desc[f, :n] if want_desc and n else None))
        if self.last_token:
            _bind_resident(self, self.last_token, out[0][0], out[0][1])
        return out

    def orb_compute(self, image, prm, kps_in):
        a = np.ascontiguousarray(image, dtype=np.uint8)
        ch = 3 if a.ndim == 3 else 1
        h, w = a.shape[0], a.shape[1]
        k = np.ascontiguousarray(kps_in, KP_DTYPE)
        n = len(k)
        kept = np.zeros(max(n, 1), np.int32)
        desc = np.zeros((max(n, 1), 32), np.uint8)
        n_out = C.c_int(0)
        self._check(self.lib.mo_orb_compute(self.h, C.byref(prm), _ptr(a), w, h, w * ch, ch, _ptr(k), n, _ptr(kept),
                                            _ptr(desc), C.byref(n_out)))
        return kept[:n_out.value].copy(), desc[:n_out.value].copy()

    def grid_good_features(self, image, n_features):
        a = np.ascontiguousarray(image, dtype=np.uint8)
        ch = 3 if a.ndim == 3 else 1
        h, w = a.shape[0], a.shape[1]
        xy = np.zeros((64 * max(int(n_features) // 64, 1), 2), np.float32)
        n = C.c_int(0)
        self._check(self.lib.mo_orb_grid_good_features(self.h, _ptr(a), w, h, w * ch, ch, int(n_features), _ptr(xy), C.byref(n)))
        return xy[:n.value].copy()

    def grid_detect_compute(self, image, prm, n_features, records=False):
        a = np.ascontiguousarray(image, dtype=np.uint8)
        ch = 3 if a.ndim == 3 else 1
        h, w = a.shape[0], a.shape[1]
        slots = 64 * max(int(n_features) // 64, 1)
        xy = np.empty((slots, 2), np.float32)
        kept = np.empty(slots, np.int32)
        desc = np.empty((slots, 32), np.uint8)
        n, nk = C.c_int(0), C.c_int(0)
        self._check(self.lib.mo_orb_grid_detect_compute(self.h, C.byref(prm), _ptr(a), w, h, w * ch, ch, int(n_features), _ptr(xy),
                                                        C.byref(n), _ptr(kept), _ptr(desc), C.byref(nk)))
        xy, kept, desc = xy[:n.value], kept[:nk.value], desc[:nk.value]
        if not records:
            return xy, kept, desc
        rec = np.zeros(nk.value, KP_DTYPE)
        rec["x"], rec["y"] = xy[kept, 0], xy[kept, 1]
        rec["size"], rec["angle"], rec["class_id"] = 31.0, -1.0, -1
        tok = C.c_uint64(0)
        self.lib.mo_last_token(self.h, C.byref(tok))
        self.last_token = int(tok.value)
        if self.last_token and nk.value:
            _bind_resident(self, self.last_token, rec, desc)
        return xy, kept, desc, rec

    def undistort(self, image, K, dist):
        a = np.ascontiguousarray(image, dtype=np.uint8)
        ch = 3 if a.ndim == 3 else 1
        h, w = a.shape[0], a.shape[1]
        Kc = np.ascontiguousarray(K, np.float64).reshape(9)
        d5 = np.zeros(5); dd = np.asarray(dist, np.float64).ravel(); d5[:min(5, len(dd))] = dd[:5]
        out = np.empty_like(a)
        self._check(self.lib.mo_undistort(self.h, _ptr(a), w, h, w * ch, ch, _ptr(Kc), _ptr(d5), _ptr(out)))
        return out

    def dbg_min_eigen(self, gray):
        g = np.ascontiguousarray(gray, np.uint8)
        h, w = g.shape
        out = np.zeros((h, w), np.float32)
        self._check(self.lib.mo_dbg_min_eigen(self.h, _ptr(g), w, h, _ptr(out)))
        return out

    def match_knn2_ratio(self, q, t, ratio=None):
        if getattr(q, "ndim", 0) == 2 and _resident:
            tq, tt = resident_token(self, q), resident_token(self, t)
            if tq and tt:
                r = self.pair_frontend(_resident_kps(q), q, _resident_kps(t), t, MODE_INIT, np.eye(3), ratio=ratio, n_hyp=0, token1=tq, token2=tt)
                return r["idx"], r["dist"], r["keep"]
        q = np.ascontiguousarray(q, np.uint8)
        t = np.ascontiguousarray(t, np.uint8)
        single = q.ndim == 2
        if single:
            q, t = q[None], t[None]
        b, nq, nt = q.shape[0], q.shape[1], t.shape[1]
        idx = np.full((b, nq, 2), -1, np.int32)
        dist = np.full((b, nq, 2), np.iinfo(np.int32).max, np.int32)
        ps = np.zeros((b, nq), np.uint8)
        r = C.c_double(float(ratio)) if ratio is not None else None
        self._check(self.lib.mo_match_knn2_ratio(self.h, _ptr(q), nq, _ptr(t), nt, C.byref(r) if r is not None else None,
                                                 b, _ptr(idx), _ptr(dist), _ptr(ps)))
        if single:
            return idx[0], dist[0], ps[0].astype(bool)
        return idx, dist, ps.astype(bool)

    def init_two_view(self, p1, p2, K, thr_px=3.0, prob=0.999, n_hyp=4096, seed=4096):
        p1 = np.ascontiguousarray(p1, np.float32).reshape(-1, 2)
        p2 = np.ascontiguousarray(p2, np.float32).reshape(-1, 2)
        Kc = np.ascontiguousarray(K, np.float64).reshape(9)
        m = len(p1)
        R = np.zeros(9); t = np.zeros(3); E = np.zeros(9)
        ran = np.zeros(max(m, 1), np.uint8); inl = np.zeros(max(m, 1), np.uint8)
        X = np.zeros((max(m, 1), 3), np.float32)
        ng = C.c_int(0)
        self._check(self.lib.mo_init_two_view(self.h, _ptr(p1), _ptr(p2), m, _ptr(Kc), float(thr_px), float(prob),
                                              int(n_hyp), C.c_uint64(int(seed)), _ptr(R), _ptr(t), _ptr(E), _ptr(ran),
                                              _ptr(inl), _ptr(X), C.byref(ng)))
        return dict(R=R.reshape(3, 3), t=t.reshape(3, 1), E=E.reshape(3, 3), ransac_mask=ran[:m].astype(bool),
                    pose_mask=inl[:m].astype(bool), X=X[:m], n_good=ng.value)

    def recover_pose(self, E, p1, p2, K, mask=None):
        p1 = np.ascontiguousarray(p1, np.float32).reshape(-1, 2)
        p2 = np.ascontiguousarray(p2, np.float32).reshape(-1, 2)
        Ec = np.ascontiguousarray(E, np.float64).reshape(9); Kc = np.ascontiguousarray(K, np.float64).reshape(9)
        m = len(p1)
        mi = None if mask is None else np.ascontiguousarray(np.asarray(mask).ravel() != 0, np.uint8)
        R = np.zeros(9); t = np.zeros(3); mo = np.zeros(max(m, 1), np.uint8); X = np.zeros((max(m, 1), 3), np.float32); ng = C.c_int(0)
        self._check(self.lib.mo_recover_pose(self.h, _ptr(Ec), _ptr(p1), _ptr(p2), m, _ptr(Kc), _ptr(mi), _ptr(R), _ptr(t), _ptr(mo),
                                             _ptr(X), C.byref(ng)))
        return dict(n_good=ng.value, R=R.reshape(3, 3), t=t.reshape(3, 1), mask=mo[:m].astype(bool), X=X[:m])

    def find_fundamental(self, p1, p2, thr_px=3.0, prob=0.99, n_hyp=4096, seed=4096):
        p1 = np.ascontiguousarray(p1, np.float32).reshape(-1, 2)
        p2 = np.ascontiguousarray(p2, np.float32).reshape(-1, 2)
        m = len(p1)
        F = np.zeros(9); mask = np.zeros(max(m, 1), np.uint8); ni = C.c_int(0)
        self._check(self.lib.mo_find_fundamental(self.h, _ptr(p1), _ptr(p2), m, float(thr_px), float(prob), int(n_hyp),
                                                 C.c_uint64(int(seed)), _ptr(F), _ptr(mask), C.byref(ni)))
        if not np.isfinite(F).all():
            return None, np.zeros(m, bool)
        return F.reshape(3, 3), mask[:m].astype(bool)

    def pair_frontend(self, kps1, desc1, kps2, desc2, mode, K, width=0, height=0, ratio=0.75, disp_frac=0.02, thr_px=None, n_hyp=4096,
                      seed=4096, pair_index=0, token1=0, token2=0, want_matches=None):
        token1 = token1 or resident_token(self, desc1, kps1)
        token2 = token2 or resident_token(self, desc2, kps2)
        k1 = np.ascontiguousarray(kps1, KP_DTYPE).reshape(-1); k2 = np.ascontiguousarray(kps2, KP_DTYPE).reshape(-1)
        d1 = np.ascontiguousarray(desc1, np.uint8).reshape(-1, 32); d2 = np.ascontiguousarray(desc2, np.uint8).reshape(-1, 32)
        n1, n2 = len(k1), len(k2)
        if len(d1) != n1 or len(d2) != n2:
            raise ValueError("keypoints and descriptor rows differ in number (%d / %d, %d / %d)" % (n1, len(d1), n2, len(d2)))
        f1 = FrameRef(int(token1), _ptr(k1), _ptr(d1), n1); f2 = FrameRef(int(token2), _ptr(k2), _ptr(d2), n2)
        pp = PairParams()
        pp.mode = int(mode); pp.w = int(width); pp.h = int(height); pp.ratio = float(ratio if ratio is not None else -1.0)
        pp.disp_frac = float(disp_frac); pp.thr_px = float(thr_px if thr_px is not None else (1.0 if mode == MODE_TRACK else 3.0))
        pp.n_hyp = int(n_hyp); pp.seed = int(seed); pp.pair_index = int(pair_index)
        Kc = np.ascontiguousarray(K, np.float64).reshape(9)
        for i in range(9):
            pp.K[i] = Kc[i]
        o = PairOut()
        m1 = max(n1, 1)
        init = mode == MODE_INIT
        if want_matches is None:
            want_matches = init
        if want_matches:
            idx = np.empty((m1, 2), np.int32); dist = np.empty((m1, 2), np.int32); keep = np.empty(m1, np.uint8)
            o.match_idx, o.match_dist, o.match_pass = _ptr(idx), _ptr(dist), _ptr(keep)
        inl = np.zeros(m1, np.uint8)
        o.inlier = _ptr(inl)
        if init:
            ran = np.zeros(m1, np.uint8); X = np.empty((m1, 3), np.float32)
            o.ransac, o.X = _ptr(ran), _ptr(X)
        else:
            sel = np.empty((m1, 2), np.int32); sd = np.empty(m1, np.int32)
            o.sel_idx, o.sel_dist = _ptr(sel), _ptr(sd)
        self._check(self.lib.mo_pair_frontend(self.h, C.byref(f1), C.byref(f2), C.byref(pp), C.byref(o)))
        r = dict(R=np.array(o.R[:]).reshape(3, 3), t=np.array(o.t[:]).reshape(3, 1), E=np.array(o.E[:]).reshape(3, 3),
                 token1=int(o.token1), token2=int(o.token2))
        if want_matches:
            r.update(idx=idx[:n1], dist=dist[:n1], keep=keep[:n1].view(bool))
        if init:
            r.update(ransac_mask=ran[:n1].view(bool), pose_mask=inl[:n1].view(bool), X=X[:n1], n_good=int(o.n_good))
        else:
            n = int(o.n_sel)
            r.update(sel=sel[:n], sel_dist=sd[:n], inlier=inl[:n].view(bool), n_inliers=int(o.n_good))
        return r

    def track_pair(self, kps1, desc1, kps2, desc2, width, height, K, ratio=0.75, disp_frac=0.02, thr_px=1.0, n_hyp=4096,
                   seed=4096, pair_index=0, token1=0, token2=0):
        return self.pair_frontend(kps1, desc1, kps2, desc2, MODE_TRACK, K, width, height, ratio, disp_frac, thr_px, n_hyp, seed, pair_index,
                                  token1, token2, want_matches=False)

    def triangulate_points(self, P1, P2, p1, p2):
        P1 = np.ascontiguousarray(P1, np.float64).reshape(12)
        P2 = np.ascontiguousarray(P2, np.float64).reshape(12)
        p1 = np.ascontiguousarray(p1, np.float32).reshape(-1, 2)
        p2 = np.ascontiguousarray(p2, np.float32).reshape(-1, 2)
        n = len(p1)
        X4 = np.zeros((max(n, 1), 4), np.float32)
        self._check(self.lib.mo_triangulate_points(self.h, _ptr(P1), _ptr(P2), _ptr(p1), _ptr(p2), n, _ptr(X4)))
        return X4[:n]

    def dbg_pyramid_level(self, gray, prm, level, blurred=False):
        g = np.ascontiguousarray(gray, np.uint8)
        h, w = g.shape
        out = np.zeros(h * w, np.uint8)
        lw, lh = C.c_int(0), C.c_int(0)
        self._check(self.lib.mo_dbg_pyramid_level(self.h, C.byref(prm), _ptr(g), w, h, level, int(blurred), _ptr(out),
                                                  C.byref(lw), C.byref(lh)))
        return out[:lw.value * lh.value].reshape(lh.value, lw.value).copy()

    def dbg_fast_level(self, gray, prm, level):
        g = np.ascontiguousarray(gray, np.uint8)
        h, w = g.shape
        cap = w * h // 4 + 16
        out = np.zeros((cap, 3), np.int32)
        n = C.c_int(0)
        self._check(self.lib.mo_dbg_fast_level(self.h, C.byref(prm), _ptr(g), w, h, level, _ptr(out), cap, C.byref(n)))
        return out[:n.value].copy()

    def dbg_retain_best(self, resp, n_points, order):
        r = np.ascontiguousarray(resp, np.float32)
        out = np.zeros(max(len(r), 1), np.int32)
        n = C.c_int(0)
        self._check(self.lib.mo_dbg_retain_best(self.h, _ptr(r), len(r), int(n_points), int(order), _ptr(out), C.byref(n)))
        return out[:n.value].copy()


_default_ctx = None


def default_context():
    global _default_ctx
    if _default_ctx is None:
        dev = int(os.environ.get("VSLAM_AMD_DEVICE", os.environ.get("LOCAL_RANK", "0")))
        _default_ctx = Context(device=dev, max_w=4095, max_h=4095, max_batch=1)
    return _default_ctx
```

Before: 115,900.

## Fuse Gaussian blur of source level into pyramid resize kernel

```diff
diff --git a/include/vslam_amd.h b/include/vslam_amd.h
--- a/include/vslam_amd.h
+++ b/include/vslam_amd.h
@@ -327,6 +327,7 @@
 
 int mo_dbg_pyramid_level(mo_ctx*, const mo_orb_params*, const uint8_t* gray, int w, int h, int level, int blurred,
                          uint8_t* out , int* lw, int* lh);
+int mo_dbg_blur_level(mo_ctx*, int frame, int level, uint8_t* out , int* lw, int* lh, int* resize_blur);
 int mo_dbg_fast_level(mo_ctx*, const mo_orb_params*, const uint8_t* gray, int w, int h, int level,
                       int32_t* xys , int cap, int* n);
 int mo_dbg_min_eigen(mo_ctx*, const uint8_t* gray, int w, int h, float* eig );
diff --git a/visual-slam_amd/csrc/api.hip b/visual-slam_amd/csrc/api.hip
--- a/visual-slam_amd/csrc/api.hip
+++ b/visual-slam_amd/csrc/api.hip
@@ -58,16 +58,18 @@
     }
     if (host_call) mo_stage_mark(c, "h2d");
     else mo_stage_begin(c);
-    const int blur_margin = (c->plan.edge_threshold - 19) & ~3, pyr_margin = std::max(blur_margin - 4, 0);
+    const int blur_margin = mo_blur_margin(c->plan.edge_threshold), pyr_margin = mo_pyr_margin(c->plan.edge_threshold);
     if (batch <= MO_FS_MAX_BATCH && c->fs_ok) {
         if ((rc = orb_launch_front_single(c, d_gray, batch, d_desc != nullptr))) return rc;
         mo_stage_mark(c, "pyramid");
         if (d_desc) mo_stage_mark(c, "blur");
     } else {
-        if ((rc = orb_launch_pyramid(c, d_gray, batch, c->plan.nlevels, pyr_margin))) return rc;
+        bool blurred = false;
+        if ((rc = orb_launch_pyramid(c, d_gray, batch, c->plan.nlevels, pyr_margin, d_desc ? blur_margin : -1, &blurred))) return rc;
         mo_stage_mark(c, "pyramid");
         if (d_desc) {
-            if ((rc = orb_launch_blur(c, d_gray, batch, c->plan.nlevels, blur_margin))) return rc;
+            const int nl = c->plan.nlevels;
+            if ((rc = orb_launch_blur(c, d_gray, batch, nl, blur_margin, blurred ? nl - 1 : 0))) return rc;
             mo_stage_mark(c, "blur");
         }
     }
@@ -809,6 +811,21 @@
     return MO_OK;
 }
 
+extern "C" int mo_dbg_blur_level(mo_ctx* c, int frame, int level, uint8_t* out, int* lw, int* lh, int* resize_blur) {
+    if (!c) return MO_ERR_ARG;
+    HIPCHK(c, hipSetDevice(c->device));
+    if (!c->plan_valid) return mo_fail(c, MO_ERR_ARG, "no extraction has run on this context");
+    if (level < 0 || level >= c->plan.nlevels) return mo_fail(c, MO_ERR_ARG, "level out of range");
+    if (frame < 0 || frame >= c->batch_alloc) return mo_fail(c, MO_ERR_ARG, "frame out of range");
+    const LevelInfo& v = c->plan.lv[level];
+    *lw = v.w; *lh = v.h;
+    if (resize_blur) *resize_blur = c->rb_ok ? 1 : 0;
+    HIPCHK(c, hipMemcpy2DAsync(out, v.w, c->d_blur + (size_t)frame * c->plan.blur_stride + v.boff, v.bpitch, v.w, v.h,
+                               hipMemcpyDeviceToHost, c->stream));
+    HIPCHK(c, hipStreamSynchronize(c->stream));
+    return MO_OK;
+}
+
 extern "C" int mo_dbg_fast_level(mo_ctx* c, const mo_orb_params* p, const uint8_t* gray, int w, int h, int level,
                                  int32_t* xys, int cap, int* n) {
     if (!c) return MO_ERR_ARG;
diff --git a/visual-slam_amd/csrc/common.h b/visual-slam_amd/csrc/common.h
--- a/visual-slam_amd/csrc/common.h
+++ b/visual-slam_amd/csrc/common.h
@@ -85,6 +85,8 @@
     mo_orb_params plan_params{};
     Plan plan{};
     ResizeTab rtab[MO_MAX_LEVELS];
+    bool rb_ok = false;
+    int rb_margin = -1, rb_pyr_margin = -1;
     int batch_alloc = 0;
 
     uint8_t* d_in = nullptr;       size_t d_in_bytes = 0;
@@ -201,12 +203,17 @@
 
 int orb_launch_gray(mo_ctx* c, const uint8_t* d_bgr, int w, int h, int batch, uint8_t* d_gray);
 int orb_launch_ingest(mo_ctx* c, const uint8_t* src_mapped, int w, int h, int ch, uint8_t* d_gray, int* flags_clear);
-int orb_launch_pyramid(mo_ctx* c, const uint8_t* d_gray, int batch, int nlevels, int margin);
+inline int mo_blur_margin(int edge_threshold) { return (edge_threshold - 19) & ~3; }
+inline int mo_pyr_margin(int edge_threshold) { return std::max(mo_blur_margin(edge_threshold) - 4, 0); }
+int orb_launch_pyramid(mo_ctx* c, const uint8_t* d_gray, int batch, int nlevels, int margin, int blur_margin = -1,
+                       bool* blurred = nullptr);
+bool orb_plan_resize_blur(const Plan& P, int L, const std::vector<uint32_t>& xp, const std::vector<uint32_t>& yp, int margin,
+                          int blur_margin);
 #define MO_FS_MAX_BATCH 2
 int fs_build(mo_ctx* c);
 int orb_launch_front_single(mo_ctx* c, const uint8_t* d_gray, int batch, int want_blur);
 void mo_linear_coeffs(int srcsize, int dstsize, std::vector<int>& ofs, std::vector<int>& c1);
-int orb_launch_blur(mo_ctx* c, const uint8_t* d_gray, int batch, int nlevels, int margin);
+int orb_launch_blur(mo_ctx* c, const uint8_t* d_gray, int batch, int nlevels, int margin, int first_level = 0);
 int orb_launch_fast(mo_ctx* c, const uint8_t* d_gray, int batch, int level_lo = 0, int level_hi = MO_MAX_LEVELS);
 int orb_launch_select(mo_ctx* c, const uint8_t* d_gray, int batch, int level_lo = 0, int level_hi = MO_MAX_LEVELS);
 int orb_launch_describe(mo_ctx* c, const uint8_t* d_gray, int batch, mo_keypoint* d_kps, uint8_t* d_desc, int cap,
diff --git a/visual-slam_amd/csrc/ctx.hip b/visual-slam_amd/csrc/ctx.hip
--- a/visual-slam_amd/csrc/ctx.hip
+++ b/visual-slam_amd/csrc/ctx.hip
@@ -298,6 +298,9 @@
     P.fin_stride = fin_off;
     c->scratch_stride = (size_t)scr_off;
 
+    c->rb_margin = mo_blur_margin(P.edge_threshold);
+    c->rb_pyr_margin = mo_pyr_margin(P.edge_threshold);
+    c->rb_ok = nl >= 2;
     for (int L = 1; L < nl; L++) {
         std::vector<int> xo, xc, yo, yc;
         mo_linear_coeffs(P.lv[L - 1].w, P.lv[L].w, xo, xc);
@@ -318,6 +321,7 @@
             window_ok = std::min(xo[xl] + 1, P.lv[L - 1].w - 1) - xo[x] <= 7;
         }
         c->rtab[L].two_pass_ok = window_ok;
+        c->rb_ok = c->rb_ok && window_ok && orb_plan_resize_blur(P, L, xp, yp, c->rb_pyr_margin, c->rb_margin);
         size_t n = (size_t)wp + hp + 2 * dw + 2 * dh;
         int* d = nullptr;
         HIPCHK(c, hipMalloc((void**)&d, n * sizeof(int)));
diff --git a/visual-slam_amd/csrc/orb_kernels.hip b/visual-slam_amd/csrc/orb_kernels.hip
--- a/visual-slam_amd/csrc/orb_kernels.hip
+++ b/visual-slam_amd/csrc/orb_kernels.hip
@@ -175,12 +175,197 @@
 
 #define RS2_ROWS 136
 #define RS2_UNR 5
+
+__device__ __forceinline__ uint2 rs2_hrow(uint32_t w0, uint32_t w1, uint32_t w2, uint32_t sh8, const uint32_t (&sel)[4],
+                                          const uint32_t (&coef)[4]) {
+    const uint32_t u0 = __builtin_amdgcn_alignbyte(w1, w0, sh8), u1 = __builtin_amdgcn_alignbyte(w2, w1, sh8);
+    uint32_t hv[4];
+#pragma unroll
+    for (int k = 0; k < 4; k++) hv[k] = udot2(__builtin_amdgcn_perm(u1, u0, sel[k]), coef[k], 0u);
+    return make_uint2(hv[0] | (hv[1] << 16), hv[2] | (hv[3] << 16));
+}
+
+__device__ __forceinline__ uint32_t rs2_vrow(uint2 a, uint2 b, uint32_t e) {
+    const uint32_t c1 = e >> 16, cy = (256u - c1) | (c1 << 16);
+    const uint32_t v0 = udot2(__builtin_amdgcn_perm(b.x, a.x, 0x05040100u), cy, 32768u);
+    const uint32_t v1 = udot2(__builtin_amdgcn_perm(b.x, a.x, 0x07060302u), cy, 32768u);
+    const uint32_t v2 = udot2(__builtin_amdgcn_perm(b.y, a.y, 0x05040100u), cy, 32768u);
+    const uint32_t v3 = udot2(__builtin_amdgcn_perm(b.y, a.y, 0x07060302u), cy, 32768u);
+    return __builtin_amdgcn_perm(v1, v0, 0x0C0C0602u) | (__builtin_amdgcn_perm(v3, v2, 0x0C0C0602u) << 16);
+}
+
+__device__ __forceinline__ uint32_t hi16_pair_sat_u8(uint32_t a, uint32_t b) {
+    uint32_t d;
+    asm("v_sat_pk_u8_i16 %0, %1" : "=v"(d) : "v"(__builtin_amdgcn_perm(b, a, 0x07060302u)));
+    return d;
+}
+
+__device__ __forceinline__ uint4 blur_row_quad(const uint32_t* pw0, const uint32_t* pw1, uint32_t g0, uint32_t g1, uint32_t g2,
+                                               uint32_t g3) {
+    const uint32_t ta = g0 | (g1 << 8) | (g2 << 16) | (g3 << 24), tb = g2 | (g1 << 8) | (g0 << 16);
+    uint32_t o[2][4];
+#pragma unroll
+    for (int h = 0; h < 2; h++) {
+        const uint32_t* pw = h ? pw1 : pw0;
+        const uint32_t w0 = pw[0], w1 = pw[1], w2 = pw[2];
+        o[h][0] = __builtin_amdgcn_udot4(__builtin_amdgcn_alignbyte(w1, w0, 1), ta, __builtin_amdgcn_udot4(__builtin_amdgcn_alignbyte(w2, w1, 1), tb, 0, false), false);
+        o[h][1] = __builtin_amdgcn_udot4(__builtin_amdgcn_alignbyte(w1, w0, 2), ta, __builtin_amdgcn_udot4(__builtin_amdgcn_alignbyte(w2, w1, 2), tb, 0, false), false);
+        o[h][2] = __builtin_amdgcn_udot4(__builtin_amdgcn_alignbyte(w1, w0, 3), ta, __builtin_amdgcn_udot4(__builtin_amdgcn_alignbyte(w2, w1, 3), tb, 0, false), false);
+        o[h][3] = __builtin_amdgcn_udot4(w1, ta, __builtin_amdgcn_udot4(w2, tb, 0, false), false);
+    }
+    return make_uint4(o[0][0] | (o[1][0] << 16), o[0][1] | (o[1][1] << 16), o[0][2] | (o[1][2] << 16), o[0][3] | (o[1][3] << 16));
+}
+
+__device__ __forceinline__ void blur_col_quad(const uint32_t* sr, int pitch, uint32_t g0, uint32_t g1, uint32_t g2, uint32_t g3,
+                                              uint32_t& pe, uint32_t& po) {
+    const uint32_t e0 = g0 | (g1 << 16), e1 = g2 | (g3 << 16), e2 = g2 | (g1 << 16), e3 = g0;
+    const uint32_t d0 = g0 << 16, d1 = g1 | (g2 << 16), d2 = g3 | (g2 << 16), d3 = g1 | (g0 << 16);
+    uint4 v[4];
+#pragma unroll
+    for (int j = 0; j < 4; j++) v[j] = *(const uint4*)(sr + j * pitch);
+    uint32_t se[4], so[4];
+#pragma unroll
+    for (int k = 0; k < 4; k++) {
+        const uint32_t a0 = k == 0 ? v[0].x : k == 1 ? v[0].y : k == 2 ? v[0].z : v[0].w;
+        const uint32_t a1 = k == 0 ? v[1].x : k == 1 ? v[1].y : k == 2 ? v[1].z : v[1].w;
+        const uint32_t a2 = k == 0 ? v[2].x : k == 1 ? v[2].y : k == 2 ? v[2].z : v[2].w;
+        const uint32_t a3 = k == 0 ? v[3].x : k == 1 ? v[3].y : k == 2 ? v[3].z : v[3].w;
+        se[k] = udot2(a0, e0, udot2(a1, e1, udot2(a2, e2, udot2(a3, e3, 1u << 15))));
+        so[k] = udot2(a0, d0, udot2(a1, d1, udot2(a2, d2, udot2(a3, d3, 1u << 15))));
+    }
+    pe = hi16_pair_sat_u8(se[0], se[1]) | (hi16_pair_sat_u8(se[2], se[3]) << 16);
+    po = hi16_pair_sat_u8(so[0], so[1]) | (hi16_pair_sat_u8(so[2], so[3]) << 16);
+}
+
+#define RB_PW 80
+#define RB_PH 80
+#define RB_WR 88
+#define RB_WP 96
+#define RB_SR_BYTES ((RB_PH / 2 + 4) * RB_PW * 4)
+struct BlurOut {
+    uint8_t* dst;
+    size_t fstride;
+    int pitch, margin;
+    uint32_t taps;
+};
+
+template <bool RS2_BLUR>
 __global__ __launch_bounds__(256) void k_resize2(const uint8_t* __restrict__ src, size_t src_fstride, int spitch, int sw, int sh,
                                                  uint8_t* __restrict__ dst, size_t dst_fstride, int dpitch, int dw, int dh,
                                                  const uint32_t* __restrict__ xpk, const uint32_t* __restrict__ ypk,
-                                                 uint32_t inv_per, uint32_t inv_gx, int org) {
+                                                 uint32_t inv_per, uint32_t inv_gx, int org, BlurOut bo) {
+    const int tid = threadIdx.x;
+    if constexpr (RS2_BLUR) {
+        __shared__ __attribute__((aligned(16))) uint8_t s_px[RB_WR * RB_WP];
+        __shared__ __attribute__((aligned(16))) uint32_t s_row[RB_SR_BYTES / 4];
+        int bx = blockIdx.x, by = blockIdx.y, bz = blockIdx.z;
+        {
+            int rem;
+            xcd_map(bx + gridDim.x * (by + gridDim.y * bz), gridDim.x * gridDim.y, inv_per, gridDim.z, bz, rem);
+            by = (int)(inv_gx ? __umulhi((uint32_t)rem, inv_gx) : (uint32_t)rem);
+            bx = rem - by * (int)gridDim.x;
+        }
+        const int tx0 = org + bx * RS_TW, ty0 = org + by * RS_TH;
+        const uint32_t ey0 = ypk[ty0], ey1 = ypk[ty0 + RS_TH - 1], ex1 = xpk[tx0 + RS_TW - 1];
+        const int sy0 = (int)(ey0 & 0x7FFFu), sy1 = (int)(ey1 & 0x7FFFu) + (int)((ey1 >> 15) & 1u);
+        const int ab0 = (int)(xpk[tx0] & 0x7FFCu), ax1 = (int)(ex1 & 0x7FFFu) + (int)((ex1 >> 15) & 1u) + 1;
+        const int bm = bo.margin;
+        const int r0 = by == 0 ? bm : sy0, r1 = by == (int)gridDim.y - 1 ? sh - bm : (int)(ypk[ty0 + RS_TH] & 0x7FFFu);
+        const int c0 = bx == 0 ? bm : ab0, c1 = bx == (int)gridDim.x - 1 ? (sw - bm + 3) & ~3 : (int)(xpk[tx0 + RS_TW] & 0x7FFCu);
+        const int wy0 = min(r0 - 3, sy0), wy1 = max(r1 + 3, sy1 + 1);
+        const int wx0 = min(c0 - 4, ab0), wx1 = max(c1 + 4, (ax1 + 3) & ~3);
+        const int nwr = wy1 - wy0, ndw = (wx1 - wx0) >> 2;
+        const uint8_t* img = src + (size_t)bz * src_fstride;
+        const int cg = tid & 15, rr = tid >> 4;
+        const uint4 xe = *(const uint4*)(xpk + tx0 + 4 * cg);
+        uint32_t ye[RS_TH / 16];
+#pragma unroll
+        for (int half = 0; half < RS_TH / 16; half++) ye[half] = ypk[ty0 + rr + 16 * half];
+        {
+            constexpr int TRIPS = (RB_WR * (RB_WP / 4 - 2) + 255) / 256;
+            const uint32_t inv = 0x100000u / (uint32_t)ndw + 1u;
+            const bool inside = wy0 >= 0 && wy1 <= sh && wx0 >= 0 && wx1 <= sw;
+            uint32_t v[TRIPS];
+#pragma unroll
+            for (int t = 0; t < TRIPS; t++) {
+                const int i = min(tid + 256 * t, nwr * ndw - 1);
+                const uint32_t r = ((uint32_t)i * inv) >> 20, c4 = (uint32_t)i - r * (uint32_t)ndw;
+                const int x0 = wx0 + 4 * (int)c4;
+                if (inside) {
+                    v[t] = *(const uint32_t*)(img + (uint32_t)((wy0 + (int)r) * spitch + x0));
+                } else {
+                    const uint8_t* row = img + (uint32_t)(reflect101(wy0 + (int)r, sh) * spitch);
+                    if (x0 >= 0 && x0 + 3 < sw) v[t] = *(const uint32_t*)(row + x0);
+                    else {
+                        uint32_t u = 0;
+#pragma unroll
+                        for (int b = 0; b < 4; b++) u |= (uint32_t)row[reflect101(x0 + b, sw)] << (8 * b);
+                        v[t] = u;
+                    }
+                }
+            }
+#pragma unroll
+            for (int t = 0; t < TRIPS; t++) {
+                const int i = tid + 256 * t;
+                if (i < nwr * ndw) {
+                    const uint32_t r = ((uint32_t)i * inv) >> 20, c4 = (uint32_t)i - r * (uint32_t)ndw;
+                    ((uint32_t*)(s_px + r * RB_WP))[c4] = v[t];
+                }
+            }
+        }
+        __syncthreads();
+        {
+            const uint32_t xk[4] = {xe.x, xe.y, xe.z, xe.w};
+            const int ox0 = (int)(xk[0] & 0x7FFFu), ab = ox0 & ~3;
+            const uint32_t sh8 = (uint32_t)(ox0 & 3);
+            uint32_t sel[4], coef[4];
+#pragma unroll
+            for (int k = 0; k < 4; k++) {
+                const uint32_t a = (xk[k] & 0x7FFFu) - (uint32_t)ox0, b = a + ((xk[k] >> 15) & 1u), c1k = xk[k] >> 16;
+                sel[k] = a | (b << 16) | 0x0C000C00u;
+                coef[k] = (256u - c1k) | (c1k << 16);
+            }
+            const int x = tx0 + 4 * cg;
+            const uint32_t* pw = (const uint32_t*)(s_px + (ab - wx0));
+#pragma unroll
+            for (int half = 0; half < RS_TH / 16; half++) {
+                const int y = ty0 + rr + 16 * half;
+                if (x >= dw || y >= dh) break;
+                const uint32_t e = ye[half];
+                const int oy = (int)(e & 0x7FFFu) - wy0, oy1 = oy + (int)((e >> 15) & 1u);
+                const uint32_t* p0 = pw + oy * (RB_WP / 4);
+                const uint32_t* p1 = pw + oy1 * (RB_WP / 4);
+                const uint2 a = rs2_hrow(p0[0], p0[1], p0[2], sh8, sel, coef), b = rs2_hrow(p1[0], p1[1], p1[2], sh8, sel, coef);
+                *(uint32_t*)(dst + (size_t)bz * dst_fstride + (size_t)y * dpitch + x) = rs2_vrow(a, b, e);
+            }
+        }
+        const uint32_t g0 = bo.taps & 255u, g1 = (bo.taps >> 8) & 255u, g2 = (bo.taps >> 16) & 255u, g3 = bo.taps >> 24;
+        const int nq = (c1 - c0) >> 2, npr = (r1 - r0 + 7) >> 1, nop = (r1 - r0 + 1) >> 1;
+        const uint32_t invq = 0x100000u / (uint32_t)max(nq, 1) + 1u;
+        {
+            const uint8_t* base = s_px + (r0 - 3 - wy0) * RB_WP + (c0 - 4 - wx0);
+            for (int t = tid; t < npr * nq; t += 256) {
+                const int p = (int)(((uint32_t)t * invq) >> 20), q = t - p * nq;
+                const uint32_t* pw = (const uint32_t*)(base + 2 * p * RB_WP + 4 * q);
+                *(uint4*)(s_row + p * RB_PW + 4 * q) = blur_row_quad(pw, pw + RB_WP / 4, g0, g1, g2, g3);
+            }
+        }
+        __syncthreads();
+        {
+            uint8_t* out0 = bo.dst + (size_t)bz * bo.fstride;
+            for (int t = tid; t < nop * nq; t += 256) {
+                const int p = (int)(((uint32_t)t * invq) >> 20), q = t - p * nq;
+                uint32_t pe, po;
+                blur_col_quad(s_row + p * RB_PW + 4 * q, RB_PW, g0, g1, g2, g3, pe, po);
+                const int y = r0 + 2 * p;
+                uint8_t* out = out0 + (size_t)y * bo.pitch + c0 + 4 * q;
+                *(uint32_t*)out = pe;
+                if (y + 1 < r1) *(uint32_t*)(out + bo.pitch) = po;
+            }
+        }
+        return;
+    }
     __shared__ __attribute__((aligned(16))) uint2 s_h[RS2_ROWS][16];
-    const int tid = threadIdx.x;
     int bx = blockIdx.x, by = blockIdx.y, bz = blockIdx.z;
     {
         int rem;
@@ -221,11 +406,7 @@
         for (int i = 0; i < RS2_UNR; i++) {
             const int r = r0 + 16 * i;
             if (r >= nrows) break;
-            const uint32_t u0 = __builtin_amdgcn_alignbyte(w[i][1], w[i][0], sh8), u1 = __builtin_amdgcn_alignbyte(w[i][2], w[i][1], sh8);
-            uint32_t hv[4];
-#pragma unroll
-            for (int k = 0; k < 4; k++) hv[k] = udot2(__builtin_amdgcn_perm(u1, u0, sel[k]), coef[k], 0u);
-            s_h[r][cg] = make_uint2(hv[0] | (hv[1] << 16), hv[2] | (hv[3] << 16));
+            s_h[r][cg] = rs2_hrow(w[i][0], w[i][1], w[i][2], sh8, sel, coef);
         }
     }
     __syncthreads();
@@ -235,33 +416,69 @@
     for (int half = 0; half < RS_TH / 16; half++) {
         const int y = ty0 + rr + 16 * half;
         if (y >= dh) break;
-        const uint32_t e = ye[half], c1 = e >> 16, cy = (256u - c1) | (c1 << 16);
+        const uint32_t e = ye[half];
         const int oy = (int)(e & 0x7FFFu) - sy0, oy1 = oy + (int)((e >> 15) & 1u);
-        const uint2 a = s_h[oy][cg], b = s_h[oy1][cg];
-        const uint32_t v0 = udot2(__builtin_amdgcn_perm(b.x, a.x, 0x05040100u), cy, 32768u);
-        const uint32_t v1 = udot2(__builtin_amdgcn_perm(b.x, a.x, 0x07060302u), cy, 32768u);
-        const uint32_t v2 = udot2(__builtin_amdgcn_perm(b.y, a.y, 0x05040100u), cy, 32768u);
-        const uint32_t v3 = udot2(__builtin_amdgcn_perm(b.y, a.y, 0x07060302u), cy, 32768u);
-        const uint32_t packed = __builtin_amdgcn_perm(v1, v0, 0x0C0C0602u) | (__builtin_amdgcn_perm(v3, v2, 0x0C0C0602u) << 16);
+        const uint32_t packed = rs2_vrow(s_h[oy][cg], s_h[oy1][cg], e);
         *(uint32_t*)(dst + (size_t)bz * dst_fstride + (size_t)y * dpitch + x) = packed;
     }
 }
 
-int orb_launch_pyramid(mo_ctx* c, const uint8_t* d_gray, int batch, int nlevels, int margin) {
+static int resize_org(const LevelInfo& d, int margin) { return (d.w > 2 * margin + 8 && d.h > 2 * margin + 8) ? margin : 0; }
+
+bool orb_plan_resize_blur(const Plan& P, int L, const std::vector<uint32_t>& xp, const std::vector<uint32_t>& yp, int margin,
+                          int blur_margin) {
+    const LevelInfo& s = P.lv[L - 1];
+    const LevelInfo& d = P.lv[L];
+    const int bm = blur_margin, org = resize_org(d, margin);
+    if (bm < 0 || (bm & 3)) return false;
+    const int gx = (d.w - 2 * org + RS_TW - 1) / RS_TW, gy = (d.h - 2 * org + RS_TH - 1) / RS_TH;
+    if (gx < 1 || gy < 1 || (size_t)(org + gx * RS_TW + 1) > xp.size() || (size_t)(org + gy * RS_TH + 1) > yp.size()) return false;
+    for (int by = 0; by < gy; by++) {
+        const int ty0 = org + by * RS_TH;
+        const uint32_t ey1 = yp[ty0 + RS_TH - 1];
+        const int sy0 = (int)(yp[ty0] & 0x7FFFu), sy1 = (int)(ey1 & 0x7FFFu) + (int)((ey1 >> 15) & 1u);
+        const int r0 = by == 0 ? bm : sy0, r1 = by == gy - 1 ? s.h - bm : (int)(yp[ty0 + RS_TH] & 0x7FFFu);
+        const int wy0 = std::min(r0 - 3, sy0), wy1 = std::max(r1 + 3, sy1 + 1);
+        if (r1 <= r0 || r1 - r0 > RB_PH || wy1 - wy0 > RB_WR || r1 + 4 - wy0 > RB_WR || sy1 >= s.h) return false;
+    }
+    for (int bx = 0; bx < gx; bx++) {
+        const int tx0 = org + bx * RS_TW;
+        const uint32_t ex1 = xp[tx0 + RS_TW - 1];
+        const int ab0 = (int)(xp[tx0] & 0x7FFCu), ax1 = (int)(ex1 & 0x7FFFu) + (int)((ex1 >> 15) & 1u) + 1;
+        const int c0 = bx == 0 ? bm : ab0, c1 = bx == gx - 1 ? (s.w - bm + 3) & ~3 : (int)(xp[tx0 + RS_TW] & 0x7FFCu);
+        const int wx0 = std::min(c0 - 4, ab0), wx1 = std::max(c1 + 4, (ax1 + 3) & ~3);
+        if (c1 <= c0 || c1 - c0 > RB_PW || wx1 - wx0 + 8 > RB_WP || ax1 > s.w) return false;
+    }
+    return true;
+}
+
+int orb_launch_pyramid(mo_ctx* c, const uint8_t* d_gray, int batch, int nlevels, int margin, int blur_margin, bool* blurred) {
     const Plan& P = c->plan;
+    auto src_of = [&](int L) { return L == 1 ? d_gray : c->d_pyr + P.lv[L - 1].off; };
+    auto sfs_of = [&](int L) { return L == 1 ? (size_t)P.w * P.h : (size_t)P.pyr_stride; };
+    auto al4_of = [&](int L) { return ((((size_t)src_of(L)) | sfs_of(L) | (size_t)P.lv[L - 1].pitch) & 3) == 0 && P.lv[L - 1].pitch >= 12; };
+    bool fuse = blur_margin >= 0 && nlevels == P.nlevels && nlevels >= 2 && c->rb_ok && c->rb_margin == blur_margin &&
+                c->rb_pyr_margin == margin;
+    for (int L = 1; L < nlevels && fuse; L++) fuse = al4_of(L) && c->rtab[L].two_pass_ok;
+    if (blurred) *blurred = fuse;
+    const uint32_t taps = (uint32_t)P.gk[0] | ((uint32_t)P.gk[1] << 8) | ((uint32_t)P.gk[2] << 16) | ((uint32_t)P.gk[3] << 24);
     for (int L = 1; L < nlevels; L++) {
         const LevelInfo& s = P.lv[L - 1];
         const LevelInfo& d = P.lv[L];
-        const uint8_t* src = L == 1 ? d_gray : c->d_pyr + s.off;
-        size_t sfs = L == 1 ? (size_t)P.w * P.h : (size_t)P.pyr_stride;
+        const uint8_t* src = src_of(L);
+        size_t sfs = sfs_of(L);
         const ResizeTab& t = c->rtab[L];
-        const int org = (d.w > 2 * margin + 8 && d.h > 2 * margin + 8) ? margin : 0;
+        const int org = resize_org(d, margin);
         dim3 grid((d.w - 2 * org + RS_TW - 1) / RS_TW, (d.h - 2 * org + RS_TH - 1) / RS_TH, batch);
         const uint32_t per = grid.x * grid.y, inv_per = per > 1 ? 0xFFFFFFFFu / per + 1u : 0u, inv_gx = grid.x > 1 ? 0xFFFFFFFFu / grid.x + 1u : 0u;
-        const bool al4 = ((((size_t)src) | sfs | (size_t)s.pitch) & 3) == 0 && s.pitch >= 12;
-        if (al4 && t.two_pass_ok)
-            hipLaunchKernelGGL(k_resize2, grid, dim3(256), 0, c->stream, src, sfs, s.pitch, s.w, s.h, c->d_pyr + d.off,
-                               (size_t)P.pyr_stride, d.pitch, d.w, d.h, t.xpk, t.ypk, inv_per, inv_gx, org);
+        const bool al4 = al4_of(L);
+        if (fuse) {
+            const BlurOut bo{c->d_blur + s.boff, (size_t)P.blur_stride, s.bpitch, blur_margin, taps};
+            hipLaunchKernelGGL(k_resize2<true>, grid, dim3(256), 0, c->stream, src, sfs, s.pitch, s.w, s.h, c->d_pyr + d.off,
+                               (size_t)P.pyr_stride, d.pitch, d.w, d.h, t.xpk, t.ypk, inv_per, inv_gx, org, bo);
+        } else if (al4 && t.two_pass_ok)
+            hipLaunchKernelGGL(k_resize2<false>, grid, dim3(256), 0, c->stream, src, sfs, s.pitch, s.w, s.h, c->d_pyr + d.off,
+                               (size_t)P.pyr_stride, d.pitch, d.w, d.h, t.xpk, t.ypk, inv_per, inv_gx, org, BlurOut{});
         else
             hipLaunchKernelGGL(k_resize, grid, dim3(256), 0, c->stream, src, sfs, s.pitch, s.w, s.h, c->d_pyr + d.off,
                                (size_t)P.pyr_stride, d.pitch, d.w, d.h, t.xofs, t.xc1, t.yofs, t.yc1, inv_per, inv_gx, org);
@@ -277,21 +494,14 @@
 #define BT_PW (BT_W + 16)
 #define BT_ROWS (BT_H + 6)
 
-
-__device__ __forceinline__ uint32_t hi16_pair_sat_u8(uint32_t a, uint32_t b) {
-    uint32_t d;
-    asm("v_sat_pk_u8_i16 %0, %1" : "=v"(d) : "v"(__builtin_amdgcn_perm(b, a, 0x07060302u)));
-    return d;
-}
-
-__global__ __launch_bounds__(256) void k_blur(Plan P, const uint32_t* __restrict__ tile_tab, uint32_t inv_per, int org,
+__global__ __launch_bounds__(256) void k_blur(Plan P, const uint32_t* __restrict__ tile_tab, int tile0, uint32_t inv_per, int org,
                                               const uint8_t* __restrict__ gray, const uint8_t* __restrict__ pyr,
                                               uint8_t* __restrict__ blur) {
     __shared__ __attribute__((aligned(16))) uint8_t s_px[BT_ROWS * BT_PW];
     __shared__ __attribute__((aligned(16))) uint32_t s_row[(BT_ROWS / 2) * BT_W];
     int tile = blockIdx.x, frame = blockIdx.y;
     xcd_map(blockIdx.x + gridDim.x * blockIdx.y, gridDim.x, inv_per, gridDim.y, frame, tile);
-    const uint32_t te = tile_tab[tile];
+    const uint32_t te = tile_tab[tile0 + tile];
     const int L = te & 0xFF;
     const LevelInfo lv = P.lv[L];
     const int tx0 = org + (int)((te >> 8) & 0xFFF) * BT_W, ty0 = org + (int)(te >> 20) * BT_H;
@@ -333,24 +543,9 @@
     const uint32_t g0 = P.gk[0], g1 = P.gk[1], g2 = P.gk[2], g3 = P.gk[3];
 #pragma unroll
     for (int h2 = 0; h2 < BT_ROWS / 2 / BT_PP; h2++) {
-        const uint32_t ta = g0 | (g1 << 8) | (g2 << 16) | (g3 << 24), tb = g2 | (g1 << 8) | (g0 << 16);
         const int p = tid / BT_QW + BT_PP * h2, q = tid % BT_QW;
-        uint32_t o[2][4];
-#pragma unroll
-        for (int h = 0; h < 2; h++) {
-            const uint32_t* pw = (const uint32_t*)(s_px + (2 * p + h) * BT_PW + 4 * q);
-            const uint32_t w0 = pw[0], w1 = pw[1], w2 = pw[2];
-            o[h][0] = __builtin_amdgcn_udot4(__builtin_amdgcn_alignbyte(w1, w0, 1), ta, __builtin_amdgcn_udot4(__builtin_amdgcn_alignbyte(w2, w1, 1), tb, 0, false), false);
-            o[h][1] = __builtin_amdgcn_udot4(__builtin_amdgcn_alignbyte(w1, w0, 2), ta, __builtin_amdgcn_udot4(__builtin_amdgcn_alignbyte(w2, w1, 2), tb, 0, false), false);
-            o[h][2] = __builtin_amdgcn_udot4(__builtin_amdgcn_alignbyte(w1, w0, 3), ta, __builtin_amdgcn_udot4(__builtin_amdgcn_alignbyte(w2, w1, 3), tb, 0, false), false);
-            o[h][3] = __builtin_amdgcn_udot4(w1, ta, __builtin_amdgcn_udot4(w2, tb, 0, false), false);
-        }
-        uint4 packed;
-        packed.x = o[0][0] | (o[1][0] << 16);
-        packed.y = o[0][1] | (o[1][1] << 16);
-        packed.z = o[0][2] | (o[1][2] << 16);
-        packed.w = o[0][3] | (o[1][3] << 16);
-        *(uint4*)(&s_row[p * BT_W + 4 * q]) = packed;
+        const uint32_t* pw = (const uint32_t*)(s_px + 2 * p * BT_PW + 4 * q);
+        *(uint4*)(&s_row[p * BT_W + 4 * q]) = blur_row_quad(pw, pw + BT_PW / 4, g0, g1, g2, g3);
     }
     __syncthreads();
 #pragma unroll
@@ -358,23 +553,8 @@
         const int p = tid / BT_QW + BT_PP * h2, c0 = (tid % BT_QW) * 4;
         const int x = tx0 + c0, y = ty0 + 2 * p;
         if (p < BT_H / 2 && y < lv.h && x < lv.w) {
-            const uint32_t e0 = g0 | (g1 << 16), e1 = g2 | (g3 << 16), e2 = g2 | (g1 << 16), e3 = g0;
-            const uint32_t d0 = g0 << 16, d1 = g1 | (g2 << 16), d2 = g3 | (g2 << 16), d3 = g1 | (g0 << 16);
-            uint4 v[4];
-#pragma unroll
-            for (int j = 0; j < 4; j++) v[j] = *(const uint4*)(&s_row[(p + j) * BT_W + c0]);
-            uint32_t se[4], so[4];
-#pragma unroll
-            for (int k = 0; k < 4; k++) {
-                const uint32_t a0 = k == 0 ? v[0].x : k == 1 ? v[0].y : k == 2 ? v[0].z : v[0].w;
-                const uint32_t a1 = k == 0 ? v[1].x : k == 1 ? v[1].y : k == 2 ? v[1].z : v[1].w;
-                const uint32_t a2 = k == 0 ? v[2].x : k == 1 ? v[2].y : k == 2 ? v[2].z : v[2].w;
-                const uint32_t a3 = k == 0 ? v[3].x : k == 1 ? v[3].y : k == 2 ? v[3].z : v[3].w;
-                se[k] = udot2(a0, e0, udot2(a1, e1, udot2(a2, e2, udot2(a3, e3, 1u << 15))));
-                so[k] = udot2(a0, d0, udot2(a1, d1, udot2(a2, d2, udot2(a3, d3, 1u << 15))));
-            }
-            const uint32_t pe = hi16_pair_sat_u8(se[0], se[1]) | (hi16_pair_sat_u8(se[2], se[3]) << 16);
-            const uint32_t po = hi16_pair_sat_u8(so[0], so[1]) | (hi16_pair_sat_u8(so[2], so[3]) << 16);
+            uint32_t pe, po;
+            blur_col_quad(&s_row[p * BT_W + c0], BT_W, g0, g1, g2, g3, pe, po);
             uint8_t* out = blur + (size_t)frame * P.blur_stride + lv.boff + (size_t)y * lv.bpitch + x;
             *(uint32_t*)out = pe;
             if (y + 1 < lv.h) *(uint32_t*)(out + lv.bpitch) = po;
@@ -382,9 +562,10 @@
     }
 }
 
-int orb_launch_blur(mo_ctx* c, const uint8_t* d_gray, int batch, int nlevels, int margin) {
+int orb_launch_blur(mo_ctx* c, const uint8_t* d_gray, int batch, int nlevels, int margin, int first_level) {
     const Plan& P = c->plan;
-    if (nlevels < 1 || nlevels > P.nlevels) return mo_fail(c, MO_ERR_ARG, "blur: level count outside the plan");
+    if (nlevels < 1 || nlevels > P.nlevels || first_level < 0 || first_level >= nlevels)
+        return mo_fail(c, MO_ERR_ARG, "blur: level range outside the plan");
     const int slot = margin > 0 ? 1 : 0;
     if (slot && c->tile_margin != margin && c->d_tile_tab[1]) { hipFree(c->d_tile_tab[1]); c->d_tile_tab[1] = nullptr; }
     if (!c->d_tile_tab[slot]) {
@@ -401,9 +582,10 @@
         HIPCHK(c, hipMemcpy(c->d_tile_tab[slot], tab.data(), tab.size() * sizeof(uint32_t), hipMemcpyHostToDevice));
         if (slot) c->tile_margin = margin;
     }
-    const uint32_t per = (uint32_t)c->tile_cum[slot][nlevels], inv_per = per > 1 ? 0xFFFFFFFFu / per + 1u : 0u;
-    hipLaunchKernelGGL(k_blur, dim3(per, batch), dim3(256), 0, c->stream, P, c->d_tile_tab[slot], inv_per, margin, d_gray, c->d_pyr,
-                       c->d_blur);
+    const int tile0 = c->tile_cum[slot][first_level];
+    const uint32_t per = (uint32_t)(c->tile_cum[slot][nlevels] - tile0), inv_per = per > 1 ? 0xFFFFFFFFu / per + 1u : 0u;
+    hipLaunchKernelGGL(k_blur, dim3(per, batch), dim3(256), 0, c->stream, P, c->d_tile_tab[slot], tile0, inv_per, margin, d_gray,
+                       c->d_pyr, c->d_blur);
     HIPCHK(c, hipGetLastError());
     return MO_OK;
 }
diff --git a/visual-slam_amd/vslam_amd/__init__.py b/visual-slam_amd/vslam_amd/__init__.py
--- a/visual-slam_amd/vslam_amd/__init__.py
+++ b/visual-slam_amd/vslam_amd/__init__.py
@@ -162,6 +162,7 @@
     "mo_stage_times": (_i, [_vp, _vp, _vp, _i]),
     "mo_stage_times_back": (_i, [_vp, _i, _vp, _vp, _i]),
     "mo_dbg_pyramid_level": (_i, [_vp, _vp, _vp, _i, _i, _i, _i, _vp, _vp, _vp]),
+    "mo_dbg_blur_level": (_i, [_vp, _i, _i, _vp, _vp, _vp, _vp]),
     "mo_dbg_fast_level": (_i, [_vp, _vp, _vp, _i, _i, _i, _vp, _i, _vp]),
     "mo_dbg_retain_best": (_i, [_vp, _vp, _i, _i, _i, _vp, _vp]),
     "mo_map_create": (_vp, [_vp, _i, _i, C.c_int64, C.c_int64]),
@@ -569,6 +570,12 @@
                                                   C.byref(lw), C.byref(lh)))
         return out[:lw.value * lh.value].reshape(lh.value, lw.value).copy()
 
+    def dbg_blur_level(self, frame, level, w, h):
+        lw, lh, rb = C.c_int(0), C.c_int(0), C.c_int(0)
+        out = np.zeros(w * h, np.uint8)
+        self._check(self.lib.mo_dbg_blur_level(self.h, int(frame), int(level), _ptr(out), C.byref(lw), C.byref(lh), C.byref(rb)))
+        return out[:lw.value * lh.value].reshape(lh.value, lw.value).copy(), bool(rb.value)
+
     def dbg_fast_level(self, gray, prm, level):
         g = np.ascontiguousarray(gray, np.uint8)
         h, w = g.shape
```

New measurement: 119,300 (median of 6 runs). 2.9% higher.
